# kienduynguyen/BoxeR

Hardware: AMD Instinct MI355X
Metric: box-attn fwd+bwd Gsample-points/s + achieved HBM GB/s, BoxeR-R50 COCO shapes (higher is better)
Workload: dtype bf16; 1 GPU; C2: box-attn fwd+bwd, levels 100x100/50x50/25x25/13x13, Lq=13294, H=8, C=32, P=4, B=2 images per GPU, inputs=model; parallelism=dp1, preheat_steps=2128, parity_gate=not run (--full runs it)

## Files before the change

boxer_amd/csrc/boxattn_binned.h:

```cpp
#pragma once
#include <type_traits>

#include "boxattn_device.h"
#include "boxattn_combine.h"
#include "boxattn_binplan.h"
#include "boxattn_scan_tail.h"
#include "boxattn_binpass.h"

namespace boxattn {

#ifndef BOXATTN_TUNE_BIN_THREADS
#define BOXATTN_TUNE_BIN_THREADS 512
#endif
constexpr int kBinThreads = BOXATTN_TUNE_BIN_THREADS;
template <int BW, int BH, bool FILL, bool WIDE, int PT>
__global__ __launch_bounds__(kBinThreads) void bin_kernel(const float *__restrict__ loc,
                                                  const float *__restrict__ w_sp, BinPlan plan,
                                                  int H, int Lq, int P, int q_per_wg, int n_wg, int interleave,
                                                  int *__restrict__ part,
                                                  const int *__restrict__ subtot,
                                                  const int *__restrict__ offsets,
                                                  int *__restrict__ records, int *__restrict__ ctickets)
{
    if (FILL && ctickets && blockIdx.x == 0)
        for (int k = threadIdx.x; k < plan.nblk; k += kBinThreads) ctickets[(size_t)blockIdx.y * plan.nblk + k] = 0;
    extern __shared__ int sh_bins[];
    __shared__ BinLevel s_lv[kMaxBinLevels];
    const int s = blockIdx.y, wg = blockIdx.x;
    bin_pass_body<kBinThreads, BW, BH, FILL, WIDE, PT>(sh_bins, s_lv, loc, w_sp, plan, H, Lq, P, q_per_wg, n_wg,
                                                       interleave != 0, part, subtot, offsets, records, s, wg);
    if constexpr (!FILL) {
        int *mypart = part + ((size_t)s * n_wg + wg) * plan.nblk;
        for (int k = threadIdx.x; k < plan.nblk; k += kBinThreads) mypart[k] = sh_bins[k];
    }
}

__global__ __launch_bounds__(256) void bin_scan_a_kernel(int *__restrict__ part, int n_wg,
                                                         int *__restrict__ subtot, BinPlan plan)
{
    const int sub = blockIdx.x, s = blockIdx.y;
    const int wps = scan_wps(n_wg);
    const int w_lo = sub * wps, w_hi = min(n_wg, w_lo + wps);
    int *sp = part + (size_t)s * n_wg * plan.nblk;
    for (int k = blockIdx.z * 256 + threadIdx.x; k < plan.nblk; k += 256 * gridDim.z) {
        int t[kScanWgPerSub], sum = 0;
#pragma unroll
        for (int u = 0; u < kScanWgPerSub; ++u)
            t[u] = w_lo + u < w_hi ? sp[(size_t)(w_lo + u) * plan.nblk + k] : 0;
#pragma unroll
        for (int u = 0; u < kScanWgPerSub; ++u) {
            if (w_lo + u < w_hi) sp[(size_t)(w_lo + u) * plan.nblk + k] = sum;
            sum += t[u];
        }
        subtot[((size_t)s * kScanSub + sub) * plan.nblk + k] = sum;
    }
}

__global__ __launch_bounds__(kScanThreads) void bin_scan_kernel(int *__restrict__ subtot,
                                                       int *__restrict__ offsets,
                                                       int4 *__restrict__ items,
                                                       int4 *__restrict__ combos,
                                                       int *__restrict__ n_items, BinPlan plan,
                                                       int *__restrict__ part, int fuse_wg)
{
    __shared__ int wsum[4][kScanThreads / 64];
    __shared__ int carry[4];
    const int s = blockIdx.x, lane = threadIdx.x & 63, wv = threadIdx.x >> 6;
    if (threadIdx.x < 4) carry[threadIdx.x] = 0;
    __syncthreads();
    for (int k0 = 0; k0 < plan.nblk; k0 += kScanThreads) {
        const int k = k0 + threadIdx.x;
        const bool live = k < plan.nblk;
        int c = 0;
        if (live && fuse_wg > 0) {
            const int wps = scan_wps(fuse_wg);
            int *sp = part + (size_t)s * fuse_wg * plan.nblk + k;
            for (int u = 0; u < kScanSub; ++u) {
                subtot[((size_t)s * kScanSub + u) * plan.nblk + k] = c;
                int in_sub = 0;
                const int w_hi = min(fuse_wg, (u + 1) * wps);
                for (int w = u * wps; w < w_hi; ++w) {
                    const int t = sp[(size_t)w * plan.nblk];
                    sp[(size_t)w * plan.nblk] = in_sub;
                    in_sub += t;
                }
                c += in_sub;
            }
        } else if (live) {
            int t[kScanSub];
#pragma unroll
            for (int u = 0; u < kScanSub; ++u)
                t[u] = subtot[((size_t)s * kScanSub + u) * plan.nblk + k];
#pragma unroll
            for (int u = 0; u < kScanSub; ++u) {
                subtot[((size_t)s * kScanSub + u) * plan.nblk + k] = c;
                c += t[u];
            }
        }
        const int nch = live ? max(plan.min_items, (c + plan.chunk - 1) / plan.chunk) : 0;
        const int v[4] = {c, nch, nch > 1 ? nch : 0, nch > 1 ? 1 : 0};
        int inc[4];
#pragma unroll
        for (int i = 0; i < 4; ++i) {
            int x = v[i];
#pragma unroll
            for (int o = 1; o < 64; o <<= 1) {
                const int t = __shfl_up(x, o, 64);
                if (lane >= o) x += t;
            }
            inc[i] = x;
            if (lane == 63) wsum[i][wv] = x;
        }
        __syncthreads();
        int ex[4];
#pragma unroll
        for (int i = 0; i < 4; ++i) {
            int pre = carry[i];
            for (int w = 0; w < wv; ++w) pre += wsum[i][w];
            ex[i] = pre + inc[i] - v[i];
        }
        int tot_items = carry[1];
        for (int w = 0; w < kScanThreads / 64; ++w) tot_items += wsum[1][w];
        if (live) {
            offsets[(size_t)s * (plan.nblk + 1) + k] = ex[0];
            int level = 0;
#pragma unroll
            for (int l = 1; l < kMaxBinLevels; ++l)
                if (l < plan.L && k >= plan.lv[l].blk0) level = l;
            BinLevel lv = plan.lv[0];
#pragma unroll
            for (int l = 1; l < kMaxBinLevels; ++l)
                if (l == level) lv = plan.lv[l];
            const int geo = (int)pack_block_geo(lv, level, k);
            const int csz = chunk_records(c, nch);
            for (int j = 0; j < nch; ++j)
                items[(size_t)s * plan.item_cap + (tot_items - 1 - (ex[1] + j))] =
                    make_int4(geo, ex[0] + j * csz, ex[0] + min(c, (j + 1) * csz),
                              nch > 1 ? (ex[2] + j) | (ex[3] << kItemSlotBits) : -1);
            if (nch > 1)
                combos[(size_t)s * plan.nblk + ex[3]] = make_int4(geo, ex[2], nch, 0);
        }
        __syncthreads();
        if (threadIdx.x == kScanThreads - 1) {
#pragma unroll
            for (int i = 0; i < 4; ++i) carry[i] = ex[i] + v[i];
        }
        __syncthreads();
    }
    if (threadIdx.x == 0) {
        offsets[(size_t)s * (plan.nblk + 1) + plan.nblk] = carry[0];
        n_items[2 * s] = carry[1];
        n_items[2 * s + 1] = carry[3];
    }
}

__global__ __launch_bounds__(kScanThreads) void bin_scan_seg_kernel(int *__restrict__ subtot,
                                                                    int *__restrict__ offsets,
                                                                    int4 *__restrict__ tmp,
                                                                    int4 *__restrict__ segtot,
                                                                    BinPlan plan, int *__restrict__ part = nullptr,
                                                                    int fuse_wg = 0)
{
    __shared__ int wsum[4][kScanThreads / 64];
    const int seg = blockIdx.x, s = blockIdx.y, lane = threadIdx.x & 63, wv = threadIdx.x >> 6;
    const int k = seg * kScanThreads + (int)threadIdx.x;
    const bool live = k < plan.nblk;
    int c = 0;
    if (live && fuse_wg > 0) {
        const int wps = scan_wps(fuse_wg);
        int *sp = part + (size_t)s * fuse_wg * plan.nblk + k;
        for (int u = 0; u < kScanSub; ++u) {
            subtot[((size_t)s * kScanSub + u) * plan.nblk + k] = c;
            int in_sub = 0;
            const int w_hi = min(fuse_wg, (u + 1) * wps);
            for (int w = u * wps; w < w_hi; ++w) {
                const int t = sp[(size_t)w * plan.nblk];
                sp[(size_t)w * plan.nblk] = in_sub;
                in_sub += t;
            }
            c += in_sub;
        }
    } else if (live) {
        int t[kScanSub];
#pragma unroll
        for (int u = 0; u < kScanSub; ++u) t[u] = subtot[((size_t)s * kScanSub + u) * plan.nblk + k];
#pragma unroll
        for (int u = 0; u < kScanSub; ++u) {
            subtot[((size_t)s * kScanSub + u) * plan.nblk + k] = c;
            c += t[u];
        }
    }
    const int nch = live ? max(plan.min_items, (c + plan.chunk - 1) / plan.chunk) : 0;
    const int v[4] = {c, nch, nch > 1 ? nch : 0, nch > 1 ? 1 : 0};
    int inc[4];
#pragma unroll
    for (int i = 0; i < 4; ++i) {
        int x = v[i];
#pragma unroll
        for (int o = 1; o < 64; o <<= 1) {
            const int t = __shfl_up(x, o, 64);
            if (lane >= o) x += t;
        }
        inc[i] = x;
        if (lane == 63) wsum[i][wv] = x;
    }
    __syncthreads();
    int ex[4], tot[4];
#pragma unroll
    for (int i = 0; i < 4; ++i) {
        int pre = 0, all = 0;
#pragma unroll
        for (int w = 0; w < kScanThreads / 64; ++w) {
            pre += w < wv ? wsum[i][w] : 0;
            all += wsum[i][w];
        }
        ex[i] = pre + inc[i] - v[i];
        tot[i] = all;
    }
    if (live) {
        offsets[(size_t)s * (plan.nblk + 1) + k] = c;
        tmp[(size_t)s * plan.nblk + k] = make_int4(ex[0], ex[1], ex[2], ex[3]);
    }
    if (threadIdx.x == 0)
        segtot[(size_t)s * gridDim.x + seg] = make_int4(tot[0], tot[1], tot[2], tot[3]);
}

__global__ __launch_bounds__(kScanThreads) void bin_scan_emit_kernel(int *__restrict__ offsets,
                                                                     const int4 *__restrict__ tmp,
                                                                     const int4 *__restrict__ segtot,
                                                                     int4 *__restrict__ items,
                                                                     int4 *__restrict__ combos,
                                                                     int *__restrict__ n_items,
                                                                     BinPlan plan)
{
    const int seg = blockIdx.x, s = blockIdx.y;
    int base[4] = {0, 0, 0, 0}, all[4] = {0, 0, 0, 0};
    for (int g = 0; g < (int)gridDim.x; ++g) {
        const int4 t = segtot[(size_t)s * gridDim.x + g];
        const int tv[4] = {t.x, t.y, t.z, t.w};
#pragma unroll
        for (int i = 0; i < 4; ++i) {
            base[i] += g < seg ? tv[i] : 0;
            all[i] += tv[i];
        }
    }
    const int k = seg * kScanThreads + (int)threadIdx.x;
    if (k < plan.nblk) {
        const int c = offsets[(size_t)s * (plan.nblk + 1) + k];
        const int4 e = tmp[(size_t)s * plan.nblk + k];
        const int ex[4] = {base[0] + e.x, base[1] + e.y, base[2] + e.z, base[3] + e.w};
        const int nch = max(plan.min_items, (c + plan.chunk - 1) / plan.chunk);
        offsets[(size_t)s * (plan.nblk + 1) + k] = ex[0];
        int level = 0;
#pragma unroll
        for (int l = 1; l < kMaxBinLevels; ++l)
            if (l < plan.L && k >= plan.lv[l].blk0) level = l;
        BinLevel lv = plan.lv[0];
#pragma unroll
        for (int l = 1; l < kMaxBinLevels; ++l)
            if (l == level) lv = plan.lv[l];
        const int geo = (int)pack_block_geo(lv, level, k);
        const int csz = chunk_records(c, nch);
        for (int j = 0; j < nch; ++j)
            items[(size_t)s * plan.item_cap + (all[1] - 1 - (ex[1] + j))] =
                make_int4(geo, ex[0] + j * csz, ex[0] + min(c, (j + 1) * csz),
                          nch > 1 ? (ex[2] + j) | (ex[3] << kItemSlotBits) : -1);
        if (nch > 1) combos[(size_t)s * plan.nblk + ex[3]] = make_int4(geo, ex[2], nch, 0);
    }
    if (seg == 0 && threadIdx.x == 0) {
        offsets[(size_t)s * (plan.nblk + 1) + plan.nblk] = all[0];
        n_items[2 * s] = all[1];
        n_items[2 * s + 1] = all[3];
    }
}

#ifndef BOXATTN_TUNE_ABLATE
#define BOXATTN_TUNE_ABLATE 0
#endif
#ifndef BOXATTN_TUNE_ACC_WPE
#define BOXATTN_TUNE_ACC_WPE 1
#endif
template <typename ST, int C, bool INST, int RPL = 1, bool WIDE = false>
__global__ __launch_bounds__(64) __attribute__((amdgpu_waves_per_eu(BOXATTN_TUNE_ACC_WPE)))
void binned_accumulate_kernel(
    const ST *__restrict__ grad_out, const ST *__restrict__ grad_mask,
    const float *__restrict__ loc, const float *__restrict__ w_sp,
    const float *__restrict__ w_lv, BinPlan plan, int S, int H, int Lq, int P,
    const int *__restrict__ offsets, const int4 *__restrict__ items,
    const int *__restrict__ n_items, const int *__restrict__ records,
    ST *__restrict__ grad_value, float *__restrict__ partials, ChunkCombine cc, ZeroRole zr)
{
    constexpr int BW = 8, PB = 32;
    constexpr int R = 64 * RPL;
    constexpr int CH = C / 2;
    constexpr int ROWB = C * (int)sizeof(ST);
#ifndef BOXATTN_TUNE_STAGE_F32
#define BOXATTN_TUNE_STAGE_F32 0
#endif
    constexpr bool kCvt = INST || (BOXATTN_TUNE_STAGE_F32 && sizeof(ST) == 2);
    constexpr int SB = kCvt ? 4 : (int)sizeof(ST);
    constexpr int RS = C * SB + 16;
    constexpr int LPR = ROWB / 16;
    constexpr int RPP = 64 / LPR;
    constexpr int NPASS = R / RPP;
    constexpr int EPL = 16 / (int)sizeof(ST);
#ifndef BOXATTN_TUNE_UNR
#define BOXATTN_TUNE_UNR 2
#endif
    constexpr int UNR = BOXATTN_TUNE_UNR;
    typedef float2 Entry;
    typedef unsigned int u32x4 __attribute__((ext_vector_type(4)));
    constexpr int NQ = CH * SB / 16;
    auto staged_pair = [](const u32x4 (&rw)[NQ], int i) -> f32x2 {
        f32x2 r;
        if constexpr (SB == 4) {
            r.x = __uint_as_float(rw[(2 * i) / 4][(2 * i) % 4]);
            r.y = __uint_as_float(rw[(2 * i + 1) / 4][(2 * i + 1) % 4]);
        } else {
            const unsigned wd = rw[i / 4][i % 4];
            r.x = __uint_as_float(wd << 16); r.y = __uint_as_float(wd & 0xffff0000u);
        }
        return r;
    };
    __shared__ __attribute__((aligned(16))) unsigned char gstage[(R + 1) * RS];
    __shared__ __attribute__((aligned(16))) Entry ent[4 * R + PB * (UNR - 1) + UNR];
    __shared__ int pcnt[PB + 1], poff[PB + 1];
    __shared__ int last_flag;

    const int n_slices = plan.n_slices, workers = (int)gridDim.x - plan.zero_workers;
    const int bid = blockIdx.y * gridDim.x + blockIdx.x;
    const int xcd = bid % 8, k = bid / 8;
    const int per_xcd = (n_slices + 7) / 8;
// ... 296 lines not shown
```

boxer_amd/csrc/boxattn_binned_tr.h:

```cpp
#pragma once
#include "boxattn_binplan.h"
#include "boxattn_combine.h"
#include "boxattn_scan_tail.h"
#include "boxattn_binpass.h"

namespace boxattn {

#ifndef BOXATTN_TUNE_TR_WPE
#define BOXATTN_TUNE_TR_WPE 4
#endif
#ifndef BOXATTN_TUNE_REC_AHEAD
#define BOXATTN_TUNE_REC_AHEAD 1
#endif

typedef __bf16 tr_bf16x8 __attribute__((ext_vector_type(8)));
typedef float tr_f32x16 __attribute__((ext_vector_type(16)));
typedef short tr_i16x4 __attribute__((ext_vector_type(4)));
__device__ __forceinline__ uint2 lds_read_tr16(const unsigned short *base, unsigned byte_off)
{
    typedef __attribute__((address_space(3))) tr_i16x4 lds_vec;
    const tr_i16x4 v = __builtin_amdgcn_ds_read_tr16_b64_v4i16(
        (lds_vec *)(reinterpret_cast<const char *>(base) + byte_off));
    return __builtin_bit_cast(uint2, v);
}

template <typename ST, int C>
__global__ __launch_bounds__(64) __attribute__((amdgpu_waves_per_eu(C <= 32 ? BOXATTN_TUNE_TR_WPE : 1))) void binned_accumulate_tr_kernel(
    const ST *__restrict__ grad_out, unsigned grad_out_bytes, BinPlan plan, int S, int H, int Lq,
    const int4 *__restrict__ items, const int *__restrict__ n_items,
    const int *__restrict__ records, ST *__restrict__ grad_value, float *__restrict__ partials, ChunkCombine cc,
    ZeroRole zr)
{
    static_assert(sizeof(ST) == 2, "bf16 storage");
    static_assert(C == 16 || C == 32 || C == 64, "channels per head");
    constexpr int BW = 8, PB = 32, R = 64;
    constexpr int CP = C < 32 ? 32 : C;
    constexpr int NCB = CP / 32;
    constexpr int ROWB = C * 2;
    constexpr int LPR = ROWB / 16;
    constexpr int RPP = 64 / LPR;
    constexpr int NPASS = R / RPP;
    constexpr int GPL = R * 64;
    constexpr int AS = 72;
    constexpr int ASB = AS * 2;
    constexpr int kDump = PB * ASB;
    constexpr int kBig = 1 << 20;
    typedef unsigned int u32x4 __attribute__((ext_vector_type(4)));
    __shared__ __attribute__((aligned(16))) unsigned short gs[NCB * GPL / 2];
    __shared__ __attribute__((aligned(16))) unsigned short at[(PB + 1) * AS];
    __shared__ int last_flag;

    const int n_slices = plan.n_slices, workers = (int)gridDim.x - plan.zero_workers;
    const int bid = blockIdx.y * gridDim.x + blockIdx.x;
    const int xcd = bid % 8, kq = bid / 8;
    const int per_xcd = (n_slices + 7) / 8;
    const int s = slice_on_xcd(xcd, kq % per_xcd, per_xcd);
    const int worker = kq / per_xcd - plan.zero_workers;
    if (s >= n_slices || worker >= workers) return;
    const int b = s / H, h = s % H;
    const int lane = threadIdx.x;
    if (worker < 0) {
        if (zr.redo) redo_blocks<ST, C>(zr, plan, s, worker + plan.zero_workers, plan.zero_workers, S, H, Lq, grad_out, grad_value, lane);
        else zero_empty_blocks<ST, C>(zr, plan.nblk, s, worker + plan.zero_workers, S, H, grad_value, lane);
        return;
    }
    const int col = lane & 31, kb = lane >> 5;
    const int n_it = n_items[2 * s];

    for (int i = lane; i < (PB + 1) * AS / 2; i += 64) reinterpret_cast<unsigned int *>(at)[i] = 0u;
    if (C < CP)
        for (int i = lane; i < NCB * GPL / 4; i += 64) reinterpret_cast<unsigned int *>(gs)[i] = 0u;
    wave_lds_sync();

    const __amdgpu_buffer_rsrc_t rs =
        __builtin_amdgcn_make_buffer_rsrc(const_cast<ST *>(grad_out), 0, grad_out_bytes, 0x00020000);
    const unsigned slice_off = (unsigned)((b * Lq) * H + h) * (unsigned)ROWB;
    const unsigned q_stride = (unsigned)(H * ROWB);
    const int piece = lane % LPR, jrow = lane / LPR;
    const unsigned stage_off = (unsigned)((piece >> 2) * GPL + jrow * 64 + (piece & 3) * 16);
    const int g16 = lane >> 4, i16 = lane & 15;
    const unsigned tr_off = (unsigned)((8 * (g16 >> 1) + (i16 >> 2)) * 64 + (16 * (g16 & 1) + 4 * (i16 & 3)) * 2);
    unsigned a_off = (unsigned)(col * ASB + 16 * kb);
    asm volatile("" : "+v"(a_off));

    const int4 *my_items = items + (size_t)s * plan.item_cap;
    int4 item_n = my_items[min(worker, plan.item_cap - 1)];
    for (int it = worker; it < n_it; it += workers) {
        const int4 item = item_n;
        item_n = my_items[min(it + workers, plan.item_cap - 1)];
        const BlockGeo bg = unpack_block_geo((unsigned)item.x);
        int lvH = plan.lv[0].H, lvW = plan.lv[0].W, lv_start = plan.lv[0].start;
#pragma unroll
        for (int k = 1; k < kMaxBinLevels; ++k)
            if (k == bg.level) { lvH = plan.lv[k].H; lvW = plan.lv[k].W; lv_start = plan.lv[k].start; }
        const int oy = bg.oy, ox = bg.ox, bh = bg.bh, bw = bg.bw;
        const float Hf = (float)lvH, Wf = (float)lvW;
        const int4 *rec = reinterpret_cast<const int4 *>(records) + (size_t)s * plan.rec_cap;
        tr_f32x16 acc[NCB];
#pragma unroll
        for (int cb = 0; cb < NCB; ++cb)
#pragma unroll
            for (int r = 0; r < 16; ++r) acc[cb][r] = 0.f;

        constexpr unsigned kNoRow = 0x80000000u;
        auto fetch_rec = [&](int rr) -> int4 {
            if (rr + lane >= item.z) return make_int4(-1, 0, 0, 0);
            return rec[rr + lane];
        };
        auto fetch_rows = [&](const int4 &r, u32x4 (&rows)[NPASS]) {
            const unsigned id = (unsigned)r.x;
            const unsigned off = r.x < 0 ? kNoRow : __umul24(id >> plan.lp_bits, q_stride) + slice_off;
#pragma unroll
            for (int ps = 0; ps < NPASS; ++ps) {
                const unsigned oj = (unsigned)__shfl((int)off, ps * RPP + jrow, 64) + (unsigned)(piece * 16);
                rows[ps] = __builtin_amdgcn_raw_buffer_load_b128(rs, oj, 0, 0);
            }
        };
        auto stage_rows = [&](const u32x4 (&rows)[NPASS]) {
#pragma unroll
            for (int ps = 0; ps < NPASS; ++ps)
                *reinterpret_cast<u32x4 *>(reinterpret_cast<char *>(gs) + stage_off + ps * RPP * 64) = rows[ps];
        };
        int4 rec_c = fetch_rec(item.y), rec_n = fetch_rec(item.y + R), rec_n2 = fetch_rec(item.y + 2 * R);
        u32x4 grow_a[NPASS], grow_b[NPASS];
        fetch_rows(rec_c, grow_a);
        stage_rows(grow_a);
        if (item.y + R < item.z) fetch_rows(rec_n, grow_a);
        auto round = [&](int rr, const u32x4 (&next)[NPASS], u32x4 (&ahead)[NPASS]) {
            const bool more = rr + R < item.z;
            int4 rec_n3 = make_int4(-1, 0, 0, 0);
            if (rr + 2 * R < item.z) {
                fetch_rows(rec_n2, ahead);
                rec_n3 = fetch_rec(rr + 3 * R);
            }
            const float x = __int_as_float(rec_c.y), y = __int_as_float(rec_c.z), a = __int_as_float(rec_c.w);
            float h_im, w_im;
            {
#pragma clang fp contract(off)
                h_im = y * Hf - 0.5f;
                w_im = x * Wf - 0.5f;
            }
            const float yf = floorf(h_im), xf = floorf(w_im);
            const float lh = h_im - yf, lw = w_im - xf;
            const int py = rec_c.x >= 0 ? (int)yf - oy : -2, px = (int)xf - ox;
            const float hh = 1.f - lh, hw = 1.f - lw;
            const float ha = hh * a, la = lh * a;
            const float w0 = ha * hw, w1 = ha * lw, w2 = la * hw, w3 = la * lw;
            const unsigned hi01 = pack_bf16x2(w0, w1), hi23 = pack_bf16x2(w2, w3);
            const unsigned lo01 = pack_bf16x2(w0 - __uint_as_float(hi01 << 16), w1 - __uint_as_float(hi01 & 0xffff0000u));
            const unsigned lo23 = pack_bf16x2(w2 - __uint_as_float(hi23 << 16), w3 - __uint_as_float(hi23 & 0xffff0000u));
            const int r0 = (unsigned)py < (unsigned)bh ? __mul24(py, BW * ASB) : kBig;
            const int r1 = (unsigned)(py + 1) < (unsigned)bh ? __mul24(py, BW * ASB) + BW * ASB : kBig;
            const int c0 = (unsigned)px < (unsigned)bw ? __mul24(px, ASB) + 2 * lane : kBig;
            const int c1 = (unsigned)(px + 1) < (unsigned)bw ? __mul24(px, ASB) + 2 * lane + ASB : kBig;
            const int dump = kDump + 2 * lane;
            const int slot[4] = {min(r0 + c0, dump), min(r0 + c1, dump), min(r1 + c0, dump), min(r1 + c1, dump)};
            auto put = [&](int k, unsigned short v) {
                *reinterpret_cast<unsigned short *>(reinterpret_cast<char *>(at) + slot[k]) = v;
            };
            put(0, (unsigned short)(hi01 & 0xffffu)); put(1, (unsigned short)(hi01 >> 16));
            put(2, (unsigned short)(hi23 & 0xffffu)); put(3, (unsigned short)(hi23 >> 16));
            wave_lds_sync();
            tr_bf16x8 g[R / 16][NCB];
#pragma unroll
            for (int t = 0; t < R / 16; ++t) {
                const tr_bf16x8 p_hi = __builtin_bit_cast(
                    tr_bf16x8, *reinterpret_cast<const u32x4 *>(reinterpret_cast<const char *>(at) + a_off + 32 * t));
#pragma unroll
                for (int cb = 0; cb < NCB; ++cb) {
                    const uint2 g0 = lds_read_tr16(gs, tr_off + cb * GPL + t * 1024);
                    const uint2 g1 = lds_read_tr16(gs, tr_off + cb * GPL + t * 1024 + 256);
                    g[t][cb] = __builtin_bit_cast(tr_bf16x8, u32x4{g0.x, g0.y, g1.x, g1.y});
                    acc[cb] = __builtin_amdgcn_mfma_f32_32x32x16_bf16(g[t][cb], p_hi, acc[cb], 0, 0, 0);
                }
            }
            wave_lds_sync();
            put(0, (unsigned short)(lo01 & 0xffffu)); put(1, (unsigned short)(lo01 >> 16));
            put(2, (unsigned short)(lo23 & 0xffffu)); put(3, (unsigned short)(lo23 >> 16));
            wave_lds_sync();
#pragma unroll
            for (int t = 0; t < R / 16; ++t) {
                const tr_bf16x8 p_lo = __builtin_bit_cast(
                    tr_bf16x8, *reinterpret_cast<const u32x4 *>(reinterpret_cast<const char *>(at) + a_off + 32 * t));
#pragma unroll
                for (int cb = 0; cb < NCB; ++cb)
                    acc[cb] = __builtin_amdgcn_mfma_f32_32x32x16_bf16(g[t][cb], p_lo, acc[cb], 0, 0, 0);
            }
            wave_lds_sync();
#pragma unroll
            for (int k = 0; k < 4; ++k) put(k, (unsigned short)0);
            if (more) {
                stage_rows(next);
                rec_c = rec_n; rec_n = rec_n2; rec_n2 = rec_n3;
            }
            wave_lds_sync();
        };
        for (int rr = item.y; rr < item.z; rr += 2 * R) {
            round(rr, grow_a, grow_b);
            if (rr + R >= item.z) break;
            round(rr + R, grow_b, grow_a);
        }
        if (item.w < 0) {
            int ln = lane;
            asm volatile("" : "+v"(ln));
            const int py = (ln & 31) / BW, px = (ln & 31) % BW;
            const bool live = py < bh && px < bw;
            ST *dst = grad_value +
                      (((size_t)b * S + lv_start + (size_t)(oy + py) * lvW + (ox + px)) * H + h) * C;
#pragma unroll
            for (int cb = 0; cb < NCB; ++cb) {
                unsigned pk[8];
#pragma unroll
                for (int i = 0; i < 8; ++i) pk[i] = pack_bf16x2(acc[cb][2 * i], acc[cb][2 * i + 1]);
                u32x4 piece_lo, piece_hi;
                {
                    const auto s0 = __builtin_amdgcn_permlane32_swap(pk[0], pk[2], false, false);
                    const auto s1 = __builtin_amdgcn_permlane32_swap(pk[1], pk[3], false, false);
                    const auto s2 = __builtin_amdgcn_permlane32_swap(pk[4], pk[6], false, false);
                    const auto s3 = __builtin_amdgcn_permlane32_swap(pk[5], pk[7], false, false);
                    piece_lo = u32x4{s0[0], s1[0], s0[1], s1[1]};
                    piece_hi = u32x4{s2[0], s3[0], s2[1], s3[1]};
                }
                const int c_lo = cb * 32 + 8 * kb, c_hi = cb * 32 + 16 + 8 * kb;
#ifndef BOXATTN_TUNE_GV_NT
#define BOXATTN_TUNE_GV_NT 0
#endif
                if (BOXATTN_TUNE_GV_NT) {
                    if (live && c_lo < C) __builtin_nontemporal_store(piece_lo, reinterpret_cast<u32x4 *>(dst + c_lo));
                    if (live && c_hi < C) __builtin_nontemporal_store(piece_hi, reinterpret_cast<u32x4 *>(dst + c_hi));
                } else {
                    if (live && c_lo < C) *reinterpret_cast<u32x4 *>(dst + c_lo) = piece_lo;
                    if (live && c_hi < C) *reinterpret_cast<u32x4 *>(dst + c_hi) = piece_hi;
                }
            }
        } else {
            const bool publish = cc.tickets != nullptr;
            const __amdgpu_buffer_rsrc_t tile =
                partial_tile(partials, s, plan.pslot_cap, item.w & ((1 << kItemSlotBits) - 1), C);
            int ln = lane;
            asm volatile("" : "+v"(ln));
            const unsigned lane_off = (unsigned)(((ln & 31) * C + 4 * (ln >> 5)) * 4);
#pragma unroll
            for (int cb = 0; cb < NCB; ++cb)
#pragma unroll
                for (int g4 = 0; g4 < 4; ++g4) {
                    const int c = cb * 32 + 8 * g4;
                    if (c + 4 * kb < C)
                        partial_store(tile, lane_off + (unsigned)(c * 4),
                                      make_float4(acc[cb][4 * g4], acc[cb][4 * g4 + 1], acc[cb][4 * g4 + 2],
                                                  acc[cb][4 * g4 + 3]), publish);
                }
            if (publish) chunk_finish<ST, C>(cc, partials, lv_start, lvW, S, H, grad_value, s, item.w, lane, &last_flag);
        }
    }
}

struct InstRows {
    const float *grad_mask;
    unsigned grad_mask_bytes;
    const float *w_lv;
    int P;
};
template <int C, bool INST = false>
__global__ __launch_bounds__(64) __attribute__((amdgpu_waves_per_eu(INST ? 2 : 3, INST ? 2 : 3))) void binned_accumulate_split_kernel(
    const float *__restrict__ grad_out, unsigned grad_out_bytes, BinPlan plan, int S, int H, int Lq,
    const int4 *__restrict__ items, const int *__restrict__ n_items,
    const int *__restrict__ records, float *__restrict__ grad_value, float *__restrict__ partials, ChunkCombine cc,
    ZeroRole zr, InstRows inst)
{
    static_assert(C == 32, "channels per head");
    constexpr int BW = 8, PB = 32, R = 64;
    constexpr int ROWB = C * 4;
    constexpr int LPR = ROWB / 16;
    constexpr int RPP = 64 / LPR;
    constexpr int NPASS = R / RPP;
    constexpr int GPL = R * 64;
    constexpr int AS = 72, ASB = AS * 2;
    constexpr int kDump = PB * ASB;
    constexpr int kBig = 1 << 20;
    typedef unsigned int u32x4 __attribute__((ext_vector_type(4)));
    __shared__ __attribute__((aligned(16))) unsigned short gs[2 * GPL / 2];
    __shared__ __attribute__((aligned(16))) unsigned short at[(PB + 1) * AS];
    __shared__ int last_flag;

    const int n_slices = plan.n_slices, workers = (int)gridDim.x - plan.zero_workers;
    const int bid = blockIdx.y * gridDim.x + blockIdx.x;
    const int xcd = bid % 8, kq = bid / 8;
    const int per_xcd = (n_slices + 7) / 8;
    const int s = slice_on_xcd(xcd, kq % per_xcd, per_xcd);
    const int worker = kq / per_xcd - plan.zero_workers;
    if (s >= n_slices || worker >= workers) return;
    const int b = s / H, h = s % H;
    const int lane = threadIdx.x;
    if (worker < 0) {
        if (zr.redo) redo_blocks<float, C>(zr, plan, s, worker + plan.zero_workers, plan.zero_workers, S, H, Lq, grad_out, grad_value, lane);
        else zero_empty_blocks<float, C>(zr, plan.nblk, s, worker + plan.zero_workers, S, H, grad_value, lane);
        return;
    }
    const int col = lane & 31, kb = lane >> 5;
    const int n_it = n_items[2 * s];
    for (int i = lane; i < (PB + 1) * AS / 2; i += 64) reinterpret_cast<unsigned int *>(at)[i] = 0u;
    wave_lds_sync();

    const __amdgpu_buffer_rsrc_t rs =
        __builtin_amdgcn_make_buffer_rsrc(const_cast<float *>(grad_out), 0, grad_out_bytes, 0x00020000);
    const unsigned slice_off = (unsigned)((b * Lq) * H + h) * (unsigned)ROWB;
    const unsigned q_stride = (unsigned)(H * ROWB);
    const __amdgpu_buffer_rsrc_t rsm = __builtin_amdgcn_make_buffer_rsrc(
        const_cast<float *>(INST ? inst.grad_mask : grad_out), 0, INST ? inst.grad_mask_bytes : grad_out_bytes, 0x00020000);
    const int P = INST ? inst.P : 1, LP = plan.L * P;
    const unsigned m_slice_off = (unsigned)((b * Lq) * P * H + h) * (unsigned)ROWB;
    const unsigned m_q_stride = (unsigned)(P * H * ROWB), m_p_stride = (unsigned)(H * ROWB);
    const float rcp_p = 1.0f / (float)P;
    const int lp_mask = (1 << plan.lp_bits) - 1;
    const int piece = lane % LPR, jrow = lane / LPR;
    const unsigned stage_off = (unsigned)(jrow * 64 + piece * 8);
    const int g16 = lane >> 4, i16 = lane & 15;
    const unsigned tr_off = (unsigned)((8 * (g16 >> 1) + (i16 >> 2)) * 64 + (16 * (g16 & 1) + 4 * (i16 & 3)) * 2);
    unsigned a_off = (unsigned)(col * ASB + 16 * kb);
    asm volatile("" : "+v"(a_off));

    const int4 *my_items = items + (size_t)s * plan.item_cap;
    int4 item_n = my_items[min(worker, plan.item_cap - 1)];
    const int4 *rec_s = reinterpret_cast<const int4 *>(records) + (size_t)s * plan.rec_cap;
    int4 rec_first = make_int4(-1, 0, 0, 0);
    if (BOXATTN_TUNE_REC_AHEAD && worker < n_it && item_n.y + lane < item_n.z) rec_first = rec_s[item_n.y + lane];
    for (int it = worker; it < n_it; it += workers) {
        const int4 item = item_n;
        item_n = my_items[min(it + workers, plan.item_cap - 1)];
        const BlockGeo bg = unpack_block_geo((unsigned)item.x);
        int lvH = plan.lv[0].H, lvW = plan.lv[0].W, lv_start = plan.lv[0].start;
#pragma unroll
        for (int k = 1; k < kMaxBinLevels; ++k)
            if (k == bg.level) { lvH = plan.lv[k].H; lvW = plan.lv[k].W; lv_start = plan.lv[k].start; }
        const int oy = bg.oy, ox = bg.ox, bh = bg.bh, bw = bg.bw;
        const float Hf = (float)lvH, Wf = (float)lvW;
        const int4 *rec = reinterpret_cast<const int4 *>(records) + (size_t)s * plan.rec_cap;
        tr_f32x16 acc;
#pragma unroll
        for (int r = 0; r < 16; ++r) acc[r] = 0.f;

        constexpr unsigned kNoRow = 0x80000000u;
        auto fetch_rec = [&](int rr) -> int4 {
            if (rr + lane >= item.z) return make_int4(-1, 0, 0, 0);
            return rec[rr + lane];
        };
        u32x4 rows[NPASS], rows_m[INST ? NPASS : 1];
        float as_rows = 0.f, al_rows = 0.f;
        auto fetch_rows = [&](const int4 &r) {
            const unsigned off = r.x < 0 ? kNoRow : __umul24((unsigned)r.x >> plan.lp_bits, q_stride) + slice_off;
            unsigned off_m = kNoRow;
            if constexpr (INST) {
                const unsigned q = (unsigned)max(r.x, 0) >> plan.lp_bits;
                const int lp = max(r.x, 0) & lp_mask;
                int l_, p_;
                divmod_small(lp, P, rcp_p, l_, p_);
                off_m = r.x < 0 ? kNoRow : q * m_q_stride + (unsigned)p_ * m_p_stride + m_slice_off;
                as_rows = r.x < 0 ? 0.f : __int_as_float(r.w);
                al_rows = r.x < 0 ? 0.f : inst.w_lv[(((size_t)b * Lq + q) * H + h) * LP + lp];
            }
#pragma unroll
            for (int ps = 0; ps < NPASS; ++ps) {
                const unsigned oj = (unsigned)__shfl((int)off, ps * RPP + jrow, 64) + (unsigned)(piece * 16);
                rows[ps] = __builtin_amdgcn_raw_buffer_load_b128(rs, oj, 0, 0);
                if constexpr (INST) {
                    const unsigned om = (unsigned)__shfl((int)off_m, ps * RPP + jrow, 64) + (unsigned)(piece * 16);
                    rows_m[ps] = __builtin_amdgcn_raw_buffer_load_b128(rsm, om, 0, 0);
                }
            }
        };
        auto split2 = [](float &x0, float &x1) -> unsigned {
            const unsigned pk = pack_bf16x2(x0, x1);
            x0 -= __uint_as_float(pk << 16);
            x1 -= __uint_as_float(pk & 0xffff0000u);
            return pk;
        };
        int4 rec_c = BOXATTN_TUNE_REC_AHEAD ? rec_first : fetch_rec(item.y);
        int4 rec_n = fetch_rec(item.y + R), rec_n2 = fetch_rec(item.y + 2 * R);
        fetch_rows(rec_c);
        if (BOXATTN_TUNE_REC_AHEAD) {
            rec_first = make_int4(-1, 0, 0, 0);
            if (it + workers < n_it && item_n.y + lane < item_n.z) rec_first = rec_s[item_n.y + lane];
        }
        for (int rr = item.y; rr < item.z; rr += R) {
            const bool more = rr + R < item.z;
            int4 rec_n3 = make_int4(-1, 0, 0, 0);
            if (rr + 3 * R < item.z) rec_n3 = fetch_rec(rr + 3 * R);
            uint2 g3pk[NPASS];
#pragma unroll
            for (int ps = 0; ps < NPASS; ++ps) {
                float x0 = __uint_as_float(rows[ps].x), x1 = __uint_as_float(rows[ps].y);
                float x2 = __uint_as_float(rows[ps].z), x3 = __uint_as_float(rows[ps].w);
                if constexpr (INST) {
                    const float as_j = __shfl(as_rows, ps * RPP + jrow, 64), al_j = __shfl(al_rows, ps * RPP + jrow, 64);
                    x0 = fmaf(al_j, __uint_as_float(rows_m[ps].x), as_j * x0);
                    x1 = fmaf(al_j, __uint_as_float(rows_m[ps].y), as_j * x1);
                    x2 = fmaf(al_j, __uint_as_float(rows_m[ps].z), as_j * x2);
                    x3 = fmaf(al_j, __uint_as_float(rows_m[ps].w), as_j * x3);
                }
                uint2 t1, t2;
                t1.x = split2(x0, x1); t1.y = split2(x2, x3);
                t2.x = split2(x0, x1); t2.y = split2(x2, x3);
                g3pk[ps] = uint2{pack_bf16x2(x0, x1), pack_bf16x2(x2, x3)};
                *reinterpret_cast<uint2 *>(reinterpret_cast<char *>(gs) + stage_off + ps * RPP * 64) = t1;
                *reinterpret_cast<uint2 *>(reinterpret_cast<char *>(gs) + GPL + stage_off + ps * RPP * 64) = t2;
            }
            if (more) fetch_rows(rec_n);
            const float x = __int_as_float(rec_c.y), y = __int_as_float(rec_c.z), a = INST ? 1.f : __int_as_float(rec_c.w);
            float h_im, w_im;
            {
#pragma clang fp contract(off)
                h_im = y * Hf - 0.5f;
                w_im = x * Wf - 0.5f;
            }
            const float yf = floorf(h_im), xf = floorf(w_im);
            const float lh = h_im - yf, lw = w_im - xf, hh = 1.f - lh, hw = 1.f - lw;
            float w0 = hh * hw * a, w1 = hh * lw * a, w2 = lh * hw * a, w3 = lh * lw * a;
            const unsigned t1_01 = split2(w0, w1), t1_23 = split2(w2, w3);
            const unsigned t2_01 = split2(w0, w1), t2_23 = split2(w2, w3);
            const unsigned t3_01 = pack_bf16x2(w0, w1), t3_23 = pack_bf16x2(w2, w3);
            const int py = rec_c.x >= 0 ? (int)yf - oy : -2, px = (int)xf - ox;
            const int r0 = (unsigned)py < (unsigned)bh ? __mul24(py, BW * ASB) : kBig;
            const int r1 = (unsigned)(py + 1) < (unsigned)bh ? __mul24(py, BW * ASB) + BW * ASB : kBig;
            const int c0 = (unsigned)px < (unsigned)bw ? __mul24(px, ASB) + 2 * lane : kBig;
            const int c1 = (unsigned)(px + 1) < (unsigned)bw ? __mul24(px, ASB) + 2 * lane + ASB : kBig;
            const int dump = kDump + 2 * lane;
            const int slot[4] = {min(r0 + c0, dump), min(r0 + c1, dump), min(r1 + c0, dump), min(r1 + c1, dump)};
            auto put4 = [&](unsigned p01, unsigned p23) {
                *reinterpret_cast<unsigned short *>(reinterpret_cast<char *>(at) + slot[0]) = (unsigned short)(p01 & 0xffffu);
                *reinterpret_cast<unsigned short *>(reinterpret_cast<char *>(at) + slot[1]) = (unsigned short)(p01 >> 16);
                *reinterpret_cast<unsigned short *>(reinterpret_cast<char *>(at) + slot[2]) = (unsigned short)(p23 & 0xffffu);
                *reinterpret_cast<unsigned short *>(reinterpret_cast<char *>(at) + slot[3]) = (unsigned short)(p23 >> 16);
            };
            put4(t1_01, t1_23);
            wave_lds_sync();
            tr_bf16x8 g1[R / 16], g2[R / 16], g3[R / 16];
#pragma unroll
            for (int t = 0; t < R / 16; ++t) {
                const uint2 a0 = lds_read_tr16(gs, tr_off + t * 1024), a1 = lds_read_tr16(gs, tr_off + t * 1024 + 256);
                g1[t] = __builtin_bit_cast(tr_bf16x8, u32x4{a0.x, a0.y, a1.x, a1.y});
                const uint2 b0 = lds_read_tr16(gs, GPL + tr_off + t * 1024), b1 = lds_read_tr16(gs, GPL + tr_off + t * 1024 + 256);
                g2[t] = __builtin_bit_cast(tr_bf16x8, u32x4{b0.x, b0.y, b1.x, b1.y});
            }
            wave_lds_sync();
#pragma unroll
            for (int ps = 0; ps < NPASS; ++ps)
                *reinterpret_cast<uint2 *>(reinterpret_cast<char *>(gs) + stage_off + ps * RPP * 64) = g3pk[ps];
            wave_lds_sync();
#pragma unroll
            for (int t = 0; t < R / 16; ++t) {
                const uint2 a0 = lds_read_tr16(gs, tr_off + t * 1024), a1 = lds_read_tr16(gs, tr_off + t * 1024 + 256);
                g3[t] = __builtin_bit_cast(tr_bf16x8, u32x4{a0.x, a0.y, a1.x, a1.y});
            }
            auto weights = [&](int t) -> tr_bf16x8 {
                return __builtin_bit_cast(
                    tr_bf16x8, *reinterpret_cast<const u32x4 *>(reinterpret_cast<const char *>(at) + a_off + 32 * t));
            };
#pragma unroll
            for (int t = 0; t < R / 16; ++t) {
                const tr_bf16x8 pw = weights(t);
                acc = __builtin_amdgcn_mfma_f32_32x32x16_bf16(g3[t], pw, acc, 0, 0, 0);
                acc = __builtin_amdgcn_mfma_f32_32x32x16_bf16(g2[t], pw, acc, 0, 0, 0);
                acc = __builtin_amdgcn_mfma_f32_32x32x16_bf16(g1[t], pw, acc, 0, 0, 0);
            }
            wave_lds_sync();
            put4(t2_01, t2_23);
            wave_lds_sync();
#pragma unroll
            for (int t = 0; t < R / 16; ++t) {
                const tr_bf16x8 pw = weights(t);
                acc = __builtin_amdgcn_mfma_f32_32x32x16_bf16(g2[t], pw, acc, 0, 0, 0);
                acc = __builtin_amdgcn_mfma_f32_32x32x16_bf16(g1[t], pw, acc, 0, 0, 0);
            }
            wave_lds_sync();
            put4(t3_01, t3_23);
            wave_lds_sync();
#pragma unroll
            for (int t = 0; t < R / 16; ++t)
                acc = __builtin_amdgcn_mfma_f32_32x32x16_bf16(g1[t], weights(t), acc, 0, 0, 0);
            wave_lds_sync();
            put4(0u, 0u);
            rec_c = rec_n; rec_n = rec_n2; rec_n2 = rec_n3;
            wave_lds_sync();
        }
        if (item.w < 0) {
            int ln = lane;
            asm volatile("" : "+v"(ln));
            const int py = (ln & 31) / BW, px = (ln & 31) % BW, kbs = ln >> 5;
            const bool live = py < bh && px < bw;
            float *dst = grad_value + (((size_t)b * S + lv_start + (size_t)(oy + py) * lvW + (ox + px)) * H + h) * C;
#pragma unroll
            for (int g4 = 0; g4 < 4; ++g4)
                if (live)
                    *reinterpret_cast<float4 *>(dst + 8 * g4 + 4 * kbs) =
                        make_float4(acc[4 * g4], acc[4 * g4 + 1], acc[4 * g4 + 2], acc[4 * g4 + 3]);
        } else {
            const bool publish = cc.tickets != nullptr;
            const __amdgpu_buffer_rsrc_t tile =
                partial_tile(partials, s, plan.pslot_cap, item.w & ((1 << kItemSlotBits) - 1), C);
            int ln = lane;
            asm volatile("" : "+v"(ln));
            const unsigned lane_off = (unsigned)(((ln & 31) * C + 4 * (ln >> 5)) * 4);
#pragma unroll
// ... 169 lines not shown
```

boxer_amd/csrc/boxattn_binpass.h:

```cpp
#pragma once
#include "boxattn_binplan.h"
#include "boxattn_ride.h"
#include "boxattn_scan_tail.h"

namespace boxattn {

template <int THREADS, int BW, int BH, bool FILL, bool WIDE, int PT>
__device__ __forceinline__ void bin_pass_body(int *hist, BinLevel *s_lv, const float *__restrict__ loc,
                                              const float *__restrict__ w_sp, const BinPlan &plan, int H,
                                              int Lq, int P, int q_per_wg, int n_wg, bool interleave,
                                              const int *__restrict__ part, const int *__restrict__ subtot,
                                              const int *__restrict__ offsets, int *__restrict__ records,
                                              int s, int wg)
{
    const int b = s / H, h = s % H;
    const int LP = plan.L * P;
    const int q0 = interleave ? wg : wg * q_per_wg, qstep = interleave ? n_wg : 1;
    const int n_q = interleave ? (q0 < Lq ? (Lq - q0 + qstep - 1) / qstep : 0)
                               : max(0, min(q0 + q_per_wg, Lq) - q0);
    const int *mypart = part + ((size_t)s * n_wg + wg) * plan.nblk;

    const float2 *loc2 = reinterpret_cast<const float2 *>(loc);
    static_assert(PT == 1 || PT == 4, "points per thread and step");
#ifndef BOXATTN_TUNE_BIN_U
#define BOXATTN_TUNE_BIN_U 2
#endif
    constexpr int U = PT == 4 ? BOXATTN_TUNE_BIN_U : 4;
    const size_t pid0 = (((size_t)b * Lq + q0) * H + h) * LP;
    const size_t qstride = (size_t)H * LP * qstep;
    const int LPG = LP / PT, n_grp = n_q * LPG;
    const float rcp_lpg = 1.0f / (float)LPG, rcp_p = 1.0f / (float)P;
    int *rec = records + (size_t)s * plan.rec_cap * (WIDE ? 4 : 1);
    struct Step {
        float2 xy[U][PT];
        float wv[U][PT];
        int lp0[U], ql[U];
    };
    auto load_step = [&](Step &t, int g0) {
#pragma unroll
        for (int u = 0; u < U; ++u) {
            const int g = min(g0 + u * THREADS, n_grp - 1);
            int lg;
            divmod_small(g, LPG, rcp_lpg, t.ql[u], lg);
            t.lp0[u] = lg * PT;
            const size_t base = pid0 + t.ql[u] * qstride + t.lp0[u];
            if constexpr (PT == 4) {
                const float4 *p4 = reinterpret_cast<const float4 *>(loc2 + base);
                const float4 a = p4[0], c = p4[1];
                t.xy[u][0] = make_float2(a.x, a.y); t.xy[u][1] = make_float2(a.z, a.w);
                t.xy[u][2] = make_float2(c.x, c.y); t.xy[u][3] = make_float2(c.z, c.w);
                if constexpr (FILL && WIDE) {
                    const float4 w4 = *reinterpret_cast<const float4 *>(w_sp + base);
                    t.wv[u][0] = w4.x; t.wv[u][1] = w4.y; t.wv[u][2] = w4.z; t.wv[u][3] = w4.w;
                }
            } else {
                t.xy[u][0] = loc2[base];
                if constexpr (FILL && WIDE) t.wv[u][0] = w_sp[base];
            }
            if constexpr (!(FILL && WIDE)) {
#pragma unroll
                for (int k = 0; k < PT; ++k) t.wv[u][k] = 0.f;
            }
        }
    };
    auto put_record = [&](const Step &t, int u, int k, int slot) {
        const int id = ((q0 + t.ql[u] * qstep) << plan.lp_bits) | (t.lp0[u] + k);
        if constexpr (WIDE)
            reinterpret_cast<int4 *>(rec)[slot] = make_int4(id, __float_as_int(t.xy[u][k].x),
                                                            __float_as_int(t.xy[u][k].y), __float_as_int(t.wv[u][k]));
        else
            rec[slot] = id;
    };
    auto work_step = [&](const Step &t, int g0) {
#pragma unroll
        for (int u = 0; u < U; ++u) {
            if (g0 + u * THREADS >= n_grp) break;
            const BinLevel lv = s_lv[(int)(((float)t.lp0[u] + 0.5f) * rcp_p)];
#pragma unroll
            for (int k = 0; k < PT; ++k) {
                int blk[4];
                touched_blocks(t.xy[u][k].x, t.xy[u][k].y, lv, blk);
#pragma unroll
                for (int j = 0; j < 4; ++j) {
                    if (blk[j] >= 0) {
                        const int slot = atomicAdd(&hist[blk[j]], 1);
                        if constexpr (FILL) put_record(t, u, k, slot);
                    }
                }
            }
        }
    };
    constexpr int STRIDE = THREADS * U;
    Step sa, sb;
    if (n_grp > 0) load_step(sa, (int)threadIdx.x);
    if (threadIdx.x == 0) {
#pragma unroll
        for (int k = 0; k < kMaxBinLevels; ++k) s_lv[k] = plan.lv[k];
    }
    const int wps = scan_wps(n_wg);
    const int *mysub = subtot + ((size_t)s * kScanSub + wg / wps) * plan.nblk;
    for (int k = threadIdx.x; k < plan.nblk; k += THREADS)
        hist[k] = FILL ? mypart[k] + mysub[k] + offsets[(size_t)s * (plan.nblk + 1) + k] : 0;
    __syncthreads();
    for (int base = 0; base < n_grp; base += 2 * STRIDE) {
        const int g0 = base + (int)threadIdx.x;
        if (base + STRIDE < n_grp) load_step(sb, g0 + STRIDE);
        work_step(sa, g0);
        if (base + STRIDE >= n_grp) break;
        if (base + 2 * STRIDE < n_grp) load_step(sa, g0 + 2 * STRIDE);
        work_step(sb, g0 + STRIDE);
    }
    if constexpr (!FILL) __syncthreads();
}

enum { kRideWide = 1, kRideInterleave = 2, kRidePt4 = 4,
       kRideSpec = 8 };
constexpr int kRideMaxBlocks = 3072;
constexpr int kRideLdsInts = kRideMaxBlocks + 8 * (int)(sizeof(BinLevel) / sizeof(int)) + 4 * 4 + 2;

struct SpecRide {
    int *cursor;
    int *cbase;
    int2 *redo;
    unsigned long long *stats;
};
struct BinRide {
    const float *loc, *w_sp;
    int *part, *subtot, *offsets, *records;
    int4 *items, *combos;
    int *n_items;
    int *tickets;
    int *ctickets;
    BinPlan plan;
    int H, Lq, P, q_per_wg, n_wg;
    unsigned nwg_magic;
    int flavour;
    RideGrid grid;
    SpecRide spec;
    unsigned long long *trace;
};
#ifndef BOXATTN_RIDE_TRACE
#define BOXATTN_RIDE_TRACE 0
#endif
#define RIDE_STAMP(k_)                                                                              \
    do {                                                                                            \
        if (BOXATTN_RIDE_TRACE && r.trace && threadIdx.x == 0) {                                    \
            __builtin_amdgcn_sched_barrier(0);                                                      \
            r.trace[(size_t)id * 8 + (k_)] = __builtin_amdgcn_s_memrealtime();                      \
        }                                                                                           \
    } while (0)

struct RideLds {
    int *hist;
    BinLevel *lv;
    int *wsum;
    int *flag;
    __device__ __forceinline__ explicit RideLds(int *base)
        : hist(base), lv(reinterpret_cast<BinLevel *>(base + kRideMaxBlocks)),
          wsum(base + kRideMaxBlocks + 8 * (int)(sizeof(BinLevel) / sizeof(int))),
          flag(base + kRideMaxBlocks + 8 * (int)(sizeof(BinLevel) / sizeof(int)) + 16) {}
};
static_assert(kMaxBinLevels == 8, "RideLds reserves 8 levels");

template <int THREADS>
__device__ __forceinline__ void bin_count_ride(const BinRide r, unsigned id, int *lds)
{
    static_assert(THREADS == 256, "4 wave sums per scan quantity");
    if (id >= r.grid.n_riders) return;
#ifndef BOXATTN_TUNE_RIDE_PRIO
#define BOXATTN_TUNE_RIDE_PRIO 0
#endif
    if (BOXATTN_TUNE_RIDE_PRIO) __builtin_amdgcn_s_setprio(BOXATTN_TUNE_RIDE_PRIO);
    RIDE_STAMP(0);
    const RideLds m(lds);
    const BinPlan plan = r.plan;
    unsigned s_u, wg_u;
    divmod_magic(id, (unsigned)r.n_wg, r.nwg_magic, s_u, wg_u);
    const int s = (int)s_u, wg = (int)wg_u;
    const bool inter = (r.flavour & kRideInterleave) != 0;
    if (r.flavour & kRidePt4)
        bin_pass_body<THREADS, 8, 4, false, false, 4>(m.hist, m.lv, r.loc, r.w_sp, plan, r.H, r.Lq, r.P, r.q_per_wg,
                                                     r.n_wg, inter, r.part, r.subtot, r.offsets, r.records, s, wg);
    else
        bin_pass_body<THREADS, 8, 4, false, false, 1>(m.hist, m.lv, r.loc, r.w_sp, plan, r.H, r.Lq, r.P, r.q_per_wg,
                                                     r.n_wg, inter, r.part, r.subtot, r.offsets, r.records, s, wg);
    RIDE_STAMP(1);
    int *mypart = r.part + ((size_t)s * r.n_wg + wg) * plan.nblk;
    for (int k = threadIdx.x; k < plan.nblk; k += THREADS) agent_store(mypart + k, m.hist[k]);
    stores_left();
    const int wps = scan_wps(r.n_wg), u = wg / wps;
    const int n_in_sub = min(r.n_wg, (u + 1) * wps) - u * wps, n_sub = (r.n_wg + wps - 1) / wps;
    int *tk = r.tickets + (size_t)s * kRideTickets;
    const bool last = last_arriver<THREADS>(tk + u, n_in_sub, m.flag);
    RIDE_STAMP(2);
    if (!last) return;
    const ScanOut o{r.subtot, r.offsets, r.items, r.combos, r.n_items};
    if (n_sub == 1) {
        RIDE_STAMP(3);
        if (plan.nblk <= kScanThreads) scan_blocks_body<THREADS>(o, plan, m.lv, 1, s, m.wsum, r.part, r.n_wg);
        else scan_blocks_big_body<THREADS>(o, plan, m.lv, 1, s, m.wsum, m.hist, r.part, r.n_wg);
    } else {
        scan_sub_body<THREADS>(r.part, r.subtot, plan, r.n_wg, s, u);
        stores_left();
        RIDE_STAMP(3);
        if (!last_arriver<THREADS>(tk + kScanSub, n_sub, m.flag)) return;
        if (plan.nblk <= kScanThreads) scan_blocks_body<THREADS>(o, plan, m.lv, n_sub, s, m.wsum);
        else scan_blocks_big_body<THREADS>(o, plan, m.lv, n_sub, s, m.wsum, m.hist);
    }
    RIDE_STAMP(4);
}

template <int THREADS> __device__ __forceinline__ void bin_fill_spec_ride(const BinRide r, unsigned id, int *lds);

template <int THREADS>
__device__ __forceinline__ void bin_fill_ride(const BinRide r, unsigned id, int *lds)
{
    if (id >= r.grid.n_riders) return;
    if (BOXATTN_TUNE_RIDE_PRIO) __builtin_amdgcn_s_setprio(BOXATTN_TUNE_RIDE_PRIO);
    if (r.flavour & kRideSpec) {
        bin_fill_spec_ride<THREADS>(r, id, lds);
        return;
    }
    RIDE_STAMP(5);
    const RideLds m(lds);
    const BinPlan plan = r.plan;
    unsigned s_u, wg_u;
    divmod_magic(id, (unsigned)r.n_wg, r.nwg_magic, s_u, wg_u);
    const int s = (int)s_u, wg = (int)wg_u;
    const bool inter = (r.flavour & kRideInterleave) != 0;
    if (wg == 0 && r.ctickets)
        for (int k = threadIdx.x; k < plan.nblk; k += THREADS) r.ctickets[(size_t)s * plan.nblk + k] = 0;
    if ((r.flavour & kRideWide) && (r.flavour & kRidePt4))
        bin_pass_body<THREADS, 8, 4, true, true, 4>(m.hist, m.lv, r.loc, r.w_sp, plan, r.H, r.Lq, r.P, r.q_per_wg,
                                                   r.n_wg, inter, r.part, r.subtot, r.offsets, r.records, s, wg);
    else if (r.flavour & kRideWide)
        bin_pass_body<THREADS, 8, 4, true, true, 1>(m.hist, m.lv, r.loc, r.w_sp, plan, r.H, r.Lq, r.P, r.q_per_wg,
                                                   r.n_wg, inter, r.part, r.subtot, r.offsets, r.records, s, wg);
    else
        bin_pass_body<THREADS, 8, 4, true, false, 1>(m.hist, m.lv, r.loc, r.w_sp, plan, r.H, r.Lq, r.P, r.q_per_wg,
                                                    r.n_wg, inter, r.part, r.subtot, r.offsets, r.records, s, wg);
    if (BOXATTN_RIDE_TRACE) { stores_left(); __syncthreads(); }
    RIDE_STAMP(6);
}

}

#include "boxattn_spec.h"
```

boxer_amd/csrc/boxattn_binplan.h:

```cpp
#pragma once
#include "boxattn_device.h"
#include "boxattn_combine.h"

namespace boxattn {

struct BinLevel {
    int H, W, start;
    int nbx, nby;
    int blk0;
    unsigned mw, mh;
    unsigned mnx, mny;
};

__device__ __forceinline__ int blk_of(int x, int nb, unsigned magic)
{
    return (int)__umulhi((unsigned)__mul24(x, nb), magic);
}
__device__ __forceinline__ int blk_lo(int c, int size, int nb) { return (c * size + nb - 1) / nb; }
__device__ __forceinline__ int div_nb(int n, int nb, unsigned magic)
{
    return magic ? (int)__umulhi((unsigned)n, magic) : n / nb;
}

struct BinPlan {
    int L;
    int nblk;
    int rec_cap;
    int item_cap;
    int chunk;
    int lp_bits;
    int n_slices;
    int pslot_cap;
    int min_items;
    int zero_workers;
    BinLevel lv[kMaxBinLevels];
};

#ifndef BOXATTN_TUNE_SLICE_MAP
#define BOXATTN_TUNE_SLICE_MAP 1
#endif
__device__ __forceinline__ int slice_on_xcd(int xcd, int i, int per_xcd)
{
    return BOXATTN_TUNE_SLICE_MAP ? xcd * per_xcd + i : xcd + 8 * i;
}

__device__ __forceinline__ void touched_blocks(float x, float y, const BinLevel &lv, int (&blk)[4])
{
    float h_im, w_im;
    {
#pragma clang fp contract(off)
        h_im = y * (float)lv.H - 0.5f;
        w_im = x * (float)lv.W - 0.5f;
    }
    const bool inside = h_im > -1.f && w_im > -1.f && h_im < (float)lv.H && w_im < (float)lv.W &&
                        lv.H > 0 && lv.W > 0;
    const int y0 = (int)floorf(inside ? h_im : 0.f), x0 = (int)floorf(inside ? w_im : 0.f);
    const int ra = blk_of(max(y0, 0), lv.nby, lv.mh), rb = blk_of(min(y0 + 1, lv.H - 1), lv.nby, lv.mh);
    const int ca = blk_of(max(x0, 0), lv.nbx, lv.mw), cb = blk_of(min(x0 + 1, lv.W - 1), lv.nbx, lv.mw);
    const int base_a = lv.blk0 + ra * lv.nbx, base_b = lv.blk0 + rb * lv.nbx;
    blk[0] = inside ? base_a + ca : -1;
    blk[1] = inside && cb != ca ? base_a + cb : -1;
    blk[2] = inside && rb != ra ? base_b + ca : -1;
    blk[3] = inside && rb != ra && cb != ca ? base_b + cb : -1;
}

}
```

boxer_amd/csrc/boxattn_capi.hip:

```cpp
#include "../../include/boxattn.h"

#include <hip/hip_runtime.h>

#include <algorithm>
#include <atomic>
#include <map>
#include <mutex>
#include <type_traits>
#include <vector>

#include "boxattn_binned.h"
#include "boxattn_fast.h"
#include "boxattn_gather2.h"
#include "boxattn_dense_plan.h"
#include "boxattn_generic.h"

using namespace boxattn;

namespace {

std::atomic<int> g_variant{0};

enum { kOptBinChunk = 10,
       kOptDense = 11,
// ... 117 lines not shown
    ix.rcp_p = 1.0f / (float)d.P;
    ix.head_xcd = (d.H == 8 && (long long)d.Lq * 4 <= d.S &&
                   (size_t)d.B * d.S * d.C * elem_bytes <= (3u << 20))
                      ? 1u : 0u;
    return true;
}
inline int gather_blocks(const Dims &d, const GatherIdx &ix, int pairs)
{
    if (ix.head_xcd) return 8 * ceil_div_sz((size_t)d.B * d.Lq, (size_t)pairs * 4);
    return ceil_div_sz(d.n_qh(), (size_t)pairs * 4);
}
inline GatherIdx with_grid(GatherIdx ix, int grid_x, int grid_y, int tiles)
{
    ix.grid_x = (unsigned)grid_x;
    ix.grid_y = (unsigned)std::max(1, grid_y);
    ix.tps = (unsigned)((tiles + (int)ix.grid_y - 1) / (int)ix.grid_y);
    return ix;
}
template <typename ST> struct GatherVec8 {
    static constexpr bool value = (sizeof(ST) == 2 ? BOXATTN_TUNE_VEC_BF16 : BOXATTN_TUNE_VEC_F32) == 8;
};
#define BOXATTN_GATHER_DISPATCH(cfg, X)                                                       \
    do {                                                                                      \
        if ((cfg).VEC == 8) {                                                                 \
            if constexpr (GatherVec8<ST>::value) {                                            \
                if ((cfg).G == 4) { X(4, 8) } else { X(8, 8) }                                \
            }                                                                                 \
        } else if ((cfg).G == 4) { X(4, 4) } else if ((cfg).G == 8) { X(8, 4) } else { X(16, 4) } \
    } while (0)

inline int point_split(int blocks, int tiles)
{
    if (blocks >= 1024 || tiles < 2) return 1;
    return std::max(1, std::min(tiles, (4096 + blocks - 1) / blocks));
}

inline int finish()
{
    return (int)hipGetLastError();
}

struct EventPair { hipEvent_t a, b; };
enum { kSlotFwd = 0, kSlotBwdPoints = 1, kSlotBwdAccum = 2, kSlotBwdBin = 3, kSlotBwdCombine = 4,
       kSlotBwdPrep = 5, kNumSlots = BOXATTN_PROFILE_SLOTS };
struct Profile {
    std::atomic<bool> on{false};
    std::mutex mu;
    std::vector<EventPair> ev[kNumSlots];
} g_prof;
constexpr size_t kMaxProfiled = 4096;

struct ScopedKernelTimer {
    hipStream_t st;
    EventPair ev{};
    std::vector<EventPair> *dst = nullptr;
    ScopedKernelTimer(std::vector<EventPair> &v, hipStream_t s) : st(s)
    {
        if (!g_prof.on.load(std::memory_order_relaxed)) return;
        if (hipEventCreate(&ev.a) != hipSuccess) return;
        if (hipEventCreate(&ev.b) != hipSuccess) { (void)hipEventDestroy(ev.a); return; }
        dst = &v;
        (void)hipEventRecord(ev.a, st);
    }
    ~ScopedKernelTimer()
    {
        if (!dst) return;
        (void)hipEventRecord(ev.b, st);
        std::lock_guard<std::mutex> g(g_prof.mu);
        if (dst->size() < kMaxProfiled) dst->push_back(ev);
        else { (void)hipEventDestroy(ev.a); (void)hipEventDestroy(ev.b); }
    }
};

inline void drain(std::vector<EventPair> &v, double *ms_sum, int *n)
{
    double sum = 0;
    int cnt = 0;
    for (auto &e : v) {
        float ms = 0;
        if (hipEventSynchronize(e.b) == hipSuccess &&
            hipEventElapsedTime(&ms, e.a, e.b) == hipSuccess) {
            sum += ms;
            ++cnt;
        }
        (void)hipEventDestroy(e.a);
        (void)hipEventDestroy(e.b);
    }
    v.clear();
    if (ms_sum) *ms_sum = sum;
    if (n) *n = cnt;
}


inline BinRide place_riders(const BinRide *ride_in, unsigned own_blocks, unsigned *total)
{
    BinRide ride = ride_in ? *ride_in : BinRide{};
    ride.grid = ride_grid(ride.grid.n_riders, own_blocks, ride.grid.shift, total);
    return ride;
}

inline bool make_dense_plan(const Dims &d, const int64_t *sh, const int64_t *ls, DensePlan &p, int elem);

template <typename ST, bool INST>
int launch_fwd(const ST *value, const int64_t *shapes, const int64_t *lsi,
               const typename Storage<ST>::compute *loc,
               const typename Storage<ST>::compute *w_sp,
               const typename Storage<ST>::compute *w_lv, const Dims &d, ST *out, ST *mask,
               hipStream_t st, const int64_t *shapes_host = nullptr,
               const int64_t *lsi_host = nullptr, const BinRide *count_ride = nullptr,
               bool *ride_taken = nullptr, bool allow_dense = true, unsigned long long *stats = nullptr)
{
    if (ride_taken) *ride_taken = false;
    if (!d.valid()) return (int)hipErrorInvalidValue;
    if (d.empty()) return 0;
    if (!shapes || !lsi || !loc || !w_sp || !out || (INST && (!w_lv || !mask)))
        return (int)hipErrorInvalidValue;
    const size_t n_qh = d.n_qh();
    if (d.n_value() == 0) {
        hipError_t e = zero_async(out, n_qh * d.C * sizeof(ST), st);
        if (e == hipSuccess && INST)
            e = zero_async(mask, n_qh * d.C * d.P * sizeof(ST), st);
        return (int)e;
    }
    if (!value) return (int)hipErrorInvalidValue;
    if constexpr (!std::is_same<ST, double>::value) {
        if (fast_ok<ST>(d, value, loc, out, INST ? (const void *)mask : (const void *)out,
                        out)) {
            if constexpr (!INST && std::is_same<ST, bf16_t>::value) {
                DensePlan dp;
                if (allow_dense && shapes_host && lsi_host && aligned(value, 16) && aligned(out, 16) &&
                    aligned(loc, 8) && make_dense_plan(d, shapes_host, lsi_host, dp, 2)) {
                    ScopedKernelTimer timer(g_prof.ev[kSlotFwd], st);
                    launch_fwd_dense(value, loc, w_sp, out, dp, (unsigned)(d.n_value() * sizeof(bf16_t)),
                                     count_ride ? *count_ride : BinRide{}, stats, st);
                    if (count_ride && ride_taken) *ride_taken = true;
                    return finish();
                }
            }
            if constexpr (!INST && std::is_same<ST, float>::value) {
                DensePlan dp;
                if (allow_dense && shapes_host && lsi_host && aligned(value, 16) && aligned(out, 16) &&
                    aligned(loc, 8) && make_dense_plan(d, shapes_host, lsi_host, dp, 4)) {
                    ScopedKernelTimer timer(g_prof.ev[kSlotFwd], st);
                    launch_fwd_dense_f32(value, loc, w_sp, out, dp, (unsigned)(d.n_value() * sizeof(float)),
                                         count_ride ? *count_ride : BinRide{}, stats, st);
                    if (count_ride && ride_taken) *ride_taken = true;
                    return finish();
                }
            }
            const size_t vbytes = d.n_value() * sizeof(ST);
            GatherIdx ix{};
            const bool gen2 = g_variant != 2 && vbytes < kOobOffset && gather_idx(d, ix, sizeof(ST));
            const GatherCfg cfg =
                gen2 ? gather_cfg<ST>(d, aligned(value, 16) && aligned(out, 16) &&
                                         (!INST || aligned(mask, 16)))
                     : GatherCfg{fast_group(d), 4};
            const int G = cfg.G;
            const int pairs = kWave / G;
            const int blocks = gen2 ? gather_blocks(d, ix, pairs) : ceil_div_sz(n_qh, (size_t)pairs * 4);
            ScopedKernelTimer timer(g_prof.ev[kSlotFwd], st);
            if constexpr (INST) {
                if (gen2 && blocks < 1024 && d.P >= kWave / G) {
                    const int steps = ceil_div_sz((size_t)d.P, (size_t)(kWave / G));
                    const unsigned ws = steps >= 8 ? 4 : steps >= 4 ? 2 : 1;
                    const size_t ppw = 4 / ws;
                    const int wblocks = ix.head_xcd ? 8 * ceil_div_sz((size_t)d.B * d.Lq, ppw)
                                                    : ceil_div_sz(n_qh, ppw);
                    unsigned total = 0;
                    const BinRide ride = place_riders(count_ride, (unsigned)wblocks, &total);
#define BOXATTN_FWD_WIDE(GG, VV)                                                              \
    hipLaunchKernelGGL((fwd_inst_wide_kernel<ST, GG, VV>), dim3(total), dim3(256), 0, st,     \
                       value, shapes, lsi, loc, w_sp, w_lv, d.S, d.H, d.L, d.Lq, d.P, out,    \
                       mask, with_grid(ix, wblocks, 1, 1), (unsigned)vbytes, ride, ws);
                    BOXATTN_GATHER_DISPATCH(cfg, BOXATTN_FWD_WIDE);
#undef BOXATTN_FWD_WIDE
                    if (count_ride && ride_taken) *ride_taken = true;
                    return finish();
                }
            }
            if (gen2) {
                unsigned total = 0;
                const BinRide ride = place_riders(count_ride, (unsigned)blocks, &total);
#define BOXATTN_FWD2(GG, VV)                                                                  \
    hipLaunchKernelGGL((fwd2_kernel<ST, GG, INST, GatherUnroll<ST, GG, VV>::value, VV>),      \
                       dim3(total, 1), dim3(256), 0, st, value, shapes, lsi, loc, w_sp,       \
                       w_lv, d.S, d.H, d.L, d.Lq, d.P, out, mask,                             \
                       with_grid(ix, blocks, 1, (d.P + GG - 1) / GG), (unsigned)vbytes, ride);
                BOXATTN_GATHER_DISPATCH(cfg, BOXATTN_FWD2);
#undef BOXATTN_FWD2
                if (count_ride && ride_taken) *ride_taken = true;
            } else {
#define BOXATTN_FWD_CASE(GG)                                                                  \
    case GG:                                                                                  \
        hipLaunchKernelGGL((fwd_fast_kernel<ST, 4, GG, INST>), dim3(blocks), dim3(256), 0, st, \
                           value, shapes, lsi, loc, w_sp, w_lv, d.S, d.H, d.L, d.Lq, d.P, out, \
                           mask, n_qh);                                                       \
        break;
                switch (G) {
                    BOXATTN_FWD_CASE(4)
                    BOXATTN_FWD_CASE(8)
                    BOXATTN_FWD_CASE(16)
                }
#undef BOXATTN_FWD_CASE
            }
            return finish();
        }
        if (g_variant == 2) return (int)hipErrorInvalidValue;
    }
    const size_t n = n_qh * d.C;
    const int blocks = (int)std::min<size_t>((n + 255) / 256, (size_t)1 << 20);
    ScopedKernelTimer timer(g_prof.ev[kSlotFwd], st);
    hipLaunchKernelGGL((fwd_generic_kernel<ST, INST>), dim3(blocks), dim3(256), 0, st, value,
                       shapes, lsi, loc, w_sp, w_lv, d.S, d.H, d.C, d.L, d.Lq, d.P, out, mask,
                       n);
    return finish();
}

template <typename ST, bool INST>
int launch_bwd(const ST *value, const int64_t *shapes, const int64_t *lsi,
               const typename Storage<ST>::compute *loc,
               const typename Storage<ST>::compute *w_sp,
               const typename Storage<ST>::compute *w_lv, const ST *grad_out,
               const ST *grad_mask, const Dims &d, ST *grad_value,
               typename Storage<ST>::compute *grad_loc, typename Storage<ST>::compute *grad_sp,
               typename Storage<ST>::compute *grad_lv,
               typename Storage<ST>::compute *grad_value_acc, hipStream_t st)
{
    typedef typename Storage<ST>::compute T;
    if (!d.valid()) return (int)hipErrorInvalidValue;
    const size_t nv = d.n_value();
    const size_t n_qh = d.n_qh();
    if (nv) {
        if (!grad_value || !grad_value_acc) return (int)hipErrorInvalidValue;
        hipError_t e = zero_async(grad_value_acc, nv * sizeof(T), st);
        if (e != hipSuccess) return (int)e;
    }
    if (n_qh) {
        if (!shapes || !lsi || !loc || !w_sp || !grad_out || !grad_loc || !grad_sp ||
            (INST && (!w_lv || !grad_mask || !grad_lv)))
            return (int)hipErrorInvalidValue;
        if (!nv) {
            const size_t np = n_qh * d.L * d.P;
            hipError_t e = zero_async(grad_loc, 2 * np * sizeof(T), st);
            if (e == hipSuccess) e = zero_async(grad_sp, np * sizeof(T), st);
            if (e == hipSuccess && INST) e = zero_async(grad_lv, np * sizeof(T), st);
            return (int)e;
        }
        if (!value) return (int)hipErrorInvalidValue;
    }
    if (n_qh && nv) {
        ScopedKernelTimer timer(g_prof.ev[kSlotBwdPoints], st);
        bool done = false;
        if constexpr (!std::is_same<ST, double>::value) {
            if (fast_ok<ST>(d, value, loc, grad_out,
                            INST ? (const void *)grad_mask : (const void *)grad_out,
                            grad_loc)) {
                const int G = fast_group(d);
                const int pairs = kWave / G;
                const int blocks = ceil_div_sz(n_qh, (size_t)pairs * 4);
#define BOXATTN_BWD_CASE(GG)                                                                  \
    case GG:                                                                                  \
        hipLaunchKernelGGL((bwd_fast_kernel<ST, 4, GG, INST>), dim3(blocks), dim3(256), 0, st, \
                           value, shapes, lsi, loc, w_sp, w_lv, grad_out, grad_mask, d.S,    \
                           d.H, d.L, d.Lq, d.P, grad_value_acc, grad_loc, grad_sp, grad_lv,  \
                           n_qh);                                                             \
        break;
                switch (G) {
                    BOXATTN_BWD_CASE(4)
                    BOXATTN_BWD_CASE(8)
                    BOXATTN_BWD_CASE(16)
                }
#undef BOXATTN_BWD_CASE
                done = true;
            } else if (g_variant == 2) {
                return (int)hipErrorInvalidValue;
            }
        }
        if (!done) {
            const int blocks = (int)std::min<size_t>((n_qh + 3) / 4, (size_t)1 << 20);
            hipLaunchKernelGGL((bwd_generic_kernel<ST, INST>), dim3(blocks), dim3(256), 0, st,
                               value, shapes, lsi, loc, w_sp, w_lv, grad_out, grad_mask, d.S,
                               d.H, d.C, d.L, d.Lq, d.P, grad_value_acc, grad_loc, grad_sp,
                               grad_lv, n_qh);
        }
        int rc = finish();
        if (rc) return rc;
    }
    if constexpr (std::is_same<ST, bf16_t>::value) {
        if (nv) {
            const int blocks = (int)std::min<size_t>((nv / 4 + 255) / 256 + 1, 256 * 16);
            hipLaunchKernelGGL(cvt_f32_to_bf16_kernel, dim3(blocks), dim3(256), 0, st,
                               grad_value_acc, grad_value, nv);
            return finish();
        }
    }
    return 0;
}



#include "boxattn_host_plan.h"

template <typename ST, bool INST>
inline int bin_flavour(const Dims &d, const float *loc, const float *w_sp)
{
    const bool wide = acc_kind<ST, INST>(d) != kAccValu;
    const bool pt4 = d.P % 4 == 0 && aligned(loc, 16) && (!wide || aligned(w_sp, 16));
    return (wide ? kRideWide : kRideInterleave) | (pt4 ? kRidePt4 : 0);
}
inline BinRide make_ride(const float *loc, const float *w_sp, const Dims &d, const BinPlan &plan,
                         const PlanLayout &pl, char *pbuf, const ScratchLayout *sl, char *sbuf, int flavour,
                         bool fill)
{
    BinRide r{};
    r.loc = loc; r.w_sp = w_sp;
    r.part = (int *)(pbuf + pl.part); r.subtot = (int *)(pbuf + pl.subtot); r.offsets = (int *)(pbuf + pl.offsets);
    r.items = (int4 *)(pbuf + pl.items); r.combos = (int4 *)(pbuf + pl.combos);
    r.n_items = (int *)(pbuf + pl.n_items); r.tickets = (int *)(pbuf + pl.tickets);
    r.records = sl ? (int *)(sbuf + sl->records) : nullptr;
    r.ctickets = fill && sl ? (int *)(sbuf + sl->ctickets) : nullptr;
    r.plan = plan;
    r.H = d.H; r.Lq = d.Lq; r.P = d.P; r.q_per_wg = pl.q_per_wg; r.n_wg = pl.n_wg;
    r.nwg_magic = div_magic((unsigned)pl.n_wg);
    r.flavour = flavour;
    r.grid.n_riders = (unsigned)(pl.n_wg * d.B * d.H);
    r.grid.shift = ride_shift(fill);
    r.trace = (unsigned long long *)g_dense_dbg.load();
    return r;
}

enum { kBinCount = 1, kBinScan = 2, kBinFill = 4 };
inline void launch_binning(int flavour, const float *loc, const float *w_sp, const Dims &d, const BinPlan &plan,
                           const PlanLayout &w, char *pbuf, int *records, hipStream_t st, int stages,
                           int *ctickets = nullptr)
{
    constexpr int BW = 8, BH = 4;
    const int ns = d.B * d.H;
    int *part = (int *)(pbuf + w.part), *subtot = (int *)(pbuf + w.subtot);
    int *n_items = (int *)(pbuf + w.n_items), *offsets = (int *)(pbuf + w.offsets);
    int4 *items = (int4 *)(pbuf + w.items), *combos = (int4 *)(pbuf + w.combos);
    const dim3 bgrid(w.n_wg, ns);
    const size_t bsh = ((size_t)plan.nblk + 1) * sizeof(int);
    const int inter = (flavour & kRideInterleave) ? 1 : 0;
    const bool wide = (flavour & kRideWide) != 0, pt4 = (flavour & kRidePt4) != 0;
    ScopedKernelTimer timer(g_prof.ev[kSlotBwdBin], st);
#define BOXATTN_BIN(FILL_, WIDE_, PT_)                                                              \
    hipLaunchKernelGGL((bin_kernel<BW, BH, FILL_, WIDE_, PT_>), bgrid, dim3(kBinThreads), bsh, st, loc, w_sp, \
                       plan, d.H, d.Lq, d.P, w.q_per_wg, w.n_wg, inter, part, subtot, offsets, records, ctickets)
    if (stages & kBinCount) {
        if (pt4) BOXATTN_BIN(false, false, 4); else BOXATTN_BIN(false, false, 1);
        if (plan.zero_workers > 0)
            hipLaunchKernelGGL(zero_geo_kernel, dim3((plan.nblk + 255) / 256), dim3(256), 0, st, plan,
                               (int2 *)(pbuf + w.zgeo));
    }
#ifndef BOXATTN_TUNE_SCAN_FUSE_WG
#define BOXATTN_TUNE_SCAN_FUSE_WG 48
#endif
    const bool fuse_a = plan.nblk <= kScanThreads ? w.n_wg <= BOXATTN_TUNE_SCAN_FUSE_WG : w.n_wg <= 8;
    if (stages & kBinScan) {
        if (!fuse_a)
            hipLaunchKernelGGL(bin_scan_a_kernel,
                               dim3(kScanSub, ns, std::min(64, (plan.nblk + 255) / 256)), dim3(256), 0, st,
                               part, w.n_wg, subtot, plan);
        if (plan.nblk > kScanThreads) {
            const int nseg = (plan.nblk + kScanThreads - 1) / kScanThreads;
            int4 *tmp = (int4 *)(pbuf + w.scan_tmp), *segtot = tmp + (size_t)ns * plan.nblk;
            hipLaunchKernelGGL(bin_scan_seg_kernel, dim3(nseg, ns), dim3(kScanThreads), 0, st, subtot,
                               offsets, tmp, segtot, plan, part, fuse_a ? w.n_wg : 0);
            hipLaunchKernelGGL(bin_scan_emit_kernel, dim3(nseg, ns), dim3(kScanThreads), 0, st, offsets,
                               tmp, segtot, items, combos, n_items, plan);
        } else {
            hipLaunchKernelGGL(bin_scan_kernel, dim3(ns), dim3(kScanThreads), 0, st, subtot, offsets,
                               items, combos, n_items, plan, part, fuse_a ? w.n_wg : 0);
        }
    }
    if (stages & kBinFill) {
        if (wide && pt4) BOXATTN_BIN(true, true, 4);
        else if (wide) BOXATTN_BIN(true, true, 1);
        else BOXATTN_BIN(true, false, 1);
    }
#undef BOXATTN_BIN
}

inline bool dense_pointgrad_ok(const DensePlan *dp, const void *value, const void *loc, const void *attn,
                               const void *grad_out, const void *grad_loc, const void *grad_attn)
{
    return dp && aligned(value, 16) && aligned(grad_out, 16) && aligned(loc, 8) &&
           aligned(attn, 4) && aligned(grad_loc, 16) && aligned(grad_attn, 16);
}

template <typename ST, int G, bool INST>
void launch_pointgrad(const ST *value, const int64_t *shapes, const int64_t *lsi, const float *loc,
                      const float *w_sp, const float *w_lv, const ST *grad_out, const ST *grad_mask,
                      const Dims &d, float *grad_loc, float *grad_sp, float *grad_lv, hipStream_t st,
                      const BinRide *fill_ride, bool *ride_taken, const DensePlan *dp)
{
    if (ride_taken) *ride_taken = false;
    ScopedKernelTimer timer(g_prof.ev[kSlotBwdPoints], st);
    if constexpr (std::is_same<ST, bf16_t>::value && !INST) {
        if (dense_pointgrad_ok(dp, value, loc, w_sp, grad_out, grad_loc, grad_sp)) {
            launch_pointgrad_dense(value, loc, w_sp, grad_out, *dp, grad_loc, grad_sp,
                                   (unsigned)(d.n_value() * sizeof(bf16_t)), st, fill_ride ? *fill_ride : BinRide{});
            if (fill_ride && ride_taken) *ride_taken = true;
            return;
        }
    }
    if constexpr (std::is_same<ST, float>::value && !INST) {
        if (dense_pointgrad_ok(dp, value, loc, w_sp, grad_out, grad_loc, grad_sp)) {
            launch_pointgrad_dense_f32(value, loc, w_sp, grad_out, *dp, grad_loc, grad_sp,
                                       (unsigned)(d.n_value() * sizeof(float)), st, fill_ride ? *fill_ride : BinRide{});
            if (fill_ride && ride_taken) *ride_taken = true;
            return;
        }
    }
    const size_t n_qh = d.n_qh();
    const size_t vbytes = d.n_value() * sizeof(ST);
    GatherIdx ix{};
    if (vbytes < kOobOffset && gather_idx(d, ix, sizeof(ST))) {
        const GatherCfg cfg = gather_cfg<ST>(d, aligned(value, 16) && aligned(grad_out, 16) &&
                                                (!INST || aligned(grad_mask, 16)));
        const int blocks = gather_blocks(d, ix, kWave / cfg.G);
        const int tiles = (d.L * d.P + cfg.G - 1) / cfg.G;
        const bool wpp = INST && blocks < 1024 && tiles >= kWave / cfg.G;
        unsigned total = 0;
        if (wpp) {
            const int wblocks = ix.head_xcd ? 8 * ceil_div_sz((size_t)d.B * d.Lq, 4)
                                            : ceil_div_sz(n_qh, 4);
            const int split = point_split(wblocks, tiles / (kWave / cfg.G));
            const BinRide ride = place_riders(fill_ride, (unsigned)wblocks, &total);
#define BOXATTN_PG2W(GG, VV)                                                                         \
hipLaunchKernelGGL((pointgrad2_kernel<ST, GG, INST, GatherUnroll<ST, GG, VV>::value, VV, true>), \
                   dim3(total, split), dim3(256), 0, st, value, shapes, lsi, loc, w_sp, w_lv,    \
                   grad_out, grad_mask, d.S, d.H, d.L, d.Lq, d.P, grad_loc, grad_sp, grad_lv,    \
                   with_grid(ix, wblocks, split, tiles), (unsigned)vbytes, ride);
            BOXATTN_GATHER_DISPATCH(cfg, BOXATTN_PG2W);
#undef BOXATTN_PG2W
        } else {
            const int split = point_split(blocks, tiles);
            const BinRide ride = place_riders(fill_ride, (unsigned)blocks, &total);
            {
#define BOXATTN_PG2(GG, VV)                                                                   \
hipLaunchKernelGGL((pointgrad2_kernel<ST, GG, INST, GatherUnroll<ST, GG, VV>::value, VV>), \
                   dim3(total, split), dim3(256), 0, st, value, shapes, lsi, loc, w_sp,    \
                   w_lv, grad_out, grad_mask, d.S, d.H, d.L, d.Lq, d.P, grad_loc, grad_sp, \
                   grad_lv, with_grid(ix, blocks, split, tiles), (unsigned)vbytes, ride);
                BOXATTN_GATHER_DISPATCH(cfg, BOXATTN_PG2);
#undef BOXATTN_PG2
            }
        }
        if (fill_ride && ride_taken) *ride_taken = true;
    } else {
        const int blocks = ceil_div_sz(n_qh, (size_t)(kWave / G) * 4);
        hipLaunchKernelGGL((bwd_fast_kernel<ST, 4, G, INST, false>), dim3(blocks), dim3(256),
                           0, st, value, shapes, lsi, loc, w_sp, w_lv, grad_out, grad_mask,
                           d.S, d.H, d.L, d.Lq, d.P, (float *)nullptr, grad_loc, grad_sp, grad_lv,
                           n_qh);
    }
}

constexpr int kAccWgCap = 1024;
template <typename ST, int G, bool INST>
int launch_accumulate(AccKind acc, const ST *grad_out, const ST *grad_mask, const float *loc, const float *w_sp,
                      const float *w_lv, const Dims &d, const BinPlan &plan, const int *offsets, const int4 *items,
                      const int *n_items, const int *records, ST *grad_value, float *partials,
                      const ChunkCombine &cc, const ZeroRole &zr, hipStream_t st)
{
    constexpr int C = 4 * G;
    const int ns = d.B * d.H, ns8 = (ns + 7) / 8 * 8;
    const int wg_per_slice = std::min(kAccWgCap, std::max(1, plan.item_cap));
    ScopedKernelTimer timer(g_prof.ev[kSlotBwdAccum], st);
    if constexpr (std::is_same<ST, bf16_t>::value && !INST) {
        if (acc == kAccTr) {
            launch_accumulate_tr(C, grad_out, (size_t)d.B * d.Lq * d.H * C * sizeof(ST), plan, d.S, d.H, d.Lq, items,
                                 n_items, records, grad_value, partials, wg_per_slice, ns8, cc, zr, st);
            return finish();
        }
    }
    if constexpr (std::is_same<ST, float>::value && !INST && C == 32) {
        if (acc == kAccSplit) {
            launch_accumulate_split(grad_out, (size_t)d.B * d.Lq * d.H * C * sizeof(float), plan, d.S, d.H, d.Lq, items,
                                    n_items, records, grad_value, partials, wg_per_slice, ns8, cc, zr, st);
            return finish();
        }
        if (acc == kAccF32) {
            launch_accumulate_f32(grad_out, (size_t)d.B * d.Lq * d.H * C * sizeof(float), plan, d.S, d.H, d.Lq, items,
                                  n_items, records, grad_value, partials, wg_per_slice, ns8, cc, zr, st);
            return finish();
        }
    }
    if constexpr (std::is_same<ST, float>::value && INST && C == 32) {
        if (acc == kAccSplit) {
            launch_accumulate_split(grad_out, (size_t)d.B * d.Lq * d.H * C * sizeof(float), plan, d.S, d.H, d.Lq, items,
                                    n_items, records, grad_value, partials, wg_per_slice, ns8, cc, zr, st, grad_mask,
                                    (size_t)d.B * d.Lq * d.P * d.H * C * sizeof(float), w_lv, d.P);
            return finish();
        }
    }
    if (acc != kAccValu) return (int)hipErrorInvalidValue;
    hipLaunchKernelGGL((binned_accumulate_kernel<ST, C, INST, 1, false>), dim3(wg_per_slice + plan.zero_workers, ns8), dim3(64), 0, st,
                       grad_out, grad_mask, loc, w_sp, w_lv, plan, d.S, d.H, d.Lq, d.P, offsets, items, n_items,
                       records, grad_value, partials, cc, zr);
    return finish();
}

template <typename ST, int G, bool INST>
int run_binned(const ST *value, const int64_t *shapes, const int64_t *lsi, const float *loc,
               const float *w_sp, const float *w_lv, const ST *grad_out, const ST *grad_mask,
               const Dims &d, const BinPlan &plan, const PlanLayout &pl, char *pbuf, const ScratchLayout &sl,
               char *sbuf, ST *grad_value, float *grad_loc, float *grad_sp, float *grad_lv, bool plan_ready,
               hipStream_t st, const DensePlan *dp, const SpecRide *spec = nullptr,
               bool spec_warm = false, int *spec_tickets = nullptr)
{
    const int ns = d.B * d.H;
    const AccKind acc = acc_kind<ST, INST>(d);
    const int flavour = bin_flavour<ST, INST>(d, loc, w_sp);
    int *records = (int *)(sbuf + sl.records);
    float *partials = (float *)(sbuf + sl.partials);
    const int *n_items = (const int *)(pbuf + pl.n_items), *offsets = (const int *)(pbuf + pl.offsets);
    const int4 *items = (const int4 *)(pbuf + pl.items), *combos = (const int4 *)(pbuf + pl.combos);
    const bool one_pass = spec && spec_warm;
    if (!plan_ready && !one_pass) launch_binning(flavour, loc, w_sp, d, plan, pl, pbuf, records, st, kBinCount | kBinScan);
    bool filled = false;
    if (one_pass) {
        BinRide ride = make_ride(loc, w_sp, d, plan, pl, pbuf, &sl, sbuf, flavour | kRideSpec, true);
        ride.spec = *spec;
        ride.tickets = spec_tickets;
        launch_pointgrad<ST, G, INST>(value, shapes, lsi, loc, w_sp, w_lv, grad_out, grad_mask, d, grad_loc,
                                      grad_sp, grad_lv, st, &ride, &filled, dp);
        if (!filled)
            launch_binning(flavour, loc, w_sp, d, plan, pl, pbuf, records, st, kBinCount | kBinScan);
    } else if (riders_ok(plan, pl)) {
        const BinRide ride = make_ride(loc, w_sp, d, plan, pl, pbuf, &sl, sbuf, flavour, true);
        launch_pointgrad<ST, G, INST>(value, shapes, lsi, loc, w_sp, w_lv, grad_out, grad_mask, d, grad_loc,
                                      grad_sp, grad_lv, st, &ride, &filled, dp);
    } else {
        launch_pointgrad<ST, G, INST>(value, shapes, lsi, loc, w_sp, w_lv, grad_out, grad_mask, d, grad_loc,
                                      grad_sp, grad_lv, st, nullptr, nullptr, dp);
    }
    const bool small = (long long)d.Lq * d.L * d.P < 65536;
    const bool own_combine = opt(kOptRiders) == 1 || opt(kOptRiders) == 2 ||
                             (opt(kOptRiders) == 0 && !riders_ok(plan, pl) && !small);
    if (!filled)
        launch_binning(flavour, loc, w_sp, d, plan, pl, pbuf, records, st, kBinFill,
                       own_combine ? nullptr : (int *)(sbuf + sl.ctickets));
    ChunkCombine cc{};
    if (!own_combine) cc = ChunkCombine{(int *)(sbuf + sl.ctickets), combos, plan.nblk, plan.pslot_cap};
    ZeroRole zr{offsets, (const int2 *)(pbuf + pl.zgeo)};
    BinPlan plan_acc = plan;
    if (one_pass && filled) {
        zr = ZeroRole{nullptr, nullptr, spec->redo, loc, w_sp, d.P};
        plan_acc.zero_workers = kSpecRedoWorkers;
    }
    int rc = launch_accumulate<ST, G, INST>(acc, grad_out, grad_mask, loc, w_sp, w_lv, d, plan_acc, offsets, items,
                                            n_items, records, grad_value, partials, cc, zr, st);
    if (rc) return rc;
    if (spec && !(one_pass && filled))
        hipLaunchKernelGGL(spec_layout_kernel<256>, dim3(ns), dim3(256), 0, st, plan, offsets, spec->cursor, spec->cbase,
                           spec->redo);
    if (own_combine) {
        ScopedKernelTimer timer(g_prof.ev[kSlotBwdCombine], st);
        hipLaunchKernelGGL((combine_partials_kernel<ST, 4 * G>), dim3(64, ns), dim3(64), 0, st, combos,
                           n_items, partials, combine_plan(plan), d.S, d.H, grad_value);
    }
    return finish();
}

template <typename ST, bool INST>
int launch_bwd_ws(const ST *value, const int64_t *shapes, const int64_t *lsi, const float *loc,
                  const float *w_sp, const float *w_lv, const ST *grad_out, const ST *grad_mask,
                  const Dims &d, ST *grad_value, float *grad_loc, float *grad_sp, float *grad_lv,
                  const int64_t *shapes_host, const int64_t *lsi_host, void *workspace,
                  size_t workspace_bytes, const void *plan_buf, size_t plan_bytes, int hints, hipStream_t st,
                  void *state = nullptr, size_t state_bytes = 0)
{
    constexpr bool kBf16 = std::is_same<ST, bf16_t>::value;
    if (!d.valid()) return (int)hipErrorInvalidValue;
    BinPlan plan;
    const size_t nv = d.n_value();
    bool binned = (g_variant == 0 || g_variant == 3) && workspace && nv && d.n_qh() &&
                  make_plan(d, shapes_host, lsi_host, plan) &&
                  fast_ok<ST>(d, value, loc, grad_out,
                              INST ? (const void *)grad_mask : (const void *)grad_out, grad_loc) &&
                  aligned(workspace, 256) && aligned(grad_value, 16);
    PlanLayout pl{};
    ScratchLayout sl{};
    bool plan_ready = false;
    if (binned) {
        pl = plan_layout(d, plan);
        sl = scratch_layout(d, plan, wide_workspace(kBf16, d));
        plan_ready = plan_buf && plan_bytes >= pl.total && aligned(plan_buf, 256);
        binned = workspace_bytes >= (plan_ready ? sl.total : pl.total + sl.total);
    }
    if (!binned) {
        if (g_variant == 3) return (int)hipErrorInvalidValue;
        float *acc = nullptr;
        if constexpr (kBf16) {
            if (!workspace || workspace_bytes < nv * sizeof(float)) return (int)hipErrorInvalidValue;
            acc = (float *)workspace;
        } else {
            acc = grad_value;
        }
        return launch_bwd<ST, INST>(value, shapes, lsi, loc, w_sp, w_lv, grad_out, grad_mask, d,
                                    grad_value, grad_loc, grad_sp, grad_lv, acc, st);
    }
    if (!shapes || !lsi || !loc || !w_sp || !grad_out || !grad_loc || !grad_sp || !grad_value ||
        !value || (INST && (!w_lv || !grad_mask || !grad_lv)))
        return (int)hipErrorInvalidValue;
    char *ws = (char *)workspace;
    char *pbuf = plan_ready ? const_cast<char *>((const char *)plan_buf) : ws;
    char *sbuf = plan_ready ? ws : ws + pl.total;
    int rc = 0;
    DensePlan dense;
    const DensePlan *dp = !std::is_same<ST, double>::value && !INST && !(hints & BOXATTN_HINT_NOT_LOCAL) &&
                                  make_dense_plan(d, shapes_host, lsi_host, dense, (int)sizeof(ST)) ? &dense : nullptr;
    SpecRide spec{};
    const SpecRide *sp = nullptr;
    bool spec_warm = false;
    int *spec_tickets = nullptr;
    if (!plan_ready && spec_ok<ST, INST>(d, plan, pl)) {
        const StateLayout sy = state_layout(d, &plan);
        const int chk = state_check(state, state_bytes, sy, d, shapes_host, st, (hints & BOXATTN_HINT_FRESH_STATE) != 0);
        if (chk < 0) return (int)hipErrorInvalidValue;
        if (chk > 0) {
            char *sb = (char *)state;
            spec = SpecRide{(int *)(sb + sy.cursor), (int *)(sb + sy.cbase), (int2 *)(sb + sy.redo),
                            (unsigned long long *)(sb + sy.spec_stats)};
            sp = &spec;
            spec_warm = chk == 2;
            spec_tickets = (int *)(sb + sy.tickets);
            state_learned(state);
        }
    }
    switch (fast_group(d)) {
#define BOXATTN_BINNED_CASE(GG)                                                                 \
    case GG:                                                                                    \
        rc = run_binned<ST, GG, INST>(value, shapes, lsi, loc, w_sp, w_lv, grad_out, grad_mask, \
                                      d, plan, pl, pbuf, sl, sbuf, grad_value, grad_loc, grad_sp, grad_lv, \
                                      plan_ready, st, dp, sp, spec_warm, spec_tickets);     \
        break;
        BOXATTN_BINNED_CASE(4)
        BOXATTN_BINNED_CASE(8)
        BOXATTN_BINNED_CASE(16)
#undef BOXATTN_BINNED_CASE
    }
    return rc;
}

template <typename ST, bool INST>
int launch_fwd_train(const ST *value, const int64_t *shapes, const int64_t *lsi, const float *loc,
                     const float *w_sp, const float *w_lv, const Dims &d, ST *out, ST *mask,
                     const int64_t *shapes_host, const int64_t *lsi_host, void *plan_buf,
                     size_t plan_bytes, void *state, size_t state_bytes, int hints, int *plan_built,
                     hipStream_t st)
{
    if (plan_built) *plan_built = 0;
    const bool allow_dense = !(hints & BOXATTN_HINT_NOT_LOCAL);
    const size_t tbytes = (size_t)std::max(0, d.B) * (size_t)std::max(0, d.H) * kRideTickets * sizeof(int);
    BinPlan plan;
    const bool planned = d.valid() && make_plan(d, shapes_host, lsi_host, plan);
    const StateLayout sy = state_layout(d, planned ? &plan : nullptr);
    if (state_check(state, state_bytes, sy, d, shapes_host, st, (hints & BOXATTN_HINT_FRESH_STATE) != 0) < 0)
        return (int)hipErrorInvalidValue;
    const bool have_state = state != nullptr;
    unsigned long long *stats = have_state ? (unsigned long long *)state : nullptr;
    if (have_state && planned && d.n_value() && d.n_qh() && (g_variant == 0 || g_variant == 3) &&
        fast_ok<ST>(d, value, loc, out, INST ? (const void *)mask : (const void *)out, out) &&
        spec_ok<ST, INST>(d, plan, plan_layout(d, plan)))
        return launch_fwd<ST, INST>(value, shapes, lsi, loc, w_sp, w_lv, d, out, mask, st,
                                    shapes_host, lsi_host, nullptr, nullptr, allow_dense, stats);
    bool ok = (g_variant == 0 || g_variant == 3) && plan_buf && planned &&
              d.n_value() && d.n_qh() &&
              aligned(plan_buf, 256) &&
              fast_ok<ST>(d, value, loc, out, INST ? (const void *)mask : (const void *)out, out);
    PlanLayout pl{};
    if (ok) {
        pl = plan_layout(d, plan);
        ok = plan_bytes >= pl.total;
    }
    if (!ok)
        return launch_fwd<ST, INST>(value, shapes, lsi, loc, w_sp, w_lv, d, out, mask, st,
                                    shapes_host, lsi_host, nullptr, nullptr, allow_dense, stats);
    char *pbuf = (char *)plan_buf;
    const int flavour = bin_flavour<ST, INST>(d, loc, w_sp);
    bool taken = false;
    int rc = 0;
    if (riders_ok(plan, pl)) {
        BinRide ride = make_ride(loc, w_sp, d, plan, pl, pbuf, nullptr, nullptr, flavour, false);
        if (have_state) {
            ride.tickets = (int *)((char *)state + sy.tickets);
        } else {
            hipError_t e = zero_async(pbuf + pl.tickets, tbytes, st);
            if (e != hipSuccess) return (int)e;
        }
        rc = launch_fwd<ST, INST>(value, shapes, lsi, loc, w_sp, w_lv, d, out, mask, st, shapes_host, lsi_host,
                                  &ride, &taken, allow_dense, stats);
    } else {
        rc = launch_fwd<ST, INST>(value, shapes, lsi, loc, w_sp, w_lv, d, out, mask, st, shapes_host, lsi_host,
                                  nullptr, nullptr, allow_dense, stats);
    }
    if (rc) return rc;
    if (!taken)
        launch_binning(flavour, loc, w_sp, d, plan, pl, pbuf, nullptr, st, kBinCount | kBinScan);
    rc = finish();
    if (rc == 0 && plan_built) *plan_built = 1;
    return rc;
}

}


extern "C" {

#define DIMS Dims{B, S, H, C, L, Lq, P}
#define ST_ (hipStream_t) stream

int boxattn_fwd_train_f32(const float *value, const int64_t *shapes, const int64_t *lsi,
                          const float *loc, const float *attn, int B, int S, int H, int C, int L,
                          int Lq, int P, float *out, const int64_t *shapes_host,
                          const int64_t *lsi_host, void *plan, size_t plan_bytes, void *state,
                          size_t state_bytes, int hints, int *plan_built, void *stream)
{
    return launch_fwd_train<float, false>(value, shapes, lsi, loc, attn, nullptr, DIMS, out, nullptr,
                                          shapes_host, lsi_host, plan, plan_bytes, state, state_bytes, hints, plan_built, ST_);
}
int boxattn_fwd_train_bf16(const uint16_t *value, const int64_t *shapes, const int64_t *lsi,
                           const float *loc, const float *attn, int B, int S, int H, int C, int L,
                           int Lq, int P, uint16_t *out, const int64_t *shapes_host,
                           const int64_t *lsi_host, void *plan, size_t plan_bytes, void *state,
                           size_t state_bytes, int hints, int *plan_built, void *stream)
{
    return launch_fwd_train<bf16_t, false>(value, shapes, lsi, loc, attn, nullptr, DIMS, out, nullptr,
                                           shapes_host, lsi_host, plan, plan_bytes, state, state_bytes, hints, plan_built, ST_);
}
int instattn_fwd_train_f32(const float *value, const int64_t *shapes, const int64_t *lsi,
                           const float *loc, const float *spatial_w, const float *level_w, int B,
                           int S, int H, int C, int L, int Lq, int P, float *out, float *mask_out,
                           const int64_t *shapes_host, const int64_t *lsi_host, void *plan,
                           size_t plan_bytes, void *state, size_t state_bytes, int hints, int *plan_built, void *stream)
{
    return launch_fwd_train<float, true>(value, shapes, lsi, loc, spatial_w, level_w, DIMS, out, mask_out,
                                         shapes_host, lsi_host, plan, plan_bytes, state, state_bytes, hints, plan_built, ST_);
}
int instattn_fwd_train_bf16(const uint16_t *value, const int64_t *shapes, const int64_t *lsi,
                            const float *loc, const float *spatial_w, const float *level_w, int B,
                            int S, int H, int C, int L, int Lq, int P, uint16_t *out,
                            uint16_t *mask_out, const int64_t *shapes_host,
                            const int64_t *lsi_host, void *plan, size_t plan_bytes, void *state,
                            size_t state_bytes, int hints, int *plan_built, void *stream)
{
    return launch_fwd_train<bf16_t, true>(value, shapes, lsi, loc, spatial_w, level_w, DIMS, out, mask_out,
                                          shapes_host, lsi_host, plan, plan_bytes, state, state_bytes, hints, plan_built, ST_);
}

size_t boxattn_plan_bytes(int is_bf16, int B, int S, int H, int C, int L, int Lq, int P,
                          const int64_t *shapes_host, const int64_t *lsi_host)
{
    (void)is_bf16;
    const Dims d = DIMS;
    BinPlan plan;
    if (!d.valid() || !make_plan(d, shapes_host, lsi_host, plan)) return 0;
    return plan_layout(d, plan).total;
}

size_t boxattn_state_bytes(int B, int S, int H, int C, int L, int Lq, int P, const int64_t *shapes_host,
                           const int64_t *lsi_host)
{
    const Dims d = DIMS;
    BinPlan plan;
    const bool planned = d.valid() && make_plan(d, shapes_host, lsi_host, plan);
    return state_layout(d, planned ? &plan : nullptr).total;
}

size_t boxattn_bwd_workspace_bytes(int is_bf16, int B, int S, int H, int C, int L, int Lq, int P,
                                   const int64_t *shapes_host, const int64_t *lsi_host)
{
    const Dims d = DIMS;
    if (!d.valid()) return 0;
    const size_t fallback = is_bf16 ? align_up(d.n_value() * sizeof(float)) : 0;
    BinPlan plan;
    if (!make_plan(d, shapes_host, lsi_host, plan)) return fallback;
    return std::max(fallback, plan_layout(d, plan).total +
                                  scratch_layout(d, plan, wide_workspace(is_bf16 != 0, d)).total);
}

int boxattn_bwd_ws_f32(const float *value, const int64_t *shapes, const int64_t *lsi,
                       const float *loc, const float *attn, const float *grad_out, int B, int S,
                       int H, int C, int L, int Lq, int P, float *grad_value, float *grad_loc,
                       float *grad_attn, const int64_t *shapes_host, const int64_t *lsi_host,
                       void *workspace, size_t workspace_bytes, const void *plan, size_t plan_bytes, void *state,
        size_t state_bytes, int hints, void *stream)
{
    return launch_bwd_ws<float, false>(value, shapes, lsi, loc, attn, nullptr, grad_out, nullptr, DIMS,
                                       grad_value, grad_loc, grad_attn, nullptr, shapes_host, lsi_host,
                                       workspace, workspace_bytes, plan, plan_bytes, hints, ST_, state, state_bytes);
}
int boxattn_bwd_ws_bf16(const uint16_t *value, const int64_t *shapes, const int64_t *lsi,
                        const float *loc, const float *attn, const uint16_t *grad_out, int B,
                        int S, int H, int C, int L, int Lq, int P, uint16_t *grad_value,
                        float *grad_loc, float *grad_attn, const int64_t *shapes_host,
                        const int64_t *lsi_host, void *workspace, size_t workspace_bytes,
                        const void *plan, size_t plan_bytes, void *state,
        size_t state_bytes, int hints, void *stream)
{
    return launch_bwd_ws<bf16_t, false>(value, shapes, lsi, loc, attn, nullptr, grad_out, nullptr, DIMS,
                                        grad_value, grad_loc, grad_attn, nullptr, shapes_host, lsi_host,
                                        workspace, workspace_bytes, plan, plan_bytes, hints, ST_, state, state_bytes);
}
int instattn_bwd_ws_f32(const float *value, const int64_t *shapes, const int64_t *lsi,
                        const float *loc, const float *spatial_w, const float *level_w,
                        const float *grad_out, const float *grad_mask, int B, int S, int H, int C,
                        int L, int Lq, int P, float *grad_value, float *grad_loc,
                        float *grad_spatial_w, float *grad_level_w, const int64_t *shapes_host,
                        const int64_t *lsi_host, void *workspace, size_t workspace_bytes,
                        const void *plan, size_t plan_bytes, void *state,
        size_t state_bytes, int hints, void *stream)
{
    return launch_bwd_ws<float, true>(value, shapes, lsi, loc, spatial_w, level_w, grad_out, grad_mask, DIMS,
                                      grad_value, grad_loc, grad_spatial_w, grad_level_w, shapes_host,
                                      lsi_host, workspace, workspace_bytes, plan, plan_bytes, hints, ST_, state, state_bytes);
}
int instattn_bwd_ws_bf16(const uint16_t *value, const int64_t *shapes, const int64_t *lsi,
                         const float *loc, const float *spatial_w, const float *level_w,
                         const uint16_t *grad_out, const uint16_t *grad_mask, int B, int S, int H,
                         int C, int L, int Lq, int P, uint16_t *grad_value, float *grad_loc,
                         float *grad_spatial_w, float *grad_level_w, const int64_t *shapes_host,
                         const int64_t *lsi_host, void *workspace, size_t workspace_bytes,
                         const void *plan, size_t plan_bytes, void *state,
        size_t state_bytes, int hints, void *stream)
{
    return launch_bwd_ws<bf16_t, true>(value, shapes, lsi, loc, spatial_w, level_w, grad_out, grad_mask, DIMS,
                                       grad_value, grad_loc, grad_spatial_w, grad_level_w, shapes_host,
                                       lsi_host, workspace, workspace_bytes, plan, plan_bytes, hints, ST_, state, state_bytes);
}


int boxattn_abi_version(void) { return BOXATTN_ABI_VERSION; }

const char *boxattn_build_info(void)
{
    return "boxattn gfx950 (CDNA4, wave64) | hipcc " __VERSION__
           " | kernels: generic{f32,f64,bf16}, gather{f32 4ch/lane, bf16 8ch/lane} C={16,32,64}, "
           "window-staged encoder forward + point gradients{bf16 on MFMA 4x4x4, f32 on VALU}, "
           "binned-bwd{bf16 on MFMA 32x32x16, f32 on the same MFMA over exact three-term bf16 splits} "
           "with fill / combine riding in the point-gradient and accumulate launches, "
           "one-pass fill into guessed bin ranges (caller-owned state), box-grid{f32} | abi 8";
}

int boxattn_profile_begin(void)
{
    std::lock_guard<std::mutex> g(g_prof.mu);
    for (auto &v : g_prof.ev) drain(v, nullptr, nullptr);
    g_prof.on = true;
    return 0;
}

int boxattn_profile_end(double *ms_sum, int *launches)
{
    g_prof.on = false;
    std::lock_guard<std::mutex> g(g_prof.mu);
    for (int i = 0; i < kNumSlots; ++i)
        drain(g_prof.ev[i], ms_sum ? ms_sum + i : nullptr, launches ? launches + i : nullptr);
    return 0;
}

std::atomic<int> g_epoch{0};
int boxattn_options_epoch(void) { return g_epoch.load(std::memory_order_relaxed); }

int boxattn_set_variant(int variant)
{
    g_epoch.fetch_add(1, std::memory_order_relaxed);
    return g_variant.exchange(variant);
}

void boxattn_set_debug_buffer(float *p) { g_dense_dbg.store(p); }

int boxattn_set_option(int key, int value)
{
    if (key < 0 || key >= kNumOpts || !opt_live(key)) return -1;
    g_epoch.fetch_add(1, std::memory_order_relaxed);
    return g_opt[key].exchange(value);
}


int boxattn_fwd_f32(const float *value, const int64_t *shapes, const int64_t *lsi,
                    const float *loc, const float *attn, int B, int S, int H, int C, int L,
                    int Lq, int P, float *out, void *stream)
{
    return launch_fwd<float, false>(value, shapes, lsi, loc, attn, nullptr, DIMS, out, nullptr,
                                    ST_);
}
int boxattn_fwd_f64(const double *value, const int64_t *shapes, const int64_t *lsi,
                    const double *loc, const double *attn, int B, int S, int H, int C, int L,
                    int Lq, int P, double *out, void *stream)
{
    return launch_fwd<double, false>(value, shapes, lsi, loc, attn, nullptr, DIMS, out,
                                     nullptr, ST_);
}
int boxattn_fwd_bf16(const uint16_t *value, const int64_t *shapes, const int64_t *lsi,
                     const float *loc, const float *attn, int B, int S, int H, int C, int L,
                     int Lq, int P, uint16_t *out, void *stream)
{
    return launch_fwd<bf16_t, false>(value, shapes, lsi, loc, attn, nullptr, DIMS, out,
                                     nullptr, ST_);
}

int boxattn_fwd_hl_f32(const float *value, const int64_t *shapes, const int64_t *lsi,
                       const float *loc, const float *attn, int B, int S, int H, int C, int L,
                       int Lq, int P, float *out, const int64_t *shapes_host,
                       const int64_t *lsi_host, void *stream)
{
    return launch_fwd<float, false>(value, shapes, lsi, loc, attn, nullptr, DIMS, out, nullptr,
                                    ST_, shapes_host, lsi_host);
}
int boxattn_fwd_hl_bf16(const uint16_t *value, const int64_t *shapes, const int64_t *lsi,
                        const float *loc, const float *attn, int B, int S, int H, int C, int L,
                        int Lq, int P, uint16_t *out, const int64_t *shapes_host,
                        const int64_t *lsi_host, void *stream)
{
    return launch_fwd<bf16_t, false>(value, shapes, lsi, loc, attn, nullptr, DIMS, out, nullptr,
                                     ST_, shapes_host, lsi_host);
}

int boxattn_bwd_f32(const float *value, const int64_t *shapes, const int64_t *lsi,
                    const float *loc, const float *attn, const float *grad_out, int B, int S,
                    int H, int C, int L, int Lq, int P, float *grad_value, float *grad_loc,
                    float *grad_attn, void *stream)
{
    return launch_bwd<float, false>(value, shapes, lsi, loc, attn, nullptr, grad_out, nullptr,
                                    DIMS, grad_value, grad_loc, grad_attn, nullptr, grad_value,
                                    ST_);
}
int boxattn_bwd_f64(const double *value, const int64_t *shapes, const int64_t *lsi,
                    const double *loc, const double *attn, const double *grad_out, int B,
                    int S, int H, int C, int L, int Lq, int P, double *grad_value,
                    double *grad_loc, double *grad_attn, void *stream)
{
    return launch_bwd<double, false>(value, shapes, lsi, loc, attn, nullptr, grad_out, nullptr,
                                     DIMS, grad_value, grad_loc, grad_attn, nullptr,
                                     grad_value, ST_);
}
int boxattn_bwd_bf16(const uint16_t *value, const int64_t *shapes, const int64_t *lsi,
                     const float *loc, const float *attn, const uint16_t *grad_out, int B,
                     int S, int H, int C, int L, int Lq, int P, uint16_t *grad_value,
                     float *grad_loc, float *grad_attn, float *grad_value_ws, void *stream)
{
    return launch_bwd<bf16_t, false>(value, shapes, lsi, loc, attn, nullptr, grad_out, nullptr,
                                     DIMS, grad_value, grad_loc, grad_attn, nullptr,
                                     grad_value_ws, ST_);
}

int instattn_fwd_f32(const float *value, const int64_t *shapes, const int64_t *lsi,
                     const float *loc, const float *spatial_w, const float *level_w, int B,
                     int S, int H, int C, int L, int Lq, int P, float *out, float *mask_out,
                     void *stream)
{
    return launch_fwd<float, true>(value, shapes, lsi, loc, spatial_w, level_w, DIMS, out,
                                   mask_out, ST_);
}
int instattn_fwd_f64(const double *value, const int64_t *shapes, const int64_t *lsi,
                     const double *loc, const double *spatial_w, const double *level_w, int B,
                     int S, int H, int C, int L, int Lq, int P, double *out, double *mask_out,
                     void *stream)
{
    return launch_fwd<double, true>(value, shapes, lsi, loc, spatial_w, level_w, DIMS, out,
                                    mask_out, ST_);
}
int instattn_fwd_bf16(const uint16_t *value, const int64_t *shapes, const int64_t *lsi,
                      const float *loc, const float *spatial_w, const float *level_w, int B,
                      int S, int H, int C, int L, int Lq, int P, uint16_t *out,
                      uint16_t *mask_out, void *stream)
{
    return launch_fwd<bf16_t, true>(value, shapes, lsi, loc, spatial_w, level_w, DIMS, out,
                                    mask_out, ST_);
}

int instattn_bwd_f32(const float *value, const int64_t *shapes, const int64_t *lsi,
                     const float *loc, const float *spatial_w, const float *level_w,
                     const float *grad_out, const float *grad_mask, int B, int S, int H, int C,
                     int L, int Lq, int P, float *grad_value, float *grad_loc,
                     float *grad_spatial_w, float *grad_level_w, void *stream)
{
    return launch_bwd<float, true>(value, shapes, lsi, loc, spatial_w, level_w, grad_out,
                                   grad_mask, DIMS, grad_value, grad_loc, grad_spatial_w,
                                   grad_level_w, grad_value, ST_);
}
int instattn_bwd_f64(const double *value, const int64_t *shapes, const int64_t *lsi,
                     const double *loc, const double *spatial_w, const double *level_w,
                     const double *grad_out, const double *grad_mask, int B, int S, int H,
                     int C, int L, int Lq, int P, double *grad_value, double *grad_loc,
                     double *grad_spatial_w, double *grad_level_w, void *stream)
{
    return launch_bwd<double, true>(value, shapes, lsi, loc, spatial_w, level_w, grad_out,
                                    grad_mask, DIMS, grad_value, grad_loc, grad_spatial_w,
                                    grad_level_w, grad_value, ST_);
}
int instattn_bwd_bf16(const uint16_t *value, const int64_t *shapes, const int64_t *lsi,
                      const float *loc, const float *spatial_w, const float *level_w,
                      const uint16_t *grad_out, const uint16_t *grad_mask, int B, int S, int H,
                      int C, int L, int Lq, int P, uint16_t *grad_value, float *grad_loc,
                      float *grad_spatial_w, float *grad_level_w, float *grad_value_ws,
                      void *stream)
{
    return launch_bwd<bf16_t, true>(value, shapes, lsi, loc, spatial_w, level_w, grad_out,
                                    grad_mask, DIMS, grad_value, grad_loc, grad_spatial_w,
                                    grad_level_w, grad_value_ws, ST_);
}


}
```

boxer_amd/csrc/boxattn_dense.hip:

```cpp
#include "boxattn_dense.h"
#include "boxattn_binned_tr.h"
#include "boxattn_dense_fwd.h"
#include "boxattn_dense_f32.h"

namespace boxattn {

static BinRide place_riders(BinRide ride, unsigned own_blocks, unsigned *total)
{
    ride.grid = ride_grid(ride.grid.n_riders, own_blocks, ride.grid.shift, total);
    return ride;
}

void launch_pointgrad_dense(const uint16_t *value, const float *loc, const float *attn,
                            const uint16_t *grad_out, const DensePlan &dp, float *grad_loc,
                            float *grad_attn, unsigned value_bytes, hipStream_t st, const BinRide &ride_in)
{
    unsigned total = 0;
    const BinRide ride = place_riders(ride_in, dense_blocks(dp), &total);
#define BOXATTN_DENSE_PG(LV_)                                                                           \
    case LV_:                                                                                           \
        hipLaunchKernelGGL((pointgrad_dense_kernel<LV_>), dim3(total), dim3(256), 0, st, value, loc, attn, \
                           grad_out, grad_loc, grad_attn, dp, value_bytes, ride);                      \
        break;
    switch (dp.L) {
        BOXATTN_DENSE_PG(1) BOXATTN_DENSE_PG(2) BOXATTN_DENSE_PG(3) BOXATTN_DENSE_PG(4)
    }
#undef BOXATTN_DENSE_PG
}

void launch_fwd_dense(const uint16_t *value, const float *loc, const float *attn, uint16_t *out,
                      const DensePlan &dp, unsigned value_bytes, const BinRide &ride_in,
                      unsigned long long *stats, hipStream_t st)
{
    unsigned total = 0;
    const BinRide ride = place_riders(ride_in, dense_blocks(dp), &total);
#define BOXATTN_DENSE_FWD(LV_)                                                                       \
    case LV_:                                                                                        \
        hipLaunchKernelGGL((fwd_dense_kernel<LV_>), dim3(total), dim3(256), 0, st, value, loc, attn, out, \
                           dp, value_bytes, ride, stats);                                            \
        break;
    switch (dp.L) {
        BOXATTN_DENSE_FWD(1) BOXATTN_DENSE_FWD(2) BOXATTN_DENSE_FWD(3) BOXATTN_DENSE_FWD(4)
    }
#undef BOXATTN_DENSE_FWD
}

void launch_pointgrad_dense_f32(const float *value, const float *loc, const float *attn, const float *grad_out,
                                const DensePlan &dp, float *grad_loc, float *grad_attn, unsigned value_bytes,
                                hipStream_t st, const BinRide &ride_in)
{
    unsigned total = 0;
    const BinRide ride = place_riders(ride_in, dense_blocks(dp), &total);
#define BOXATTN_DENSE_PG32(LV_)                                                                         \
    case LV_:                                                                                           \
        hipLaunchKernelGGL((pointgrad_dense_f32_kernel<LV_>), dim3(total), dim3(256), 0, st, value, loc, attn, \
                           grad_out, grad_loc, grad_attn, dp, value_bytes, ride);                      \
        break;
    switch (dp.L) {
        BOXATTN_DENSE_PG32(1) BOXATTN_DENSE_PG32(2) BOXATTN_DENSE_PG32(3) BOXATTN_DENSE_PG32(4)
    }
#undef BOXATTN_DENSE_PG32
}

void launch_fwd_dense_f32(const float *value, const float *loc, const float *attn, float *out, const DensePlan &dp,
                          unsigned value_bytes, const BinRide &ride_in, unsigned long long *stats, hipStream_t st)
{
    unsigned total = 0;
    const BinRide ride = place_riders(ride_in, dense_blocks(dp), &total);
#define BOXATTN_DENSE_FWD32(LV_)                                                                     \
    case LV_:                                                                                        \
        hipLaunchKernelGGL((fwd_dense_f32_kernel<LV_>), dim3(total), dim3(256), 0, st, value, loc, attn, out, \
                           dp, value_bytes, ride, stats);                                            \
        break;
    switch (dp.L) {
        BOXATTN_DENSE_FWD32(1) BOXATTN_DENSE_FWD32(2) BOXATTN_DENSE_FWD32(3) BOXATTN_DENSE_FWD32(4)
    }
#undef BOXATTN_DENSE_FWD32
}

void launch_accumulate_tr(int C, const uint16_t *grad_out, size_t grad_out_bytes, const BinPlan &plan, int S,
                          int H, int Lq, const int4 *items, const int *n_items, const int *records,
                          uint16_t *grad_value, float *partials, int wg_per_slice, int ns8, const ChunkCombine &cc,
                          const ZeroRole &zr, hipStream_t st)
{
#define BOXATTN_ACC_TR(C_)                                                                              \
    hipLaunchKernelGGL((binned_accumulate_tr_kernel<uint16_t, C_>), dim3(wg_per_slice + plan.zero_workers, ns8), dim3(64), 0, st, \
                       grad_out, (unsigned)grad_out_bytes, plan, S, H, Lq, items, n_items, records,     \
                       grad_value, partials, cc, zr)
    switch (C) {
    case 16: BOXATTN_ACC_TR(16); break;
    case 32: BOXATTN_ACC_TR(32); break;
    case 64: BOXATTN_ACC_TR(64); break;
    }
#undef BOXATTN_ACC_TR
}

void launch_accumulate_split(const float *grad_out, size_t grad_out_bytes, const BinPlan &plan, int S, int H, int Lq,
                             const int4 *items, const int *n_items, const int *records, float *grad_value,
                             float *partials, int wg_per_slice, int ns8, const ChunkCombine &cc, const ZeroRole &zr,
                             hipStream_t st, const float *grad_mask, size_t grad_mask_bytes, const float *w_lv, int P)
{
    const InstRows inst{grad_mask, (unsigned)grad_mask_bytes, w_lv, P};
    if (grad_mask)
        hipLaunchKernelGGL((binned_accumulate_split_kernel<32, true>), dim3(wg_per_slice + plan.zero_workers, ns8), dim3(64), 0, st,
                           grad_out, (unsigned)grad_out_bytes, plan, S, H, Lq, items, n_items, records, grad_value, partials, cc,
                           zr, inst);
    else
        hipLaunchKernelGGL((binned_accumulate_split_kernel<32, false>), dim3(wg_per_slice + plan.zero_workers, ns8), dim3(64), 0, st,
                           grad_out, (unsigned)grad_out_bytes, plan, S, H, Lq, items, n_items, records, grad_value, partials, cc,
                           zr, inst);
}

void launch_accumulate_f32(const float *grad_out, size_t grad_out_bytes, const BinPlan &plan, int S, int H, int Lq,
                           const int4 *items, const int *n_items, const int *records, float *grad_value,
                           float *partials, int wg_per_slice, int ns8, const ChunkCombine &cc, const ZeroRole &zr,
                           hipStream_t st)
{
    hipLaunchKernelGGL((binned_accumulate_f32_kernel<32>), dim3(wg_per_slice + plan.zero_workers, ns8), dim3(64), 0, st, grad_out,
                       (unsigned)grad_out_bytes, plan, S, H, Lq, items, n_items, records, grad_value, partials, cc, zr);
}

}
```

boxer_amd/csrc/boxattn_dense_plan.h:

```cpp
#pragma once
#include <hip/hip_runtime.h>
#include <stdint.h>
#include "boxattn_combine.h"
#include "boxattn_binplan.h"
#include "boxattn_binpass.h"
#include "boxattn_scan_tail.h"

namespace boxattn {

constexpr int kDenseMaxLevels = 4;
constexpr int kDenseTile = 8;
constexpr int kDenseSub = 4;
constexpr int kDenseWinMax = 16;
constexpr int kDenseSlotBytes = 64;
constexpr int kDenseRowSkew = 16;
#ifndef BOXATTN_DENSE_LDS
#define BOXATTN_DENSE_LDS 28160
#endif
constexpr int kDenseLdsBytes = BOXATTN_DENSE_LDS;
constexpr int kDenseZeroOff = kDenseLdsBytes - kDenseSlotBytes;
constexpr int kDenseStatSlots = 64;

struct DenseLevel {
    int H, W, start;
    int ntx, ntiles;
    unsigned n_all;
    unsigned mag_ntx, mag_ntiles;
};
struct DenseWin {
    int ax, bx, ay, by;
    unsigned geo;
};
inline int dense_win_pitch16(int cols) { return (cols * kDenseSlotBytes + kDenseRowSkew) / 16; }
inline unsigned dense_win_pack(int rows, int cols, int off16)
{
    return (unsigned)rows | ((unsigned)cols << 5) | ((unsigned)dense_win_pitch16(cols) << 10) | ((unsigned)off16 << 17);
}
struct DensePlan {
    int L, B, Lq, S, H;
    unsigned mag_h;
    DenseLevel lv[kDenseMaxLevels];
    DenseWin win[kDenseMaxLevels][kDenseMaxLevels];
    float *dbg;
};

inline unsigned dense_blocks(const DensePlan &p)
{
    unsigned longest = 0;
    for (unsigned x = 0; x < 8; ++x) {
        unsigned n_x = 0;
        for (int l = 0; l < p.L; ++l) {
            const unsigned n = (unsigned)p.B * (unsigned)p.lv[l].ntiles;
            n_x += (((x + 1) * n) >> 3) - ((x * n) >> 3);
        }
        longest = longest > n_x ? longest : n_x;
    }
    return 8u * (unsigned)p.H * longest;
}

void launch_pointgrad_dense(const uint16_t *value, const float *loc, const float *attn,
                            const uint16_t *grad_out, const DensePlan &dp, float *grad_loc,
                            float *grad_attn, unsigned value_bytes, hipStream_t st, const BinRide &ride);

void launch_fwd_dense(const uint16_t *value, const float *loc, const float *attn, uint16_t *out,
                      const DensePlan &dp, unsigned value_bytes, const BinRide &ride,
                      unsigned long long *stats, hipStream_t st);

void launch_pointgrad_dense_f32(const float *value, const float *loc, const float *attn, const float *grad_out,
                                const DensePlan &dp, float *grad_loc, float *grad_attn, unsigned value_bytes,
                                hipStream_t st, const BinRide &ride);
void launch_fwd_dense_f32(const float *value, const float *loc, const float *attn, float *out, const DensePlan &dp,
                          unsigned value_bytes, const BinRide &ride, unsigned long long *stats, hipStream_t st);
#ifndef BOXATTN_DENSE_F32_LDS
#define BOXATTN_DENSE_F32_LDS 53248
#endif

constexpr size_t kAccTrMaxBytes = (size_t)1 << 31;
void launch_accumulate_tr(int C, const uint16_t *grad_out, size_t grad_out_bytes, const BinPlan &plan, int S,
                          int H, int Lq, const int4 *items, const int *n_items, const int *records,
                          uint16_t *grad_value, float *partials, int wg_per_slice, int ns8, const ChunkCombine &cc,
                          const ZeroRole &zr, hipStream_t st);

void launch_accumulate_split(const float *grad_out, size_t grad_out_bytes, const BinPlan &plan, int S, int H, int Lq,
                             const int4 *items, const int *n_items, const int *records, float *grad_value,
                             float *partials, int wg_per_slice, int ns8, const ChunkCombine &cc, const ZeroRole &zr,
                             hipStream_t st, const float *grad_mask = nullptr, size_t grad_mask_bytes = 0,
                             const float *w_lv = nullptr, int P = 1);

void launch_accumulate_f32(const float *grad_out, size_t grad_out_bytes, const BinPlan &plan, int S, int H, int Lq,
                           const int4 *items, const int *n_items, const int *records, float *grad_value,
                           float *partials, int wg_per_slice, int ns8, const ChunkCombine &cc, const ZeroRole &zr,
                           hipStream_t st);

}
```

boxer_amd/csrc/boxattn_host_plan.h:

```cpp
#pragma once

constexpr int kChunk = 1024, kChunkBig = 1536;
inline int bin_chunk(const Dims &d)
{
    const int forced = opt(kOptBinChunk);
    if (forced > 0) return std::min(4096, std::max(64, (forced + 63) / 64 * 64));
    const long long rec_est = 3ll * d.Lq * d.L * d.P / 2;
    const long long c = (rec_est / 256 + 63) / 64 * 64;
    return c >= kChunk ? kChunkBig : (int)std::max<long long>(128, c);
}

enum AccKind { kAccValu = 0, kAccTr = 1, kAccF32 = 2, kAccSplit = 3 };
inline bool accumulate_tr_ok(const Dims &d)
{
    return (d.C == 16 || d.C == 32 || d.C == 64) && (size_t)d.B * d.Lq * d.H * d.C * 2 < kAccTrMaxBytes &&
           d.Lq < (1 << 24) && d.H * d.C * 2 < (1 << 24);
}
inline bool f32_matrix_shape_ok(const Dims &d)
{
    return d.C == 32 && (size_t)d.B * d.Lq * d.H * 32 * 4 < kAccTrMaxBytes && d.Lq < (1 << 24) && d.H * 128 < (1 << 24);
}
inline bool f32_mfma_ok(const Dims &d) { return opt(kOptAccF32) == 2 && f32_matrix_shape_ok(d); }
constexpr size_t kInstSplitMinPoints = 65536;
inline bool f32_split_ok(const Dims &d) { return opt(kOptAccF32) == 0 && f32_matrix_shape_ok(d); }
template <typename ST, bool INST> inline AccKind acc_kind(const Dims &d)
{
    if constexpr (!INST && std::is_same<ST, bf16_t>::value) {
        if (accumulate_tr_ok(d)) return kAccTr;
    }
    if constexpr (!INST && std::is_same<ST, float>::value) {
        if (f32_mfma_ok(d)) return kAccF32;
        if (f32_split_ok(d)) return kAccSplit;
    }
    if constexpr (INST && std::is_same<ST, float>::value) {
        if (f32_split_ok(d) && (size_t)d.Lq * d.L * d.P >= kInstSplitMinPoints &&
            (size_t)d.B * d.Lq * d.P * d.H * 32 * 4 < kAccTrMaxBytes)
            return kAccSplit;
    }
    return kAccValu;
}
inline bool wide_workspace(bool is_bf16, const Dims &d)
{
    return is_bf16 ? accumulate_tr_ok(d) : f32_mfma_ok(d) || f32_split_ok(d);
}
constexpr int kMaxBlocks = 8192;

inline size_t align_up(size_t x, size_t a = 256) { return (x + a - 1) / a * a; }

inline bool make_plan_blocks(const Dims &d, const int64_t *sh, const int64_t *ls, BinPlan &p)
{
    constexpr int BW = 8, BH = 4;
    p.L = d.L;
    long long blk0 = 0, next_start = 0;
    for (int l = 0; l < d.L; ++l) {
        const long long hl = sh[2 * l], wl = sh[2 * l + 1], st = ls[l];
        if (hl < 0 || wl < 0 || hl > INT32_MAX || wl > INT32_MAX || st != next_start ||
            st + hl * wl > d.S)
            return false;
        next_start = st + hl * wl;
        p.lv[l].H = (int)hl;
        p.lv[l].W = (int)wl;
        p.lv[l].start = (int)st;
        p.lv[l].nbx = (int)((wl + BW - 1) / BW);
        p.lv[l].nby = (int)((hl + BH - 1) / BH);
        if ((unsigned long long)wl * wl * p.lv[l].nbx >= (1ull << 32) ||
            (unsigned long long)hl * hl * p.lv[l].nby >= (1ull << 32))
            return false;
        p.lv[l].mw = wl > 1 ? (unsigned)((1ull << 32) / (unsigned long long)wl + 1) : 0u;
        p.lv[l].mh = hl > 1 ? (unsigned)((1ull << 32) / (unsigned long long)hl + 1) : 0u;
        const auto nb_magic = [](long long nmax, int nb) -> unsigned {
            if (nb <= 1 || nmax >= (1ll << 24)) return 0u;
            static std::mutex mu;
            static std::map<std::pair<long long, int>, unsigned> known;
            std::lock_guard<std::mutex> g(mu);
            const auto it = known.find({nmax, nb});
            if (it != known.end()) return it->second;
            unsigned m = (unsigned)((1ull << 32) / (unsigned long long)nb + 1);
            for (long long n = 0; n <= nmax && m; ++n)
                if ((unsigned)(((unsigned long long)n * m) >> 32) != (unsigned)(n / nb)) m = 0u;
            known[{nmax, nb}] = m;
            return m;
        };
        p.lv[l].mnx = nb_magic(std::max<long long>((long long)p.lv[l].nbx * p.lv[l].nby, (long long)p.lv[l].nbx * wl + p.lv[l].nbx), p.lv[l].nbx);
        p.lv[l].mny = nb_magic((long long)p.lv[l].nby * hl + p.lv[l].nby, p.lv[l].nby);
        p.lv[l].blk0 = (int)blk0;
        blk0 += (long long)p.lv[l].nbx * p.lv[l].nby;
    }
    if (next_start != d.S) return false;
    const long long rec_cap = 4ll * d.Lq * d.L * d.P;
    if (blk0 == 0 || blk0 > kMaxBlocks || rec_cap > INT32_MAX / 2 ||
        (long long)d.B * d.Lq * d.H > INT32_MAX || (long long)d.B * d.Lq * d.P * d.H > INT32_MAX)
        return false;
    int lp_bits = 0;
    while ((1ll << lp_bits) < (long long)d.L * d.P) ++lp_bits;
    if (((long long)d.Lq << lp_bits) > INT32_MAX) return false;
    if ((long long)d.L * d.P > (1 << 16)) return false;
    p.lp_bits = lp_bits;
    p.n_slices = d.B * d.H;
    p.nblk = (int)blk0;
    p.rec_cap = (int)rec_cap;
    p.chunk = bin_chunk(d);
    p.item_cap = (int)(blk0 + rec_cap / p.chunk + 1);
    p.min_items = blk0 > kScanThreads && 3ll * d.Lq * d.L * d.P / 2 < 2 * blk0 ? 0 : 1;
    p.zero_workers = p.min_items ? 0 : (int)((blk0 + kZeroPer - 1) / kZeroPer);
    p.pslot_cap = (int)std::min<long long>(2 * (rec_cap / p.chunk) + 2, blk0 + rec_cap / p.chunk + 1);
    if (p.pslot_cap >= (1 << kItemSlotBits) || blk0 >= (1 << (31 - kItemSlotBits))) return false;
    return true;
}

inline bool make_plan(const Dims &d, const int64_t *sh, const int64_t *ls, BinPlan &p)
{
    if (!sh || !ls || !d.valid() || fast_group(d) == 0 || d.L > kMaxBinLevels) return false;
    return make_plan_blocks(d, sh, ls, p);
}

std::atomic<float *> g_dense_dbg{nullptr};

struct PlanLayout {
    size_t n_items, part, tickets, subtot, offsets, items, combos, scan_tmp, zgeo, total;
    int q_per_wg, n_wg;
};
struct ScratchLayout { size_t records, partials, ctickets, total; };

constexpr long long kSpecMinRecordsPerBlock = 192;
inline bool spec_shape(const Dims &d, const BinPlan &p)
{
    const int o = opt(kOptRiders);
    return (o == 0 || o == 2 || o == 3) && p.nblk <= kSpecMaxBlocks && p.min_items == 1 &&
           3ll * d.Lq * d.L * d.P / 2 >= kSpecMinRecordsPerBlock * p.nblk;
}

inline PlanLayout plan_layout(const Dims &d, const BinPlan &p)
{
    const size_t ns = (size_t)d.B * d.H;
    PlanLayout w;
    const long long wg_target = bin_wg_target(spec_shape(d, p), (long long)d.Lq * (long long)ns);
    w.q_per_wg = std::max(8, (int)(((long long)d.Lq * (long long)ns + wg_target - 1) / wg_target));
    w.q_per_wg = std::max(w.q_per_wg, (d.Lq + kScanSub * kScanWgPerSub - 1) /
                                          (kScanSub * kScanWgPerSub));
    const long long lp = (long long)d.L * d.P;
    w.q_per_wg = (int)std::max<long long>(w.q_per_wg, (4ll * p.nblk + lp - 1) / lp);
    w.n_wg = (d.Lq + w.q_per_wg - 1) / w.q_per_wg;
    size_t o = 0;
    w.n_items = o; o += align_up(ns * 2 * 4);
    w.tickets = o; o += align_up(ns * kRideTickets * 4);
    w.part = o;    o += align_up(ns * (size_t)w.n_wg * (size_t)p.nblk * 4);
    w.subtot = o;  o += align_up(ns * kScanSub * (size_t)p.nblk * 4);
    w.offsets = o; o += align_up(ns * (p.nblk + 1) * 4);
    w.items = o;   o += align_up(ns * p.item_cap * 16);
    w.combos = o;  o += align_up(ns * (size_t)p.nblk * 16);
    w.scan_tmp = o;
    if (p.nblk > kScanThreads) o += align_up(ns * ((size_t)p.nblk + kMaxBlocks / kScanThreads) * 16);
    w.zgeo = o;
    if (p.zero_workers > 0) o += align_up((size_t)p.nblk * 8);
    w.total = o;
    return w;
}
inline ScratchLayout scratch_layout(const Dims &d, const BinPlan &p, bool wide)
{
    const size_t ns = (size_t)d.B * d.H;
    ScratchLayout w;
    size_t o = 0;
    w.ctickets = o; o += align_up(ns * (size_t)p.nblk * 4);
    w.records = o;  o += align_up(ns * (size_t)p.rec_cap * (wide ? 16 : 4));
    w.partials = o; o += align_up(ns * (size_t)p.pslot_cap * 32 * d.C * 4);
    w.total = o;
    return w;
}

constexpr size_t kStatBytes = (size_t)kDenseStatSlots * 2 * sizeof(unsigned long long);

inline bool riders_ok(const BinPlan &plan, const PlanLayout &w)
{
    return opt(kOptRiders) != 1 && plan.nblk <= kRideMaxBlocks && plan.min_items == 1 &&
           w.n_wg <= kScanSub * kScanWgPerSub;
}

template <typename ST, bool INST> inline bool spec_ok(const Dims &d, const BinPlan &plan, const PlanLayout &pl)
{
    if (INST || std::is_same<ST, double>::value) return false;
    return spec_shape(d, plan) && acc_kind<ST, INST>(d) != kAccValu && riders_ok(plan, pl) &&
           (long long)d.Lq * d.P < (1 << 24) && plan.rec_cap < (1 << 28) &&
           d.n_qh() * (size_t)d.L * (size_t)d.P < ((size_t)1 << 29);
}

struct StateLayout { size_t spec_stats, tickets, cursor, cbase, redo, total; };
inline StateLayout state_layout(const Dims &d, const BinPlan *plan)
{
    const size_t ns = (size_t)std::max(0, d.B) * (size_t)std::max(0, d.H);
    StateLayout w;
    size_t o = kStatBytes;
    w.spec_stats = o; o += 64;
    w.tickets = o;    o += align_up(ns * kRideTickets * sizeof(int));
    w.cursor = w.cbase = w.redo = o;
    if (plan && plan->nblk <= kSpecMaxBlocks) {
        w.cursor = o; o += align_up(ns * (size_t)plan->nblk * sizeof(int));
        w.cbase = o;  o += align_up(ns * ((size_t)plan->nblk + 1) * sizeof(int));
        w.redo = o;   o += align_up(ns * ((size_t)plan->nblk + 1) * sizeof(int2));
    }
    w.total = o;
    return w;
}

struct StateShadow { Dims d; unsigned long long geo; bool learned; };
std::mutex g_state_mu;
std::map<const void *, StateShadow> g_state_shadow;
inline bool same_dims(const Dims &a, const Dims &b)
{
    return a.B == b.B && a.S == b.S && a.H == b.H && a.C == b.C && a.L == b.L && a.Lq == b.Lq && a.P == b.P;
}
inline int state_check(void *state, size_t bytes, const StateLayout &sy, const Dims &d, const int64_t *sh, hipStream_t st,
                       bool fresh = false)
{
    if (!state) return 0;
    if (!aligned(state, 8) || bytes < sy.total) return -1;
    unsigned long long geo = 1469598103934665603ull;
    for (int i = 0; sh && i < 2 * d.L; ++i) geo = (geo ^ (unsigned long long)sh[i]) * 1099511628211ull;
    std::lock_guard<std::mutex> g(g_state_mu);
    if (fresh) g_state_shadow.erase(state);
    const auto it = g_state_shadow.find(state);
    if (it == g_state_shadow.end()) {
        if (g_state_shadow.size() >= 4096) g_state_shadow.clear();
        g_state_shadow[state] = StateShadow{d, geo, false};
        return 1;
    }
    if (same_dims(it->second.d, d) && it->second.geo == geo) return it->second.learned ? 2 : 1;
    if (zero_async((char *)state + kStatBytes, bytes - kStatBytes, st) != hipSuccess) return -1;
    it->second = StateShadow{d, geo, false};
    return 1;
}
inline void state_learned(const void *state)
{
    std::lock_guard<std::mutex> g(g_state_mu);
    const auto it = g_state_shadow.find(state);
    if (it != g_state_shadow.end()) it->second.learned = true;
}

inline bool make_dense_plan(const Dims &d, const int64_t *sh, const int64_t *ls, DensePlan &p, int elem)
{
    if (!sh || !ls || !d.valid() || opt(kOptDense) == 1 || g_variant == 1 || g_variant == 2) return false;
    if (d.Lq != d.S || d.C != 32 || d.P != 4 || d.L > kDenseMaxLevels || d.B < 1 || d.S < 1) return false;
    if ((size_t)d.B * d.Lq * d.H * d.L * d.P >= (1ull << 31)) return false;
    if (d.n_value() * (size_t)elem >= kOobOffset) return false;
    const int unit = 8 * elem;
    const int budget = elem == 2 ? kDenseZeroOff : BOXATTN_DENSE_F32_LDS - 128;
    p = DensePlan{};
    p.dbg = g_dense_dbg.load();
    p.L = d.L; p.B = d.B; p.Lq = d.Lq; p.S = d.S; p.H = d.H;
    const auto magic = [](int dd) { return dd == 1 ? 0xFFFFFFFFu : (unsigned)((1ull << 32) / (unsigned)dd); };
    p.mag_h = magic(d.H);
    long long next = 0;
    for (int l = 0; l < d.L; ++l) {
        const long long hl = sh[2 * l], wl = sh[2 * l + 1];
        if (hl <= 0 || wl <= 0 || hl > 32000 || wl > 32000 || ls[l] != next) return false;
        next += hl * wl;
        DenseLevel &v = p.lv[l];
        v.H = (int)hl; v.W = (int)wl; v.start = (int)ls[l];
        v.ntx = (int)((wl + kDenseTile - 1) / kDenseTile);
        v.ntiles = v.ntx * (int)((hl + kDenseTile - 1) / kDenseTile);
        if ((long long)v.ntiles * d.B * d.H >= (1 << 24)) return false;
        v.n_all = (unsigned)(v.ntiles * d.B);
        v.mag_ntx = magic(v.ntx);
        v.mag_ntiles = magic(v.ntiles);
    }
    if (next != d.S) return false;
    constexpr float ref4 = 4.0f / 4.0f;
    constexpr float jit = 2.5f;
    for (int lq = 0; lq < d.L; ++lq) {
        int used = 0;
        for (int k = 0; k < d.L; ++k) {
            const int l = k == 0 ? lq : (d.L - k <= lq ? d.L - k - 1 : d.L - k);
            DenseWin &w = p.win[lq][l];
            const float rx = (float)p.lv[l].W / (float)p.lv[lq].W, ry = (float)p.lv[l].H / (float)p.lv[lq].H;
            const float mx = rx * ref4 * (1.0f + jit), my = ry * ref4 * (1.0f + jit);
            const int cols = (int)std::ceil(rx * (kDenseTile - 1) + 2 * mx) + 2;
            const int rows = (int)std::ceil(ry * (kDenseTile - 1) + 2 * my) + 2;
            w.ax = (int)std::lround(kDenseTile * rx * 65536.0f); w.bx = (int)std::floor((0.5f * rx - 0.5f - mx) * 65536.0f);
            w.ay = (int)std::lround(kDenseTile * ry * 65536.0f); w.by = (int)std::floor((0.5f * ry - 0.5f - my) * 65536.0f);
            if (rx > 8.0f || ry > 8.0f) { w.ax = w.ay = 0; }
            const int need = rows * dense_win_pitch16(cols);
            const bool fits = cols <= kDenseWinMax && rows <= kDenseWinMax && unit * (used + need) <= budget;
            w.geo = dense_win_pack(fits ? rows : 0, fits ? cols : 0, used);
            if (fits) used += need;
        }
    }
    return true;
}
```

boxer_amd/csrc/boxattn_spec.h:

```cpp
#pragma once
#include "boxattn_binpass.h"

namespace boxattn {

constexpr int kSpecDump = 256;
constexpr int kSpecMaxBlocks = kRideMaxBlocks / 2 - kSpecDump - 1;
constexpr int kSpecRedoWorkers = 64;
constexpr int kSpecRankBits = 16;
static_assert(kSpecMaxBlocks < (1 << 12), "block index bits of a packed candidate");

__device__ __forceinline__ void lds_barrier()
{
    asm volatile("s_waitcnt lgkmcnt(0)\n\ts_barrier" ::: "memory");
}

__device__ __forceinline__ int spec_want(int c, int cap_old)
{
    return (max(2 * c + 64, cap_old - (cap_old >> 2)) + 3) & ~3;
}

#ifndef BOXATTN_TUNE_SPEC_U
#define BOXATTN_TUNE_SPEC_U 1
#endif
template <int THREADS, int PT>
__device__ __forceinline__ void spec_fill_body(int *hist, int *base, BinLevel *s_lv, const float *__restrict__ loc,
                                               const float *__restrict__ w_sp, const BinPlan &plan, int H, int Lq,
                                               int P, int q_per_wg, int *__restrict__ cursor_s,
                                               const int *__restrict__ cbase_s, int *__restrict__ records, int s, int wg,
                                               unsigned long long *trace = nullptr)
{
    static_assert(PT == 1 || PT == 4, "points per thread and group");
    constexpr int U = PT == 4 ? BOXATTN_TUNE_SPEC_U : 4;
    constexpr int STRIDE = THREADS * U;
    static_assert(STRIDE * PT * 4 < (1 << kSpecRankBits), "ranks of a step");
    const int b = s / H, h = s % H;
    const int LP = plan.L * P;
    const int q0 = wg * q_per_wg;
    const int n_q = max(0, min(q0 + q_per_wg, Lq) - q0);
    const unsigned pid0 = (unsigned)(((b * Lq + q0) * H + h) * LP);
    const unsigned qstride = (unsigned)(H * LP);
    const int LPG = LP / PT, n_grp = n_q * LPG;
    const float rcp_lpg = 1.0f / (float)LPG, rcp_p = 1.0f / (float)P;
    int4 *rec = reinterpret_cast<int4 *>(records) + (size_t)s * plan.rec_cap;
    struct Step {
        float2 xy[U][PT];
        float wv[U][PT];
        int lp0[U], ql[U];
    };
    auto load_step = [&](Step &t, int g0) {
#pragma unroll
        for (int u = 0; u < U; ++u) {
            const int g = min(g0 + u * THREADS, n_grp - 1);
            int lg;
            divmod_small(g, LPG, rcp_lpg, t.ql[u], lg);
            t.lp0[u] = lg * PT;
            const unsigned pbase = pid0 + (unsigned)t.ql[u] * qstride + (unsigned)t.lp0[u];
            const char *lp8 = reinterpret_cast<const char *>(loc) + (pbase << 3);
            const char *wp4 = reinterpret_cast<const char *>(w_sp) + (pbase << 2);
            if constexpr (PT == 4) {
                const float4 a = *reinterpret_cast<const float4 *>(lp8), c = *reinterpret_cast<const float4 *>(lp8 + 16);
                t.xy[u][0] = make_float2(a.x, a.y); t.xy[u][1] = make_float2(a.z, a.w);
                t.xy[u][2] = make_float2(c.x, c.y); t.xy[u][3] = make_float2(c.z, c.w);
                const float4 w4 = *reinterpret_cast<const float4 *>(wp4);
                t.wv[u][0] = w4.x; t.wv[u][1] = w4.y; t.wv[u][2] = w4.z; t.wv[u][3] = w4.w;
            } else {
                t.xy[u][0] = *reinterpret_cast<const float2 *>(lp8);
                t.wv[u][0] = *reinterpret_cast<const float *>(wp4);
            }
        }
    };
    constexpr unsigned kIn = 1u << 12, kCc = 1u << 13, kCr = 1u << 14;
    unsigned long long ph[4] = {0, 0, 0, 0};
#define SPEC_PHASE(i_, t0_)                                                                            \
    do {                                                                                             \
        if (BOXATTN_RIDE_TRACE) {                                                                    \
            __builtin_amdgcn_sched_barrier(0);                                                       \
            const unsigned long long now_ = __builtin_amdgcn_s_memrealtime();                        \
            ph[i_] += now_ - t0_;                                                                    \
            t0_ = now_;                                                                              \
        }                                                                                            \
    } while (0)
    auto work_step = [&](const Step &t, int g0) {
        unsigned meta[U][PT], rk01[U][PT], rk23[U][PT];
        int nbx_u[U];
        unsigned long long tph = BOXATTN_RIDE_TRACE ? __builtin_amdgcn_s_memrealtime() : 0ull;
#pragma unroll
        for (int u = 0; u < U; ++u) {
            const bool have = g0 + u * THREADS < n_grp;
            const BinLevel lv = s_lv[(int)(((float)t.lp0[u] + 0.5f) * rcp_p)];
            nbx_u[u] = lv.nbx;
            const float Hf = (float)lv.H, Wf = (float)lv.W;
            int b0[PT];
            bool in[PT], cc[PT], cr[PT];
#pragma unroll
            for (int k = 0; k < PT; ++k) {
                float h_im, w_im;
                {
#pragma clang fp contract(off)
                    h_im = t.xy[u][k].y * Hf - 0.5f;
                    w_im = t.xy[u][k].x * Wf - 0.5f;
                }
                in[k] = have & (h_im > -1.f) & (w_im > -1.f) & (h_im < Hf) & (w_im < Wf) & (lv.H > 0) & (lv.W > 0);
                const int y0 = (int)floorf(in[k] ? h_im : 0.f), x0 = (int)floorf(in[k] ? w_im : 0.f);
                const int ty = __mul24(max(y0, 0), lv.nby), tx = __mul24(max(x0, 0), lv.nbx);
                const int ra = (int)__umulhi((unsigned)ty, lv.mh), ca = (int)__umulhi((unsigned)tx, lv.mw);
                b0[k] = lv.blk0 + ra * lv.nbx + ca;
                cr[k] = in[k] & ((unsigned)y0 < (unsigned)(lv.H - 1)) & (ty - __mul24(ra, lv.H) + lv.nby >= lv.H);
                cc[k] = in[k] & ((unsigned)x0 < (unsigned)(lv.W - 1)) & (tx - __mul24(ca, lv.W) + lv.nbx >= lv.W);
            }
            unsigned r[PT][4];
            const int dump = kSpecMaxBlocks + 1 + (int)threadIdx.x;
#pragma unroll
            for (int k = 0; k < PT; ++k) {
                r[k][0] = (unsigned)atomicAdd(&hist[in[k] ? b0[k] : dump], 1);
                r[k][1] = (unsigned)atomicAdd(&hist[cc[k] ? b0[k] + 1 : dump], 1);
                r[k][2] = (unsigned)atomicAdd(&hist[cr[k] ? b0[k] + lv.nbx : dump], 1);
                r[k][3] = (unsigned)atomicAdd(&hist[cc[k] & cr[k] ? b0[k] + lv.nbx + 1 : dump], 1);
            }
#pragma unroll
            for (int k = 0; k < PT; ++k) {
                meta[u][k] = (in[k] ? (unsigned)b0[k] | kIn : 0u) | (cc[k] ? kCc : 0u) | (cr[k] ? kCr : 0u);
                rk01[u][k] = (r[k][0] & 0xFFFFu) | (r[k][1] << 16);
                rk23[u][k] = (r[k][2] & 0xFFFFu) | (r[k][3] << 16);
            }
        }
        SPEC_PHASE(0, tph);
        lds_barrier();
        constexpr int KB = 2;
        for (int k0 = (int)threadIdx.x; k0 < plan.nblk; k0 += KB * THREADS) {
            int c[KB], old[KB], end[KB];
#pragma unroll
            for (int i = 0; i < KB; ++i) {
                const int bk = k0 + i * THREADS;
                c[i] = bk < plan.nblk ? hist[bk] : 0;
                old[i] = end[i] = 0;
            }
#pragma unroll
            for (int i = 0; i < KB; ++i)
                if (c[i] > 0) {
                    const unsigned bo = (unsigned)(k0 + i * THREADS) << 2;
                    old[i] = __hip_atomic_fetch_add(reinterpret_cast<int *>(reinterpret_cast<char *>(cursor_s) + bo), c[i],
                                                    __ATOMIC_RELAXED, __HIP_MEMORY_SCOPE_AGENT);
                    end[i] = *reinterpret_cast<const int *>(reinterpret_cast<const char *>(cbase_s) + bo + 4u);
                }
#pragma unroll
            for (int i = 0; i < KB; ++i)
                if (c[i] > 0) {
                    const int bk = k0 + i * THREADS;
                    hist[bk] = 0;
                    base[bk] = old[i] + c[i] <= end[i] ? old[i] : -1;
                }
        }
        SPEC_PHASE(1, tph);
        lds_barrier();
        SPEC_PHASE(2, tph);
#pragma unroll
        for (int u = 0; u < U; ++u) {
            const int idq = (q0 + t.ql[u]) << plan.lp_bits;
            int sb[PT][4];
#pragma unroll
            for (int k = 0; k < PT; ++k) {
                const int b0 = (int)(meta[u][k] & 0xFFFu);
                sb[k][0] = base[b0]; sb[k][1] = base[b0 + 1];
                sb[k][2] = base[b0 + nbx_u[u]]; sb[k][3] = base[b0 + nbx_u[u] + 1];
            }
            char *rb8 = reinterpret_cast<char *>(rec);
#pragma unroll
            for (int k = 0; k < PT; ++k) {
                const unsigned m = meta[u][k];
                const int4 r = make_int4(idq | (t.lp0[u] + k), __float_as_int(t.xy[u][k].x),
                                         __float_as_int(t.xy[u][k].y), __float_as_int(t.wv[u][k]));
                if ((m & kIn) && sb[k][0] >= 0)
                    *reinterpret_cast<int4 *>(rb8 + ((unsigned)(sb[k][0] + (int)(rk01[u][k] & 0xFFFFu)) << 4)) = r;
                if ((m & kCc) && sb[k][1] >= 0)
                    *reinterpret_cast<int4 *>(rb8 + ((unsigned)(sb[k][1] + (int)(rk01[u][k] >> 16)) << 4)) = r;
                if ((m & kCr) && sb[k][2] >= 0)
                    *reinterpret_cast<int4 *>(rb8 + ((unsigned)(sb[k][2] + (int)(rk23[u][k] & 0xFFFFu)) << 4)) = r;
                if ((m & kCc) && (m & kCr) && sb[k][3] >= 0)
                    *reinterpret_cast<int4 *>(rb8 + ((unsigned)(sb[k][3] + (int)(rk23[u][k] >> 16)) << 4)) = r;
            }
        }
        SPEC_PHASE(3, tph);
    };
#ifndef BOXATTN_TUNE_SPEC_PREFETCH
#define BOXATTN_TUNE_SPEC_PREFETCH 1
#endif
    Step sa;
    if (n_grp > 0) load_step(sa, (int)threadIdx.x);
    if (threadIdx.x == 0) {
#pragma unroll
        for (int k = 0; k < kMaxBinLevels; ++k) s_lv[k] = plan.lv[k];
    }
    for (int k = threadIdx.x; k < plan.nblk; k += THREADS) hist[k] = 0;
    __syncthreads();
    if constexpr (BOXATTN_TUNE_SPEC_PREFETCH != 0) {
        Step sb;
        for (int start = 0; start < n_grp; start += 2 * STRIDE) {
            const int g0 = start + (int)threadIdx.x;
            if (start + STRIDE < n_grp) load_step(sb, g0 + STRIDE);
            work_step(sa, g0);
            if (start + STRIDE >= n_grp) break;
            if (start + 2 * STRIDE < n_grp) load_step(sa, g0 + 2 * STRIDE);
            work_step(sb, g0 + STRIDE);
        }
    } else {
        for (int start = 0; start < n_grp; start += STRIDE) {
            const int g0 = start + (int)threadIdx.x;
            work_step(sa, g0);
            if (start + STRIDE < n_grp) load_step(sa, g0 + STRIDE);
        }
    }
#undef SPEC_PHASE
    if (BOXATTN_RIDE_TRACE && trace && threadIdx.x == 0)
        for (int i = 0; i < 4; ++i) trace[i] = ph[i];
}

template <int THREADS>
__device__ __forceinline__ void spec_chain_body(const ScanOut o, const BinPlan &plan, const BinLevel *lv_lds, int s,
                                                int *wsum, int *cnt, int *cbl, int *__restrict__ cursor_s,
                                                int *__restrict__ cbase_s, int2 *__restrict__ redo_s,
                                                unsigned long long *__restrict__ stats)
{
    constexpr int NW = THREADS / 64;
    const int tid = threadIdx.x, lane = tid & 63, wv = tid >> 6;
    const int nblk = plan.nblk;
    __syncthreads();
    for (int k = tid; k <= nblk; k += THREADS) {
        const int cb = cbase_s[k];
        cbl[k] = cb;
        if (k < nblk) cnt[k] = agent_load(cursor_s + k) - cb;
    }
    __syncthreads();
    const int per = (nblk + THREADS - 1) / THREADS;
    const int k_lo = min(tid * per, nblk), k_hi = min(k_lo + per, nblk);
    int sumA[4] = {0, 0, 0, 0}, sumB[4] = {0, 0, 0, 0};
    for (int k = k_lo; k < k_hi; ++k) {
        const int c = cnt[k], cap = cbl[k + 1] - cbl[k];
        const bool over = c > cap;
        const int nch = over ? 0 : max(1, (c + plan.chunk - 1) / plan.chunk);
        sumA[0] += spec_want(c, cap); sumA[1] += nch; sumA[2] += nch > 1 ? nch : 0; sumA[3] += nch > 1 ? 1 : 0;
        sumB[0] += over ? 1 : 0; sumB[1] += (c + 3) & ~3;
    }
    auto scan4 = [&](const int (&sum)[4], int (&run)[4], int (&tot)[4]) {
#pragma unroll
        for (int i = 0; i < 4; ++i) {
            int x = sum[i];
#pragma unroll
            for (int d = 1; d < 64; d <<= 1) {
                const int y = __shfl_up(x, d, 64);
                if (lane >= d) x += y;
            }
            run[i] = x - sum[i];
            if (lane == 63) wsum[i * NW + wv] = x;
        }
        __syncthreads();
#pragma unroll
        for (int i = 0; i < 4; ++i) {
            int pre = 0, all = 0;
#pragma unroll
            for (int w = 0; w < NW; ++w) {
                pre += w < wv ? wsum[i * NW + w] : 0;
                all += wsum[i * NW + w];
            }
            run[i] += pre;
            tot[i] = all;
        }
        __syncthreads();
    };
    int runA[4], totA[4], runB[4], totB[4];
    scan4(sumA, runA, totA);
    scan4(sumB, runB, totB);
    const bool roomy = totA[0] <= plan.rec_cap;
    const int share = roomy ? 0 : max(0, (int)((float)max(0, plan.rec_cap - totB[1]) / (float)max(nblk, 1)) - 4) & ~3;
    int next = roomy ? runA[0] : runB[1] + k_lo * share;
    int n_over = runB[0];
    for (int k = k_lo; k < k_hi; ++k) {
        const int c = cnt[k], cap = cbl[k + 1] - cbl[k];
        const bool over = c > cap;
        const int nch = over ? 0 : max(1, (c + plan.chunk - 1) / plan.chunk);
        int level = 0;
        for (int l = 1; l < plan.L; ++l)
            if (k >= lv_lds[l].blk0) level = l;
        const BinLevel lv = lv_lds[level];
        const int geo = (int)pack_block_geo(lv, level, k);
        const int csz = chunk_records(c, nch);
        for (int jj = 0; jj < nch; ++jj)
            o.items[(size_t)s * plan.item_cap + (totA[1] - 1 - (runA[1] + jj))] =
                make_int4(geo, cbl[k] + jj * csz, cbl[k] + min(c, (jj + 1) * csz),
                          nch > 1 ? (runA[2] + jj) | (runA[3] << kItemSlotBits) : -1);
        if (nch > 1) o.combos[(size_t)s * nblk + runA[3]] = make_int4(geo, runA[2], nch, 0);
        if (over) redo_s[1 + n_over++] = make_int2(k, geo);
        runA[1] += nch; runA[2] += nch > 1 ? nch : 0; runA[3] += nch > 1 ? 1 : 0;
        const int first = min(next, plan.rec_cap);
        cbase_s[k] = first;
        cursor_s[k] = first;
        next += roomy ? spec_want(c, cap) : ((c + 3) & ~3) + share;
    }
    if (k_hi == nblk && k_lo < nblk) cbase_s[nblk] = min(next, plan.rec_cap);
    if (tid == 0) {
        o.n_items[2 * s] = totA[1];
        o.n_items[2 * s + 1] = totA[3];
        redo_s[0] = make_int2(totB[0], 0);
        if (stats) {
            atomicAdd(stats, 1ull);
            if (totB[0]) atomicAdd(stats + 1, (unsigned long long)totB[0]);
        }
    }
}

template <int THREADS>
__global__ __launch_bounds__(THREADS) void spec_layout_kernel(BinPlan plan, const int *__restrict__ offsets,
                                                          int *__restrict__ cursor, int *__restrict__ cbase,
                                                          int2 *__restrict__ redo)
{
    static_assert(THREADS == 256, "4 wave sums per quantity");
    __shared__ int wsum[2 * 4];
    const int s = blockIdx.x, tid = threadIdx.x, lane = tid & 63, wv = tid >> 6;
    const int nblk = plan.nblk;
    const int *off = offsets + (size_t)s * (nblk + 1);
    int *cursor_s = cursor + (size_t)s * nblk, *cbase_s = cbase + (size_t)s * (nblk + 1);
    const int per = (nblk + 255) / 256;
    const int k_lo = min(tid * per, nblk), k_hi = min(k_lo + per, nblk);
    int sum[2] = {0, 0};
    for (int k = k_lo; k < k_hi; ++k) {
        const int c = off[k + 1] - off[k];
        sum[0] += spec_want(c, 0);
        sum[1] += (c + 3) & ~3;
    }
    int run[2], tot[2];
#pragma unroll
    for (int i = 0; i < 2; ++i) {
        int x = sum[i];
#pragma unroll
        for (int d = 1; d < 64; d <<= 1) {
            const int y = __shfl_up(x, d, 64);
            if (lane >= d) x += y;
        }
        run[i] = x - sum[i];
        if (lane == 63) wsum[i * 4 + wv] = x;
    }
    __syncthreads();
#pragma unroll
    for (int i = 0; i < 2; ++i) {
        int pre = 0, all = 0;
#pragma unroll
        for (int w = 0; w < 4; ++w) {
            pre += w < wv ? wsum[i * 4 + w] : 0;
            all += wsum[i * 4 + w];
        }
        run[i] += pre;
        tot[i] = all;
    }
    const bool roomy = tot[0] <= plan.rec_cap;
    const int share = roomy ? 0 : max(0, (int)((float)max(0, plan.rec_cap - tot[1]) / (float)max(nblk, 1)) - 4) & ~3;
    int next = roomy ? run[0] : run[1] + k_lo * share;
    for (int k = k_lo; k < k_hi; ++k) {
        const int c = off[k + 1] - off[k];
        const int first = min(next, plan.rec_cap);
        cbase_s[k] = first;
        cursor_s[k] = first;
        next += roomy ? spec_want(c, 0) : ((c + 3) & ~3) + share;
    }
    if (k_hi == nblk && k_lo < nblk) cbase_s[nblk] = min(next, plan.rec_cap);
    if (tid == 0) redo[(size_t)s * (nblk + 1)] = make_int2(0, 0);
}

template <int THREADS>
__device__ __forceinline__ void bin_fill_spec_ride(const BinRide r, unsigned id, int *lds)
{
    static_assert(THREADS == 256, "4 wave sums per scan quantity");
    const RideLds m(lds);
    int *hist = m.hist, *base = m.hist + kRideMaxBlocks / 2;
    const BinPlan plan = r.plan;
    unsigned s_u, wg_u;
    divmod_magic(id, (unsigned)r.n_wg, r.nwg_magic, s_u, wg_u);
    const int s = (int)s_u, wg = (int)wg_u;
    if (wg == 0 && r.ctickets)
        for (int k = threadIdx.x; k < plan.nblk; k += THREADS) r.ctickets[(size_t)s * plan.nblk + k] = 0;
    int *cursor_s = r.spec.cursor + (size_t)s * plan.nblk;
    int *cbase_s = r.spec.cbase + (size_t)s * (plan.nblk + 1);
    RIDE_STAMP(5);
    unsigned long long *tr = BOXATTN_RIDE_TRACE && r.trace ? r.trace + (size_t)id * 8 : nullptr;
    if (r.flavour & kRidePt4)
        spec_fill_body<THREADS, 4>(hist, base, m.lv, r.loc, r.w_sp, plan, r.H, r.Lq, r.P, r.q_per_wg, cursor_s, cbase_s,
                                   r.records, s, wg, tr);
    else
        spec_fill_body<THREADS, 1>(hist, base, m.lv, r.loc, r.w_sp, plan, r.H, r.Lq, r.P, r.q_per_wg, cursor_s, cbase_s,
                                   r.records, s, wg, tr);
    RIDE_STAMP(6);
    if (!last_arriver<THREADS>(r.tickets + (size_t)s * kRideTickets + kScanSub, r.n_wg, m.flag)) return;
    const ScanOut o{r.subtot, r.offsets, r.items, r.combos, r.n_items};
    spec_chain_body<THREADS>(o, plan, m.lv, s, m.wsum, hist, base, cursor_s, cbase_s,
                             r.spec.redo + (size_t)s * (plan.nblk + 1), r.spec.stats);
    RIDE_STAMP(7);
}

template <typename ST, int C>
__device__ __forceinline__ void redo_blocks(const ZeroRole zr, const BinPlan &plan, int s, int zw, int n_zw, int S, int H,
                                            int Lq, const ST *__restrict__ grad_out, ST *__restrict__ grad_value, int lane)
{
    constexpr int BW = 8, CH = C / 2, EPL = 16 / (int)sizeof(ST);
    const int2 *redo_s = zr.redo + (size_t)s * (plan.nblk + 1);
    const int n = redo_s[0].x;
    if (zw >= n) return;
    const int b = s / H, h = s % H, P = zr.P, LP = plan.L * P;
    const float2 *loc2 = reinterpret_cast<const float2 *>(zr.loc);
    const int mypix = lane >> 1, half = lane & 1;
    const int np = Lq * P;
    const float rcp_p = 1.0f / (float)P;
    for (int i = zw; i < n; i += n_zw) {
        const BlockGeo bg = unpack_block_geo((unsigned)redo_s[1 + i].y);
        int lvH = plan.lv[0].H, lvW = plan.lv[0].W, lv_start = plan.lv[0].start;
#pragma unroll
        for (int k = 1; k < kMaxBinLevels; ++k)
            if (k == bg.level) { lvH = plan.lv[k].H; lvW = plan.lv[k].W; lv_start = plan.lv[k].start; }
        const float Hf = (float)lvH, Wf = (float)lvW;
        const int Y = bg.oy + mypix / BW, X = bg.ox + mypix % BW;
        const bool live = mypix / BW < bg.bh && mypix % BW < bg.bw;
        float acc[CH];
#pragma unroll
        for (int c = 0; c < CH; ++c) acc[c] = 0.f;
        for (int i0 = 0; i0 < np; i0 += 64) {
            const bool have = i0 + lane < np;
            int q, p;
            divmod_small(have ? i0 + lane : 0, P, rcp_p, q, p);
            const size_t pid = (((size_t)b * Lq + q) * H + h) * LP + (size_t)bg.level * P + p;
            const float2 xy = loc2[pid];
            float h_im, w_im;
            {
#pragma clang fp contract(off)
                h_im = xy.y * Hf - 0.5f;
                w_im = xy.x * Wf - 0.5f;
            }
            const bool inside = h_im > -1.f && w_im > -1.f && h_im < Hf && w_im < Wf;
            const int y0 = (int)floorf(inside ? h_im : 0.f), x0 = (int)floorf(inside ? w_im : 0.f);
            const bool hit = have && inside && y0 + 1 >= bg.oy && y0 < bg.oy + bg.bh && x0 + 1 >= bg.ox && x0 < bg.ox + bg.bw;
            const float a = hit ? zr.w_sp[pid] : 0.f;
            unsigned long long mask = __builtin_amdgcn_ballot_w64(hit);
            while (mask) {
                const int j = (int)__builtin_ctzll(mask);
                mask &= mask - 1;
                const float hj = __builtin_bit_cast(float, __builtin_amdgcn_readlane(__builtin_bit_cast(int, h_im), j));
                const float wj = __builtin_bit_cast(float, __builtin_amdgcn_readlane(__builtin_bit_cast(int, w_im), j));
                const float aj = __builtin_bit_cast(float, __builtin_amdgcn_readlane(__builtin_bit_cast(int, a), j));
                const int qj = __builtin_amdgcn_readlane(q, j);
                const float yf = floorf(hj), xf = floorf(wj);
                const float lh = hj - yf, lw = wj - xf, hh = 1.f - lh, hw = 1.f - lw;
                const int yj = (int)yf, xj = (int)xf;
                const bool corner = (Y == yj || Y == yj + 1) && (X == xj || X == xj + 1);
                const float w = (Y == yj ? hh : lh) * (X == xj ? hw : lw) * aj;
                const ST *g = grad_out + (((size_t)b * Lq + qj) * H + h) * C + half * CH;
#pragma unroll
                for (int c = 0; c < CH; c += EPL) {
                    float t[EPL];
                    VecIO<ST, EPL>::ld(g + c, t);
                    if (corner) {
#pragma unroll
                        for (int e = 0; e < EPL; ++e) acc[c + e] = fmaf(w, t[e], acc[c + e]);
                    }
                }
            }
        }
        if (live) {
            ST *dst = grad_value + (((size_t)b * S + lv_start + (size_t)Y * lvW + X) * H + h) * C + half * CH;
#pragma unroll
            for (int c = 0; c < CH; c += EPL) {
                float t[EPL];
#pragma unroll
                for (int e = 0; e < EPL; ++e) t[e] = acc[c + e];
                VecIO<ST, EPL>::st(dst + c, t);
            }
        }
    }
}

}
```

Measured before the change: 25.50 Gsample-points/s.

## Bin point quads as compact 4-byte records and accumulate via fp32 LDS atomics

```diff
diff --git a/boxer_amd/csrc/boxattn_binned.h b/boxer_amd/csrc/boxattn_binned.h
--- a/boxer_amd/csrc/boxattn_binned.h
+++ b/boxer_amd/csrc/boxattn_binned.h
@@ -13,7 +13,7 @@
 #define BOXATTN_TUNE_BIN_THREADS 512
 #endif
 constexpr int kBinThreads = BOXATTN_TUNE_BIN_THREADS;
-template <int BW, int BH, bool FILL, bool WIDE, int PT>
+template <int BW, int BH, bool FILL, bool WIDE, int PT, bool QUAD = false>
 __global__ __launch_bounds__(kBinThreads) void bin_kernel(const float *__restrict__ loc,
                                                   const float *__restrict__ w_sp, BinPlan plan,
                                                   int H, int Lq, int P, int q_per_wg, int n_wg, int interleave,
@@ -27,7 +27,7 @@
     extern __shared__ int sh_bins[];
     __shared__ BinLevel s_lv[kMaxBinLevels];
     const int s = blockIdx.y, wg = blockIdx.x;
-    bin_pass_body<kBinThreads, BW, BH, FILL, WIDE, PT>(sh_bins, s_lv, loc, w_sp, plan, H, Lq, P, q_per_wg, n_wg,
+    bin_pass_body<kBinThreads, BW, BH, FILL, WIDE, PT, QUAD>(sh_bins, s_lv, loc, w_sp, plan, H, Lq, P, q_per_wg, n_wg,
                                                        interleave != 0, part, subtot, offsets, records, s, wg);
     if constexpr (!FILL) {
         int *mypart = part + ((size_t)s * n_wg + wg) * plan.nblk;
diff --git a/boxer_amd/csrc/boxattn_binned_tr.h b/boxer_amd/csrc/boxattn_binned_tr.h
--- a/boxer_amd/csrc/boxattn_binned_tr.h
+++ b/boxer_amd/csrc/boxattn_binned_tr.h
@@ -3,6 +3,7 @@
 #include "boxattn_combine.h"
 #include "boxattn_scan_tail.h"
 #include "boxattn_binpass.h"
+#include <type_traits>
 
 namespace boxattn {
 
@@ -24,8 +25,11 @@
     return __builtin_bit_cast(uint2, v);
 }
 
-template <typename ST, int C>
-__global__ __launch_bounds__(64) __attribute__((amdgpu_waves_per_eu(C <= 32 ? BOXATTN_TUNE_TR_WPE : 1))) void binned_accumulate_tr_kernel(
+#ifndef BOXATTN_TUNE_TR_QUAD_WPE
+#define BOXATTN_TUNE_TR_QUAD_WPE 3
+#endif
+template <typename ST, int C, bool QUAD = false>
+__global__ __launch_bounds__(64) __attribute__((amdgpu_waves_per_eu(C <= 32 ? (QUAD ? BOXATTN_TUNE_TR_QUAD_WPE : BOXATTN_TUNE_TR_WPE) : 1))) void binned_accumulate_tr_kernel(
     const ST *__restrict__ grad_out, unsigned grad_out_bytes, BinPlan plan, int S, int H, int Lq,
     const int4 *__restrict__ items, const int *__restrict__ n_items,
     const int *__restrict__ records, ST *__restrict__ grad_value, float *__restrict__ partials, ChunkCombine cc,
@@ -45,9 +49,11 @@
     constexpr int ASB = AS * 2;
     constexpr int kDump = PB * ASB;
     constexpr int kBig = 1 << 20;
+    constexpr int AF = R + 4, AFB = AF * 4, kDumpF = PB * AFB;
+    constexpr int AT_USHORTS = QUAD ? (PB + 1) * AF * 2 : (PB + 1) * AS;
     typedef unsigned int u32x4 __attribute__((ext_vector_type(4)));
     __shared__ __attribute__((aligned(16))) unsigned short gs[NCB * GPL / 2];
-    __shared__ __attribute__((aligned(16))) unsigned short at[(PB + 1) * AS];
+    __shared__ __attribute__((aligned(16))) unsigned short at[AT_USHORTS];
     __shared__ int last_flag;
 
     const int n_slices = plan.n_slices, workers = (int)gridDim.x - plan.zero_workers;
@@ -67,7 +73,7 @@
     const int col = lane & 31, kb = lane >> 5;
     const int n_it = n_items[2 * s];
 
-    for (int i = lane; i < (PB + 1) * AS / 2; i += 64) reinterpret_cast<unsigned int *>(at)[i] = 0u;
+    for (int i = lane; i < AT_USHORTS / 2; i += 64) reinterpret_cast<unsigned int *>(at)[i] = 0u;
     if (C < CP)
         for (int i = lane; i < NCB * GPL / 4; i += 64) reinterpret_cast<unsigned int *>(gs)[i] = 0u;
     wave_lds_sync();
@@ -82,6 +88,10 @@
     const unsigned tr_off = (unsigned)((8 * (g16 >> 1) + (i16 >> 2)) * 64 + (16 * (g16 & 1) + 4 * (i16 & 3)) * 2);
     unsigned a_off = (unsigned)(col * ASB + 16 * kb);
     asm volatile("" : "+v"(a_off));
+    const unsigned af_off = (unsigned)(col * AFB + 32 * kb);
+    const unsigned qpid0 = (unsigned)((b * Lq) * H + h) * (unsigned)(plan.L * 4);
+    const unsigned qstride_p = (unsigned)(H * plan.L * 4);
+    const int lp_mask = (1 << plan.lp_bits) - 1;
 
     const int4 *my_items = items + (size_t)s * plan.item_cap;
     int4 item_n = my_items[min(worker, plan.item_cap - 1)];
@@ -96,6 +106,7 @@
         const int oy = bg.oy, ox = bg.ox, bh = bg.bh, bw = bg.bw;
         const float Hf = (float)lvH, Wf = (float)lvW;
         const int4 *rec = reinterpret_cast<const int4 *>(records) + (size_t)s * plan.rec_cap;
+        const int *rec_q = records + (size_t)s * plan.rec_cap;
         tr_f32x16 acc[NCB];
 #pragma unroll
         for (int cb = 0; cb < NCB; ++cb)
@@ -103,13 +114,23 @@
             for (int r = 0; r < 16; ++r) acc[cb][r] = 0.f;
 
         constexpr unsigned kNoRow = 0x80000000u;
-        auto fetch_rec = [&](int rr) -> int4 {
-            if (rr + lane >= item.z) return make_int4(-1, 0, 0, 0);
-            return rec[rr + lane];
-        };
-        auto fetch_rows = [&](const int4 &r, u32x4 (&rows)[NPASS]) {
-            const unsigned id = (unsigned)r.x;
-            const unsigned off = r.x < 0 ? kNoRow : __umul24(id >> plan.lp_bits, q_stride) + slice_off;
+        using Rec = typename std::conditional<QUAD, int, int4>::type;
+        auto rec_id = [](const Rec &r) -> int {
+            if constexpr (QUAD) return r;
+            else return r.x;
+        };
+        auto fetch_rec = [&](int rr) -> Rec {
+            if constexpr (QUAD) {
+                return rr + lane >= item.z ? -1 : rec_q[rr + lane];
+            } else {
+                if (rr + lane >= item.z) return make_int4(-1, 0, 0, 0);
+                return rec[rr + lane];
+            }
+        };
+        auto fetch_rows = [&](const Rec &r, u32x4 (&rows)[NPASS]) {
+            const int rx = rec_id(r);
+            const unsigned id = (unsigned)rx;
+            const unsigned off = rx < 0 ? kNoRow : __umul24(id >> (plan.lp_bits + (QUAD ? 2 : 0)), q_stride) + slice_off;
 #pragma unroll
             for (int ps = 0; ps < NPASS; ++ps) {
                 const unsigned oj = (unsigned)__shfl((int)off, ps * RPP + jrow, 64) + (unsigned)(piece * 16);
@@ -121,18 +142,99 @@
             for (int ps = 0; ps < NPASS; ++ps)
                 *reinterpret_cast<u32x4 *>(reinterpret_cast<char *>(gs) + stage_off + ps * RPP * 64) = rows[ps];
         };
-        int4 rec_c = fetch_rec(item.y), rec_n = fetch_rec(item.y + R), rec_n2 = fetch_rec(item.y + 2 * R);
+        Rec rec_c = fetch_rec(item.y), rec_n = fetch_rec(item.y + R), rec_n2 = fetch_rec(item.y + 2 * R);
+        struct QuadPts { float4 a, c, w; };
+        auto fetch_pts = [&](int r, QuadPts &g) {
+            const int rq = max(r, 0);
+            const unsigned pid = qpid0 + (unsigned)(rq >> (plan.lp_bits + 2)) * qstride_p + (unsigned)((rq >> 2) & lp_mask & ~3);
+            const float4 *l4 = reinterpret_cast<const float4 *>(zr.loc + 2 * (size_t)pid);
+            g.a = l4[0];
+            g.c = l4[1];
+            g.w = *reinterpret_cast<const float4 *>(zr.w_sp + pid);
+        };
+        QuadPts qp_a, qp_b;
+        if constexpr (QUAD) {
+            fetch_pts(rec_c, qp_a);
+            fetch_pts(rec_n, qp_b);
+        }
         u32x4 grow_a[NPASS], grow_b[NPASS];
         fetch_rows(rec_c, grow_a);
         stage_rows(grow_a);
         if (item.y + R < item.z) fetch_rows(rec_n, grow_a);
-        auto round = [&](int rr, const u32x4 (&next)[NPASS], u32x4 (&ahead)[NPASS]) {
+        auto round = [&](int rr, const u32x4 (&next)[NPASS], u32x4 (&ahead)[NPASS], QuadPts &qp) {
             const bool more = rr + R < item.z;
-            int4 rec_n3 = make_int4(-1, 0, 0, 0);
+            Rec rec_n3;
+            if constexpr (QUAD) rec_n3 = -1;
+            else rec_n3 = make_int4(-1, 0, 0, 0);
             if (rr + 2 * R < item.z) {
                 fetch_rows(rec_n2, ahead);
                 rec_n3 = fetch_rec(rr + 3 * R);
             }
+            if constexpr (QUAD) {
+                const unsigned mask = rec_c >= 0 ? (unsigned)rec_c & 15u : 0u;
+                const float xs[4] = {qp.a.x, qp.a.z, qp.c.x, qp.c.z}, ys[4] = {qp.a.y, qp.a.w, qp.c.y, qp.c.w};
+                const float as[4] = {qp.w.x, qp.w.y, qp.w.z, qp.w.w};
+                const int dump = kDumpF + 4 * lane;
+#pragma unroll
+                for (int k = 0; k < 4; ++k) {
+                    float h_im, w_im;
+                    {
+#pragma clang fp contract(off)
+                        h_im = ys[k] * Hf - 0.5f;
+                        w_im = xs[k] * Wf - 0.5f;
+                    }
+                    const float yf = floorf(h_im), xf = floorf(w_im);
+                    const float lh = h_im - yf, lw = w_im - xf;
+                    const int py = (mask >> k) & 1u ? (int)yf - oy : -2, px = (int)xf - ox;
+                    const float hh = 1.f - lh, hw = 1.f - lw;
+                    const float ha = hh * as[k], la = lh * as[k];
+                    const float w0 = ha * hw, w1 = ha * lw, w2 = la * hw, w3 = la * lw;
+                    const int r0 = (unsigned)py < (unsigned)bh ? __mul24(py, BW * AFB) : kBig;
+                    const int r1 = (unsigned)(py + 1) < (unsigned)bh ? __mul24(py, BW * AFB) + BW * AFB : kBig;
+                    const int c0 = (unsigned)px < (unsigned)bw ? __mul24(px, AFB) + 4 * lane : kBig;
+                    const int c1 = (unsigned)(px + 1) < (unsigned)bw ? __mul24(px, AFB) + 4 * lane + AFB : kBig;
+                    char *atb = reinterpret_cast<char *>(at);
+                    atomicAdd(reinterpret_cast<float *>(atb + min(r0 + c0, dump)), w0);
+                    atomicAdd(reinterpret_cast<float *>(atb + min(r0 + c1, dump)), w1);
+                    atomicAdd(reinterpret_cast<float *>(atb + min(r1 + c0, dump)), w2);
+                    atomicAdd(reinterpret_cast<float *>(atb + min(r1 + c1, dump)), w3);
+                }
+                if (rr + 2 * R < item.z) fetch_pts(rec_n2, qp);
+                wave_lds_sync();
+#pragma unroll
+                for (int t = 0; t < R / 16; ++t) {
+                    char *pa = reinterpret_cast<char *>(at) + af_off + 64 * t;
+                    const float4 v0 = *reinterpret_cast<const float4 *>(pa), v1 = *reinterpret_cast<const float4 *>(pa + 16);
+                    *reinterpret_cast<float4 *>(pa) = make_float4(0.f, 0.f, 0.f, 0.f);
+                    *reinterpret_cast<float4 *>(pa + 16) = make_float4(0.f, 0.f, 0.f, 0.f);
+                    const float v[8] = {v0.x, v0.y, v0.z, v0.w, v1.x, v1.y, v1.z, v1.w};
+                    unsigned hi[4], lo[4];
+#pragma unroll
+                    for (int e = 0; e < 4; ++e) {
+                        hi[e] = pack_bf16x2(v[2 * e], v[2 * e + 1]);
+                        lo[e] = pack_bf16x2(v[2 * e] - __uint_as_float(hi[e] << 16),
+                                            v[2 * e + 1] - __uint_as_float(hi[e] & 0xffff0000u));
+                    }
+                    const tr_bf16x8 p_hi = __builtin_bit_cast(tr_bf16x8, u32x4{hi[0], hi[1], hi[2], hi[3]});
+                    const tr_bf16x8 p_lo = __builtin_bit_cast(tr_bf16x8, u32x4{lo[0], lo[1], lo[2], lo[3]});
+#pragma unroll
+                    for (int cb = 0; cb < NCB; ++cb) {
+                        const uint2 g0 = lds_read_tr16(gs, tr_off + cb * GPL + t * 1024);
+                        const uint2 g1 = lds_read_tr16(gs, tr_off + cb * GPL + t * 1024 + 256);
+                        const tr_bf16x8 g = __builtin_bit_cast(tr_bf16x8, u32x4{g0.x, g0.y, g1.x, g1.y});
+                        acc[cb] = __builtin_amdgcn_mfma_f32_32x32x16_bf16(g, p_hi, acc[cb], 0, 0, 0);
+                        acc[cb] = __builtin_amdgcn_mfma_f32_32x32x16_bf16(g, p_lo, acc[cb], 0, 0, 0);
+                    }
+                }
+                wave_lds_sync();
+                if (more) {
+                    stage_rows(next);
+                    rec_c = rec_n; rec_n = rec_n2; rec_n2 = rec_n3;
+                }
+                wave_lds_sync();
+                return;
+            }
+            else {
             const float x = __int_as_float(rec_c.y), y = __int_as_float(rec_c.z), a = __int_as_float(rec_c.w);
             float h_im, w_im;
             {
@@ -194,11 +296,12 @@
                 rec_c = rec_n; rec_n = rec_n2; rec_n2 = rec_n3;
             }
             wave_lds_sync();
+            }
         };
         for (int rr = item.y; rr < item.z; rr += 2 * R) {
-            round(rr, grow_a, grow_b);
+            round(rr, grow_a, grow_b, qp_a);
             if (rr + R >= item.z) break;
-            round(rr + R, grow_b, grow_a);
+            round(rr + R, grow_b, grow_a, qp_b);
         }
         if (item.w < 0) {
             int ln = lane;
diff --git a/boxer_amd/csrc/boxattn_binpass.h b/boxer_amd/csrc/boxattn_binpass.h
--- a/boxer_amd/csrc/boxattn_binpass.h
+++ b/boxer_amd/csrc/boxattn_binpass.h
@@ -5,7 +5,7 @@
 
 namespace boxattn {
 
-template <int THREADS, int BW, int BH, bool FILL, bool WIDE, int PT>
+template <int THREADS, int BW, int BH, bool FILL, bool WIDE, int PT, bool QUAD = false>
 __device__ __forceinline__ void bin_pass_body(int *hist, BinLevel *s_lv, const float *__restrict__ loc,
                                               const float *__restrict__ w_sp, const BinPlan &plan, int H,
                                               int Lq, int P, int q_per_wg, int n_wg, bool interleave,
@@ -22,6 +22,7 @@
 
     const float2 *loc2 = reinterpret_cast<const float2 *>(loc);
     static_assert(PT == 1 || PT == 4, "points per thread and step");
+    static_assert(!QUAD || (PT == 4 && !WIDE), "quad records: one (query, level) group of four points per thread");
 #ifndef BOXATTN_TUNE_BIN_U
 #define BOXATTN_TUNE_BIN_U 2
 #endif
@@ -76,6 +77,19 @@
         for (int u = 0; u < U; ++u) {
             if (g0 + u * THREADS >= n_grp) break;
             const BinLevel lv = s_lv[(int)(((float)t.lp0[u] + 0.5f) * rcp_p)];
+            if constexpr (QUAD) {
+                int cand[16];
+                quad_blocks(t.xy[u], lv, true, cand);
+                const int id0 = ((q0 + t.ql[u] * qstep) << plan.lp_bits) | t.lp0[u];
+#pragma unroll
+                for (int i = 0; i < 16; ++i) {
+                    if (cand[i] >= 0) {
+                        const int slot = atomicAdd(&hist[cand[i] & kQuadBlockMask], 1);
+                        if constexpr (FILL) rec[slot] = (id0 << 2) | (cand[i] >> kQuadMaskShift);
+                    }
+                }
+                continue;
+            }
 #pragma unroll
             for (int k = 0; k < PT; ++k) {
                 int blk[4];
@@ -114,7 +128,8 @@
 }
 
 enum { kRideWide = 1, kRideInterleave = 2, kRidePt4 = 4,
-       kRideSpec = 8 };
+       kRideSpec = 8,
+       kRideQuad = 16 };
 constexpr int kRideMaxBlocks = 3072;
 constexpr int kRideLdsInts = kRideMaxBlocks + 8 * (int)(sizeof(BinLevel) / sizeof(int)) + 4 * 4 + 2;
 
@@ -178,7 +193,10 @@
     divmod_magic(id, (unsigned)r.n_wg, r.nwg_magic, s_u, wg_u);
     const int s = (int)s_u, wg = (int)wg_u;
     const bool inter = (r.flavour & kRideInterleave) != 0;
-    if (r.flavour & kRidePt4)
+    if (r.flavour & kRideQuad)
+        bin_pass_body<THREADS, 8, 4, false, false, 4, true>(m.hist, m.lv, r.loc, r.w_sp, plan, r.H, r.Lq, r.P, r.q_per_wg,
+                                                           r.n_wg, inter, r.part, r.subtot, r.offsets, r.records, s, wg);
+    else if (r.flavour & kRidePt4)
         bin_pass_body<THREADS, 8, 4, false, false, 4>(m.hist, m.lv, r.loc, r.w_sp, plan, r.H, r.Lq, r.P, r.q_per_wg,
                                                      r.n_wg, inter, r.part, r.subtot, r.offsets, r.records, s, wg);
     else
@@ -230,7 +248,10 @@
     const bool inter = (r.flavour & kRideInterleave) != 0;
     if (wg == 0 && r.ctickets)
         for (int k = threadIdx.x; k < plan.nblk; k += THREADS) r.ctickets[(size_t)s * plan.nblk + k] = 0;
-    if ((r.flavour & kRideWide) && (r.flavour & kRidePt4))
+    if (r.flavour & kRideQuad)
+        bin_pass_body<THREADS, 8, 4, true, false, 4, true>(m.hist, m.lv, r.loc, r.w_sp, plan, r.H, r.Lq, r.P, r.q_per_wg,
+                                                          r.n_wg, inter, r.part, r.subtot, r.offsets, r.records, s, wg);
+    else if ((r.flavour & kRideWide) && (r.flavour & kRidePt4))
         bin_pass_body<THREADS, 8, 4, true, true, 4>(m.hist, m.lv, r.loc, r.w_sp, plan, r.H, r.Lq, r.P, r.q_per_wg,
                                                    r.n_wg, inter, r.part, r.subtot, r.offsets, r.records, s, wg);
     else if (r.flavour & kRideWide)
diff --git a/boxer_amd/csrc/boxattn_binplan.h b/boxer_amd/csrc/boxattn_binplan.h
--- a/boxer_amd/csrc/boxattn_binplan.h
+++ b/boxer_amd/csrc/boxattn_binplan.h
@@ -64,4 +64,46 @@
     blk[3] = inside && rb != ra && cb != ca ? base_b + cb : -1;
 }
 
+constexpr int kQuadMaskShift = 13;
+constexpr int kQuadBlockMask = (1 << kQuadMaskShift) - 1;
+__device__ __forceinline__ void quad_blocks(const float2 (&xy)[4], const BinLevel &lv, bool have, int (&cand)[16])
+{
+    const float Hf = (float)lv.H, Wf = (float)lv.W;
+    int ra[4], ca[4], cr[4], cc[4];
+    bool in[4];
+#pragma unroll
+    for (int k = 0; k < 4; ++k) {
+        float h_im, w_im;
+        {
+#pragma clang fp contract(off)
+            h_im = xy[k].y * Hf - 0.5f;
+            w_im = xy[k].x * Wf - 0.5f;
+        }
+        in[k] = have & (h_im > -1.f) & (w_im > -1.f) & (h_im < Hf) & (w_im < Wf) & (lv.H > 0) & (lv.W > 0);
+        const int y0 = (int)floorf(in[k] ? h_im : 0.f), x0 = (int)floorf(in[k] ? w_im : 0.f);
+        const int ty = __mul24(max(y0, 0), lv.nby), tx = __mul24(max(x0, 0), lv.nbx);
+        const int r = (int)__umulhi((unsigned)ty, lv.mh), c = (int)__umulhi((unsigned)tx, lv.mw);
+        cr[k] = (in[k] & ((unsigned)y0 < (unsigned)(lv.H - 1)) & (ty - __mul24(r, lv.H) + lv.nby >= lv.H)) ? 1 : 0;
+        cc[k] = (in[k] & ((unsigned)x0 < (unsigned)(lv.W - 1)) & (tx - __mul24(c, lv.W) + lv.nbx >= lv.W)) ? 1 : 0;
+        ra[k] = in[k] ? r : -8;
+        ca[k] = c;
+    }
+#pragma unroll
+    for (int k = 0; k < 4; ++k)
+#pragma unroll
+        for (int j = 0; j < 4; ++j) {
+            const int R = ra[k] + (j >> 1), Cc = ca[k] + (j & 1);
+            bool lead = in[k] & ((j & 1) == 0 || cc[k] != 0) & ((j >> 1) == 0 || cr[k] != 0);
+            unsigned mask = 1u << k;
+#pragma unroll
+            for (int k2 = 0; k2 < 4; ++k2) {
+                if (k2 == k) continue;
+                const bool member = ((unsigned)(R - ra[k2]) <= (unsigned)cr[k2]) & ((unsigned)(Cc - ca[k2]) <= (unsigned)cc[k2]);
+                if (k2 < k) lead &= !member;
+                else mask |= member ? 1u << k2 : 0u;
+            }
+            cand[4 * k + j] = lead ? (lv.blk0 + R * lv.nbx + Cc) | (int)(mask << kQuadMaskShift) : -1;
+        }
 }
+
+}
diff --git a/boxer_amd/csrc/boxattn_capi.hip b/boxer_amd/csrc/boxattn_capi.hip
--- a/boxer_amd/csrc/boxattn_capi.hip
+++ b/boxer_amd/csrc/boxattn_capi.hip
@@ -443,12 +443,14 @@
 #include "boxattn_host_plan.h"
 
 template <typename ST, bool INST>
-inline int bin_flavour(const Dims &d, const float *loc, const float *w_sp)
+inline int bin_flavour(const Dims &d, const BinPlan &plan, const float *loc, const float *w_sp)
 {
     const bool wide = acc_kind<ST, INST>(d) != kAccValu;
     const bool pt4 = d.P % 4 == 0 && aligned(loc, 16) && (!wide || aligned(w_sp, 16));
+    if (!INST && std::is_same<ST, bf16_t>::value && pt4 && quad_shape(true, d, plan)) return kRideQuad | kRidePt4;
     return (wide ? kRideWide : kRideInterleave) | (pt4 ? kRidePt4 : 0);
 }
+inline int flavour_record_bytes(int flavour) { return (flavour & kRideWide) ? 16 : 4; }
 inline BinRide make_ride(const float *loc, const float *w_sp, const Dims &d, const BinPlan &plan,
                          const PlanLayout &pl, char *pbuf, const ScratchLayout *sl, char *sbuf, int flavour,
                          bool fill)
@@ -483,13 +485,14 @@
     const dim3 bgrid(w.n_wg, ns);
     const size_t bsh = ((size_t)plan.nblk + 1) * sizeof(int);
     const int inter = (flavour & kRideInterleave) ? 1 : 0;
-    const bool wide = (flavour & kRideWide) != 0, pt4 = (flavour & kRidePt4) != 0;
+    const bool wide = (flavour & kRideWide) != 0, pt4 = (flavour & kRidePt4) != 0, quad = (flavour & kRideQuad) != 0;
     ScopedKernelTimer timer(g_prof.ev[kSlotBwdBin], st);
-#define BOXATTN_BIN(FILL_, WIDE_, PT_)                                                              \
-    hipLaunchKernelGGL((bin_kernel<BW, BH, FILL_, WIDE_, PT_>), bgrid, dim3(kBinThreads), bsh, st, loc, w_sp, \
+#define BOXATTN_BIN(FILL_, WIDE_, PT_, ...)                                                         \
+    hipLaunchKernelGGL((bin_kernel<BW, BH, FILL_, WIDE_, PT_, ##__VA_ARGS__>), bgrid, dim3(kBinThreads), bsh, st, loc, w_sp, \
                        plan, d.H, d.Lq, d.P, w.q_per_wg, w.n_wg, inter, part, subtot, offsets, records, ctickets)
     if (stages & kBinCount) {
-        if (pt4) BOXATTN_BIN(false, false, 4); else BOXATTN_BIN(false, false, 1);
+        if (quad) BOXATTN_BIN(false, false, 4, true);
+        else if (pt4) BOXATTN_BIN(false, false, 4); else BOXATTN_BIN(false, false, 1);
         if (plan.zero_workers > 0)
             hipLaunchKernelGGL(zero_geo_kernel, dim3((plan.nblk + 255) / 256), dim3(256), 0, st, plan,
                                (int2 *)(pbuf + w.zgeo));
@@ -516,7 +519,8 @@
         }
     }
     if (stages & kBinFill) {
-        if (wide && pt4) BOXATTN_BIN(true, true, 4);
+        if (quad) BOXATTN_BIN(true, false, 4, true);
+        else if (wide && pt4) BOXATTN_BIN(true, true, 4);
         else if (wide) BOXATTN_BIN(true, true, 1);
         else BOXATTN_BIN(true, false, 1);
     }
@@ -604,7 +608,7 @@
 int launch_accumulate(AccKind acc, const ST *grad_out, const ST *grad_mask, const float *loc, const float *w_sp,
                       const float *w_lv, const Dims &d, const BinPlan &plan, const int *offsets, const int4 *items,
                       const int *n_items, const int *records, ST *grad_value, float *partials,
-                      const ChunkCombine &cc, const ZeroRole &zr, hipStream_t st)
+                      const ChunkCombine &cc, const ZeroRole &zr, hipStream_t st, bool quad = false)
 {
     constexpr int C = 4 * G;
     const int ns = d.B * d.H, ns8 = (ns + 7) / 8 * 8;
@@ -613,7 +617,7 @@
     if constexpr (std::is_same<ST, bf16_t>::value && !INST) {
         if (acc == kAccTr) {
             launch_accumulate_tr(C, grad_out, (size_t)d.B * d.Lq * d.H * C * sizeof(ST), plan, d.S, d.H, d.Lq, items,
-                                 n_items, records, grad_value, partials, wg_per_slice, ns8, cc, zr, st);
+                                 n_items, records, grad_value, partials, wg_per_slice, ns8, cc, zr, st, quad);
             return finish();
         }
     }
@@ -654,7 +658,8 @@
 {
     const int ns = d.B * d.H;
     const AccKind acc = acc_kind<ST, INST>(d);
-    const int flavour = bin_flavour<ST, INST>(d, loc, w_sp);
+    const int flavour = bin_flavour<ST, INST>(d, plan, loc, w_sp);
+    const bool quad = (flavour & kRideQuad) != 0;
     int *records = (int *)(sbuf + sl.records);
     float *partials = (float *)(sbuf + sl.partials);
     const int *n_items = (const int *)(pbuf + pl.n_items), *offsets = (const int *)(pbuf + pl.offsets);
@@ -686,14 +691,14 @@
                        own_combine ? nullptr : (int *)(sbuf + sl.ctickets));
     ChunkCombine cc{};
     if (!own_combine) cc = ChunkCombine{(int *)(sbuf + sl.ctickets), combos, plan.nblk, plan.pslot_cap};
-    ZeroRole zr{offsets, (const int2 *)(pbuf + pl.zgeo)};
+    ZeroRole zr{offsets, (const int2 *)(pbuf + pl.zgeo), nullptr, quad ? loc : nullptr, quad ? w_sp : nullptr, d.P};
     BinPlan plan_acc = plan;
     if (one_pass && filled) {
         zr = ZeroRole{nullptr, nullptr, spec->redo, loc, w_sp, d.P};
         plan_acc.zero_workers = kSpecRedoWorkers;
     }
     int rc = launch_accumulate<ST, G, INST>(acc, grad_out, grad_mask, loc, w_sp, w_lv, d, plan_acc, offsets, items,
-                                            n_items, records, grad_value, partials, cc, zr, st);
+                                            n_items, records, grad_value, partials, cc, zr, st, quad);
     if (rc) return rc;
     if (spec && !(one_pass && filled))
         hipLaunchKernelGGL(spec_layout_kernel<256>, dim3(ns), dim3(256), 0, st, plan, offsets, spec->cursor, spec->cbase,
@@ -728,7 +733,7 @@
     bool plan_ready = false;
     if (binned) {
         pl = plan_layout(d, plan);
-        sl = scratch_layout(d, plan, wide_workspace(kBf16, d));
+        sl = scratch_layout(d, plan, flavour_record_bytes(bin_flavour<ST, INST>(d, plan, loc, w_sp)));
         plan_ready = plan_buf && plan_bytes >= pl.total && aligned(plan_buf, 256);
         binned = workspace_bytes >= (plan_ready ? sl.total : pl.total + sl.total);
     }
@@ -822,7 +827,7 @@
         return launch_fwd<ST, INST>(value, shapes, lsi, loc, w_sp, w_lv, d, out, mask, st,
                                     shapes_host, lsi_host, nullptr, nullptr, allow_dense, stats);
     char *pbuf = (char *)plan_buf;
-    const int flavour = bin_flavour<ST, INST>(d, loc, w_sp);
+    const int flavour = bin_flavour<ST, INST>(d, plan, loc, w_sp);
     bool taken = false;
     int rc = 0;
     if (riders_ok(plan, pl)) {
@@ -921,7 +926,7 @@
     BinPlan plan;
     if (!make_plan(d, shapes_host, lsi_host, plan)) return fallback;
     return std::max(fallback, plan_layout(d, plan).total +
-                                  scratch_layout(d, plan, wide_workspace(is_bf16 != 0, d)).total);
+                                  scratch_layout(d, plan, record_bytes(is_bf16 != 0, d, plan)).total);
 }
 
 int boxattn_bwd_ws_f32(const float *value, const int64_t *shapes, const int64_t *lsi,
diff --git a/boxer_amd/csrc/boxattn_dense.hip b/boxer_amd/csrc/boxattn_dense.hip
--- a/boxer_amd/csrc/boxattn_dense.hip
+++ b/boxer_amd/csrc/boxattn_dense.hip
@@ -81,16 +81,19 @@
 void launch_accumulate_tr(int C, const uint16_t *grad_out, size_t grad_out_bytes, const BinPlan &plan, int S,
                           int H, int Lq, const int4 *items, const int *n_items, const int *records,
                           uint16_t *grad_value, float *partials, int wg_per_slice, int ns8, const ChunkCombine &cc,
-                          const ZeroRole &zr, hipStream_t st)
+                          const ZeroRole &zr, hipStream_t st, bool quad)
 {
-#define BOXATTN_ACC_TR(C_)                                                                              \
-    hipLaunchKernelGGL((binned_accumulate_tr_kernel<uint16_t, C_>), dim3(wg_per_slice + plan.zero_workers, ns8), dim3(64), 0, st, \
+#define BOXATTN_ACC_TR(C_, Q_)                                                                          \
+    hipLaunchKernelGGL((binned_accumulate_tr_kernel<uint16_t, C_, Q_>), dim3(wg_per_slice + plan.zero_workers, ns8), dim3(64), 0, st, \
                        grad_out, (unsigned)grad_out_bytes, plan, S, H, Lq, items, n_items, records,     \
                        grad_value, partials, cc, zr)
-    switch (C) {
-    case 16: BOXATTN_ACC_TR(16); break;
-    case 32: BOXATTN_ACC_TR(32); break;
-    case 64: BOXATTN_ACC_TR(64); break;
+    switch (C * 2 + (quad ? 1 : 0)) {
+    case 32: BOXATTN_ACC_TR(16, false); break;
+    case 64: BOXATTN_ACC_TR(32, false); break;
+    case 128: BOXATTN_ACC_TR(64, false); break;
+    case 33: BOXATTN_ACC_TR(16, true); break;
+    case 65: BOXATTN_ACC_TR(32, true); break;
+    case 129: BOXATTN_ACC_TR(64, true); break;
     }
 #undef BOXATTN_ACC_TR
 }
diff --git a/boxer_amd/csrc/boxattn_dense_plan.h b/boxer_amd/csrc/boxattn_dense_plan.h
--- a/boxer_amd/csrc/boxattn_dense_plan.h
+++ b/boxer_amd/csrc/boxattn_dense_plan.h
@@ -79,7 +79,7 @@
 void launch_accumulate_tr(int C, const uint16_t *grad_out, size_t grad_out_bytes, const BinPlan &plan, int S,
                           int H, int Lq, const int4 *items, const int *n_items, const int *records,
                           uint16_t *grad_value, float *partials, int wg_per_slice, int ns8, const ChunkCombine &cc,
-                          const ZeroRole &zr, hipStream_t st);
+                          const ZeroRole &zr, hipStream_t st, bool quad);
 
 void launch_accumulate_split(const float *grad_out, size_t grad_out_bytes, const BinPlan &plan, int S, int H, int Lq,
                              const int4 *items, const int *n_items, const int *records, float *grad_value,
diff --git a/boxer_amd/csrc/boxattn_host_plan.h b/boxer_amd/csrc/boxattn_host_plan.h
--- a/boxer_amd/csrc/boxattn_host_plan.h
+++ b/boxer_amd/csrc/boxattn_host_plan.h
@@ -156,13 +156,22 @@
     w.total = o;
     return w;
 }
-inline ScratchLayout scratch_layout(const Dims &d, const BinPlan &p, bool wide)
+inline bool quad_shape(bool is_bf16, const Dims &d, const BinPlan &p)
+{
+    return is_bf16 && accumulate_tr_ok(d) && d.P == 4 && d.Lq == d.S && spec_shape(d, p) &&
+           ((long long)d.Lq << p.lp_bits) < (1ll << 29);
+}
+inline int record_bytes(bool is_bf16, const Dims &d, const BinPlan &p)
+{
+    return quad_shape(is_bf16, d, p) ? 4 : wide_workspace(is_bf16, d) ? 16 : 4;
+}
+inline ScratchLayout scratch_layout(const Dims &d, const BinPlan &p, int rec_bytes)
 {
     const size_t ns = (size_t)d.B * d.H;
     ScratchLayout w;
     size_t o = 0;
     w.ctickets = o; o += align_up(ns * (size_t)p.nblk * 4);
-    w.records = o;  o += align_up(ns * (size_t)p.rec_cap * (wide ? 16 : 4));
+    w.records = o;  o += align_up(ns * (size_t)p.rec_cap * rec_bytes);
     w.partials = o; o += align_up(ns * (size_t)p.pslot_cap * 32 * d.C * 4);
     w.total = o;
     return w;
diff --git a/boxer_amd/csrc/boxattn_spec.h b/boxer_amd/csrc/boxattn_spec.h
--- a/boxer_amd/csrc/boxattn_spec.h
+++ b/boxer_amd/csrc/boxattn_spec.h
@@ -22,7 +22,7 @@
 #ifndef BOXATTN_TUNE_SPEC_U
 #define BOXATTN_TUNE_SPEC_U 1
 #endif
-template <int THREADS, int PT>
+template <int THREADS, int PT, bool QUAD = false>
 __device__ __forceinline__ void spec_fill_body(int *hist, int *base, BinLevel *s_lv, const float *__restrict__ loc,
                                                const float *__restrict__ w_sp, const BinPlan &plan, int H, int Lq,
                                                int P, int q_per_wg, int *__restrict__ cursor_s,
@@ -33,6 +33,7 @@
     constexpr int U = PT == 4 ? BOXATTN_TUNE_SPEC_U : 4;
     constexpr int STRIDE = THREADS * U;
     static_assert(STRIDE * PT * 4 < (1 << kSpecRankBits), "ranks of a step");
+    static_assert(!QUAD || (PT == 4 && STRIDE * 16 <= (1 << (31 - kQuadMaskShift - 4))), "quad candidates and their ranks");
     const int b = s / H, h = s % H;
     const int LP = plan.L * P;
     const int q0 = wg * q_per_wg;
@@ -42,6 +43,7 @@
     const int LPG = LP / PT, n_grp = n_q * LPG;
     const float rcp_lpg = 1.0f / (float)LPG, rcp_p = 1.0f / (float)P;
     int4 *rec = reinterpret_cast<int4 *>(records) + (size_t)s * plan.rec_cap;
+    int *rec_q = records + (size_t)s * plan.rec_cap;
     struct Step {
         float2 xy[U][PT];
         float wv[U][PT];
@@ -61,8 +63,12 @@
                 const float4 a = *reinterpret_cast<const float4 *>(lp8), c = *reinterpret_cast<const float4 *>(lp8 + 16);
                 t.xy[u][0] = make_float2(a.x, a.y); t.xy[u][1] = make_float2(a.z, a.w);
                 t.xy[u][2] = make_float2(c.x, c.y); t.xy[u][3] = make_float2(c.z, c.w);
-                const float4 w4 = *reinterpret_cast<const float4 *>(wp4);
-                t.wv[u][0] = w4.x; t.wv[u][1] = w4.y; t.wv[u][2] = w4.z; t.wv[u][3] = w4.w;
+                if constexpr (!QUAD) {
+                    const float4 w4 = *reinterpret_cast<const float4 *>(wp4);
+                    t.wv[u][0] = w4.x; t.wv[u][1] = w4.y; t.wv[u][2] = w4.z; t.wv[u][3] = w4.w;
+                } else {
+                    (void)wp4;
+                }
             } else {
                 t.xy[u][0] = *reinterpret_cast<const float2 *>(lp8);
                 t.wv[u][0] = *reinterpret_cast<const float *>(wp4);
@@ -83,12 +89,24 @@
     auto work_step = [&](const Step &t, int g0) {
         unsigned meta[U][PT], rk01[U][PT], rk23[U][PT];
         int nbx_u[U];
+        int qc[QUAD ? U : 1][16];
         unsigned long long tph = BOXATTN_RIDE_TRACE ? __builtin_amdgcn_s_memrealtime() : 0ull;
 #pragma unroll
         for (int u = 0; u < U; ++u) {
             const bool have = g0 + u * THREADS < n_grp;
             const BinLevel lv = s_lv[(int)(((float)t.lp0[u] + 0.5f) * rcp_p)];
             nbx_u[u] = lv.nbx;
+            if constexpr (QUAD) {
+                int cand[16];
+                quad_blocks(t.xy[u], lv, have, cand);
+                const int dump = kSpecMaxBlocks + 1 + (int)threadIdx.x;
+                unsigned r[16];
+#pragma unroll
+                for (int i = 0; i < 16; ++i) r[i] = (unsigned)atomicAdd(&hist[cand[i] >= 0 ? cand[i] & kQuadBlockMask : dump], 1);
+#pragma unroll
+                for (int i = 0; i < 16; ++i) qc[u][i] = cand[i] >= 0 ? cand[i] | (int)((r[i] & 0x7FFFu) << (kQuadMaskShift + 4)) : -1;
+                continue;
+            }
             const float Hf = (float)lv.H, Wf = (float)lv.W;
             int b0[PT];
             bool in[PT], cc[PT], cr[PT];
@@ -157,6 +175,21 @@
 #pragma unroll
         for (int u = 0; u < U; ++u) {
             const int idq = (q0 + t.ql[u]) << plan.lp_bits;
+            if constexpr (QUAD) {
+                int sq[16];
+#pragma unroll
+                for (int i = 0; i < 16; ++i) sq[i] = base[qc[u][i] >= 0 ? qc[u][i] & kQuadBlockMask : 0];
+                char *rb4 = reinterpret_cast<char *>(rec_q);
+                const int rq = (idq | t.lp0[u]) << 2;
+#pragma unroll
+                for (int i = 0; i < 16; ++i) {
+                    const int c = qc[u][i];
+                    if (c >= 0 && sq[i] >= 0)
+                        *reinterpret_cast<int *>(rb4 + ((unsigned)(sq[i] + (c >> (kQuadMaskShift + 4))) << 2)) =
+                            rq | ((c >> kQuadMaskShift) & 15);
+                }
+                continue;
+            }
             int sb[PT][4];
 #pragma unroll
             for (int k = 0; k < PT; ++k) {
@@ -381,7 +414,10 @@
     int *cbase_s = r.spec.cbase + (size_t)s * (plan.nblk + 1);
     RIDE_STAMP(5);
     unsigned long long *tr = BOXATTN_RIDE_TRACE && r.trace ? r.trace + (size_t)id * 8 : nullptr;
-    if (r.flavour & kRidePt4)
+    if (r.flavour & kRideQuad)
+        spec_fill_body<THREADS, 4, true>(hist, base, m.lv, r.loc, r.w_sp, plan, r.H, r.Lq, r.P, r.q_per_wg, cursor_s, cbase_s,
+                                         r.records, s, wg, tr);
+    else if (r.flavour & kRidePt4)
         spec_fill_body<THREADS, 4>(hist, base, m.lv, r.loc, r.w_sp, plan, r.H, r.Lq, r.P, r.q_per_wg, cursor_s, cbase_s,
                                    r.records, s, wg, tr);
     else
```

Result: slower. 13.15 Gsample-points/s, median of 2 (-48.4%).
